# adriente/espm

Measured on AMD Instinct MI355X. Metric: MU iterations/sec, 2048ch x (512*512)px X, k=5 SmoothNMF, higher is better.
Workload: dtype f32; 1 GPU; 2048ch x (512x512)px, k=5, SmoothNMF simplex_H + Laplacian lambda=1, X stored ell, W/H fp32; n=2048, k=5, simplex_H=True, parallelism=single GPU, autotune=True, engine_policy=autotune='auto', as SmoothNMF(max_iter=10000).fit builds it, launch_plan=fused, units handed out dynamically

## Files before the change

espm_amd/_lib.py:

```python
from __future__ import annotations

import ctypes as C
import os

import torch

_HERE = os.path.dirname(os.path.abspath(__file__))
LIB_PATH = os.environ.get("ESPM_MU_LIB", os.path.join(_HERE, "lib", "libespm_mu.so"))

from . import _abi

_HEADER_TEXT = _abi.header_text()
_D = _abi.parse_defines(_HEADER_TEXT)
OK, EINVAL, ENOSOLUTION, EHIP, EUNSUPPORTED = 0, -1, -2, -3, -4
X_F32, X_BF16, X_U8, X_ELL = 0, 1, 2, 3
F64_X_U8, F64_X_BF16, F64_X_F32, F64_X_F64 = (_D["ESPM_F64_X_" + n] for n in ("U8", "BF16", "F32", "F64"))
F64_MAX_K, F64_MAXIT = _D["ESPM_F64_MAX_K"], _D["ESPM_F64_MAXIT"]
F64S_MAX_COUNT, F64S_MAX_N, F64S_WBLOCK = _D["ESPM_F64S_MAX_COUNT"], _D["ESPM_F64S_MAX_N"], _D["ESPM_F64S_WBLOCK"]
DIAG_X_U8, DIAG_X_U16, DIAG_X_F32, DIAG_X_F64 = (_D["ESPM_DIAG_X_" + n] for n in ("U8", "U16", "F32", "F64"))
DIAG_MAX_K, DIAG_BLOCK, DIAG_CHUNK = _D["ESPM_DIAG_MAX_K"], _D["ESPM_DIAG_BLOCK"], _D["ESPM_DIAG_CHUNK"]
CDIAG_BLOCK, CDIAG_PCHUNK = _D["ESPM_CDIAG_BLOCK"], _D["ESPM_CDIAG_PCHUNK"]
BIN_BLOCK, BIN_PARTS = _D["ESPM_BIN_BLOCK"], _D["ESPM_BIN_PARTS"]
SPLIT_BLOCK, SPLIT_HEAVY, SPLIT_MAX_K = _D["ESPM_SPLIT_BLOCK"], _D["ESPM_SPLIT_HEAVY"], _D["ESPM_SPLIT_MAX_K"]
SRC_F32, SRC_F64 = 0, 1
LAYOUT_CM, LAYOUT_PM = 0, 1
ABI_VERSION = _D["ESPM_MU_ABI_VERSION"]
XCHG_HANDLE_BYTES = _D["ESPM_XCHG_HANDLE_BYTES"]
ELL_TILE, ELL_PB, ELL_PBITS, ELL_LDS_MAX = _D["ESPM_ELL_TILE"], _D["ESPM_ELL_PB"], _D["ESPM_ELL_PBITS"], _D["ESPM_ELL_LDS_MAX"]
ELL_STREAM_BYTES = _D["ESPM_ELL_STREAM_BYTES"]
ELL_BUCKETS = _D["ESPM_ELL_BUCKETS"]
ELL_HEAVY_MIN, ELL_HEAVY_MAX = _D["ESPM_ELL_HEAVY_MIN"], _D["ESPM_ELL_HEAVY_MAX"]
ELL_UNIT_ROWS, ELL_UNIT_MAX_N, ELL_PAIR_MAX_K = _D["ESPM_ELL_UNIT_ROWS"], _D["ESPM_ELL_UNIT_MAX_N"], _D["ESPM_ELL_PAIR_MAX_K"]
KP, PPAD, NPAD = _D["ESPM_KP"], _D["ESPM_PPAD"], _D["ESPM_NPAD"]
MAX_K = KP
HP_STRIDE, HS_STRIDE, HI_STRIDE = 8 + 2 * KP, 2 * KP, _D["ESPM_HI_STRIDE"]
HS_ROWSUM, HS_MAX = 0, KP
WIDE_MAX_K = 16
WIDEST_MAX_K = 32
TAIL_DEFER, TAIL_RIDE = _D["ESPM_TAIL_DEFER"], _D["ESPM_TAIL_RIDE"]
HI_KLX, HI_REG, HI_LAP, HI_SUMY, HI_BAD, HI_REL_W, HI_REL_H = (_D["ESPM_HI_" + n] for n in ("KLX", "REG", "LAP", "SUMY", "BAD", "REL_W", "REL_H"))

_vp, _i32, _i64, _f32 = C.c_void_p, C.c_int32, C.c_int64, C.c_float


class MUState(C.Structure):
    _fields_ = _abi.parse_struct(_HEADER_TEXT)

    def __init__(self, *args, **kw):
        super().__init__(*args, **kw)
        self.struct_size = C.sizeof(type(self))
        self.abi_version = ABI_VERSION


_SP = C.POINTER(MUState)
SYMBOLS = {
    "espm_mu_version": (C.c_char_p, []),
    "espm_mu_last_error": (C.c_char_p, []),
    "espm_mu_state_size": (C.c_size_t, []),
    "espm_mu_abi_version": (C.c_int, []),
    "espm_mu_state_layout": (C.c_char_p, []),
    "espm_mu_query": (C.c_int, [_SP]),
    "espm_mu_w_update_is_local": (C.c_int, [_SP]),
    "espm_mu_w_update_tail": (C.c_int, [_SP, C.c_int, C.c_int, _vp]),
    "espm_mu_pack_x": (C.c_int, [_vp, C.c_int, C.c_int, _i64, C.c_int, C.c_int, _vp, _vp, C.c_int, C.c_int, C.c_int, C.c_int, C.c_int, _vp]),
    "espm_mu_ell_count": (C.c_int, [_SP, _vp, _vp, _vp, _vp, _vp]),
    "espm_mu_ell_count_hist": (C.c_int, [_SP, _vp, _vp, _vp, _vp, _vp, _vp, _vp]),
    "espm_mu_ell_fill_hist": (C.c_int, [_SP, _vp, _vp, _vp, _vp, _vp, _vp, _vp, _vp, _vp, _vp]),
    "espm_mu_ell_plan": (C.c_int, [_SP, _vp, _vp, _vp, _vp, _vp, _vp, _vp, _vp]),
    "espm_mu_ell_fill": (C.c_int, [_SP, _vp, _vp, _vp, _vp, _vp, _vp, _vp, _vp]),
    "espm_mu_ell_heavy_count": (C.c_int, [_SP, _vp, C.c_int, C.c_int, _i64, _vp, _vp, _vp, _vp]),
    "espm_mu_ell_heavy_fill": (C.c_int, [_SP, _vp, C.c_int, C.c_int, _i64, _vp, _vp, _vp]),
    "espm_mu_hstat": (C.c_int, [_SP, C.c_int, _vp]),
    "espm_mu_build_gw": (C.c_int, [_SP, C.c_int, _vp]),
    "espm_mu_step_h": (C.c_int, [_SP, C.c_int, C.c_int, _vp]),
    "espm_mu_h_finalize": (C.c_int, [_SP, C.c_int, C.c_int, _vp]),
    "espm_mu_loss_only": (C.c_int, [_SP, C.c_int, C.c_int, _vp]),
    "espm_mu_w_accum": (C.c_int, [_SP, _vp]),
    "espm_mu_step_hw": (C.c_int, [_SP, C.c_int, _vp]),
    "espm_mu_fused_applies": (C.c_int, [_SP]),
    "espm_mu_w_reduce": (C.c_int, [_SP, _vp]),
    "espm_mu_w_reduce_finalize": (C.c_int, [_SP, C.c_int, C.c_int, _vp]),
    "espm_mu_w_finish": (C.c_int, [_SP, C.c_int, C.c_int, C.c_int, _vp]),
    "espm_mu_iterate_timed": (C.c_int, [_SP, C.c_int, _vp, _vp, _vp]),
    "espm_mu_iterate": (C.c_int, [_SP, C.c_int, C.c_int, _vp]),
    "espm_mu_iterate_h": (C.c_int, [_SP, C.c_int, C.c_int, _vp]),
    "espm_mu_h_chain_applies": (C.c_int, [_SP]),
    "espm_mu_shard_record_bytes": (C.c_size_t, [_SP]),
    "espm_mu_shard_pack": (C.c_int, [_SP, C.c_int, _vp, _vp]),
    "espm_mu_shard_combine": (C.c_int, [_SP, _vp, C.c_int, C.c_int, _vp]),
    "espm_mu_shard_combine_finish": (C.c_int, [_SP, _vp, C.c_int, C.c_int, C.c_int, _vp]),
    "espm_mu_w_reduce_finish": (C.c_int, [_SP, C.c_int, C.c_int, C.c_int, _vp]),
    "espm_mu_w_reduce_pack": (C.c_int, [_SP, C.c_int, C.c_int, _vp, _vp]),
    "espm_xchg_create": (C.c_int, [C.c_int, C.c_int, C.c_size_t, C.POINTER(_vp)]),
    "espm_xchg_handle": (C.c_int, [_vp, _vp]),
    "espm_xchg_connect": (C.c_int, [_vp, _vp]),
    "espm_xchg_staging": (_vp, [_vp]),
    "espm_xchg_records": (_vp, [_vp, C.c_int]),
    "espm_xchg_post": (C.c_int, [_vp, C.c_uint32, _vp]),
    "espm_xchg_wait": (C.c_int, [_vp, C.c_uint32, _vp]),
    "espm_xchg_timeouts": (C.c_int, [_vp, C.POINTER(C.c_uint32)]),
    "espm_xchg_set_order": (C.c_int, [_vp, C.c_int]),
    "espm_xchg_order": (C.c_int, [_vp]),
    "espm_xchg_destroy": (C.c_int, [_vp]),
    "espm_mu_shard_exchange_finish": (C.c_int, [_SP, _vp, C.c_uint32, C.c_int, C.c_int, _vp]),
    "espm_mu_iterate_sharded": (C.c_int, [_SP, _vp, C.POINTER(C.c_uint32), C.c_int, C.c_int, _vp]),
    "espm_mu_linesearch_terms": (C.c_int, [_SP, C.c_int, C.c_int, _vp, _vp]),
    "espm_mu_linesearch_terms_sharded": (C.c_int, [_SP, C.c_int, C.c_int, _vp, _vp, _vp, _vp]),
    "espm_surrogate_terms": (C.c_int, [_vp, _vp, C.c_int, C.c_int, C.c_int64, C.c_int, C.c_int, C.c_int, _vp, C.c_int, _vp, _vp]),
    "espm_dichotomy_simplex_acc": (C.c_int, [C.c_double, _vp, _vp, C.c_int, C.c_int, C.c_int, C.c_double, C.c_double, C.c_int, _vp, _vp, _vp]),
    "espm_dichotomy_simplex_pg": (C.c_int, [_vp, C.c_int, C.c_int, C.c_double, C.c_double, C.c_int, _vp, _vp]),
    "espm_mu_l2_step_h": (C.c_int, [_SP, C.c_int, _vp, _vp, C.c_int, _vp]),
    "espm_mu_l2_step_w": (C.c_int, [_SP, C.c_int, _vp, _vp, _vp, C.c_int, _vp]),
    "espm_mu_l2_w_partials": (C.c_int, [_SP, _vp, _vp, C.c_int, _vp]),
    "espm_mu_l2_w_finish": (C.c_int, [_SP, C.c_int, _vp, _vp, _vp]),
    "espm_simplex_root_f32": (C.c_int, [_vp, _vp, C.c_int, C.c_int, C.c_float, C.c_float, C.c_int, C.c_int, _vp, _vp, _vp, _vp]),
    "espm_dichotomy_simplex": (C.c_int, [_vp, _vp, C.c_int, C.c_int, C.c_int, C.c_double, C.c_double, C.c_int, _vp, _vp, _vp]),
    "espm_mu_laplacian": (C.c_int, [_vp, C.c_int, C.c_int, C.c_int, _i64, _vp, _vp]),
    "espm_lu_pl_scratch_bytes": (C.c_size_t, [C.c_int, C.c_int, C.c_int]),
    "espm_lu_pl": (C.c_int, [_vp, C.c_int, C.c_int, C.c_int, _i64, _vp, _vp, C.c_size_t, _vp]),
    "espm_f64_scratch_doubles": (_i64, [C.c_int, C.c_int, C.c_int, _i64]),
    "espm_f64_gw": (C.c_int, [_vp, _vp, C.c_int, C.c_int, C.c_int, C.c_double, _vp, _vp, _vp, _vp]),
    "espm_f64_hstat": (C.c_int, [_vp, C.c_int, C.c_int, C.c_double, _vp, _vp, _vp]),
    "espm_f64_h_pass": (C.c_int, [_vp, C.c_int, C.c_int, C.c_int, C.c_double, _vp, _vp, _vp, _vp, C.c_int, _vp, _vp, C.c_double,
                                  C.c_double, C.c_double, C.c_int, C.c_int, C.c_double, C.c_int, _vp, _vp, _vp, _vp, _vp, _vp, _vp]),
    "espm_f64_bisect": (C.c_int, [_vp, _vp, C.c_int, C.c_int, C.c_double, C.c_double, C.c_int, _vp, _vp, _vp, _vp, _vp]),
    "espm_f64_rel": (C.c_int, [_vp, _vp, _i64, C.c_double, _vp, _vp, _vp]),
    "espm_f64_w_accum": (C.c_int, [_vp, C.c_int, C.c_int, C.c_int, C.c_double, _vp, _vp, C.c_int, C.c_double, _vp, _vp, _vp]),
    "espm_f64_w_finish": (C.c_int, [_vp, _vp, _vp, C.c_int, C.c_int, C.c_int, _vp, _vp, C.c_int, _vp, C.c_int, C.c_double, C.c_double,
                                    C.c_int, _vp, _vp, _vp, _vp]),
    "espm_f64_sparse_scratch_doubles": (_i64, [C.c_int, C.c_int, C.c_int]),
    "espm_f64_sparse_h_pass": (C.c_int, [_vp, _vp, _vp, C.c_int, _vp, C.c_int, C.c_int, C.c_double, _vp, _vp, _vp, _vp, C.c_int, _vp, _vp,
                                         C.c_double, C.c_double, C.c_double, C.c_int, C.c_int, C.c_double, C.c_int, _vp, _vp, _vp, _vp,
                                         _vp, _vp, _vp]),
    "espm_f64_sparse_w_accum": (C.c_int, [_vp, _vp, _vp, _vp, _vp, C.c_int, C.c_int, C.c_double, _vp, _vp, C.c_int, C.c_double, _vp, _vp,
                                          _vp]),
    "espm_pixel_diagnostics": (C.c_int, [_vp, C.c_int, C.c_int, _i64, C.c_int, C.c_int, _vp, _vp, C.c_int, C.c_double, C.c_int, _vp, _vp,
                                         _vp, _vp]),
    "espm_channel_diagnostics": (C.c_int, [_vp, C.c_int, C.c_int, _i64, C.c_int, C.c_int, _vp, _vp, C.c_int, C.c_double, _vp, _vp, _vp, _vp,
                                           _vp, C.c_size_t, _vp]),
    "espm_channel_diagnostics_scratch": (C.c_size_t, [C.c_int, C.c_int, C.c_int]),
    "espm_rebin_pixels": (C.c_int, [_vp, C.c_int, C.c_int, _i64, C.c_int, C.c_int, C.c_int, C.c_int, C.c_int, _vp, C.c_int, _i64, _vp]),
    "espm_binning_sums": (C.c_int, [_vp, C.c_int, C.c_int, _i64, C.c_int, C.c_int, C.c_int, _vp, C.c_int, _vp, _vp, C.c_size_t, _vp]),
    "espm_binning_sums_scratch": (C.c_size_t, [C.c_int, C.c_int, C.c_int, C.c_int]),
    "espm_thin_counts": (C.c_int, [_vp, C.c_int, C.c_int, _i64, C.c_int, C.c_int, _i64, _i64, _i64, C.c_uint64, _vp, _vp, _i64, _vp]),
    "espm_split_deviance": (C.c_int, [_vp, C.c_int, C.c_int, _i64, C.c_int, C.c_int, _i64, _i64, _i64, C.c_uint64, _vp, _vp, C.c_int, C.c_double,
                                      _vp, _vp, _vp, _vp]),
}

# ... 77 lines not shown
```

espm_amd/csrc/mu_api.hip:

```cpp
#include <vector>
#include <stdarg.h>
#include <stdio.h>

#include "mu_common.hpp"
#include "mu_xchg.hpp"

namespace espm {

static thread_local char g_err[512] = "";

int set_error(int code, const char* fmt, ...) {
  va_list ap;
  va_start(ap, fmt);
  vsnprintf(g_err, sizeof(g_err), fmt, ap);
  va_end(ap);
  return code;
}

int check_hip(hipError_t e, const char* what) {
  if (e == hipSuccess) return ESPM_OK;
  return set_error(ESPM_EHIP, "%s: %s", what, hipGetErrorString(e));
}

static int roundup(int v, int m) { return (v + m - 1) / m * m; }

#define ESPM_MU_STATE_FIELDS(F) \
  F(struct_size) F(abi_version) F(n) F(m) F(k) F(p) F(nx) F(ny) F(n_pad) F(p_pad) F(x_dtype) F(tile_px) F(nblk_w) \
  F(x_tile) F(n_cm) F(h_variant) F(p_total) F(simplex_h) F(simplex_w) F(grid_mode) F(compute_loss) F(lambda_l) \
  F(sigma_l) F(eps_reg) F(log_shift) F(dicotomy_tol) F(rel_tol) F(xscale) F(gw_floor) F(x_cm) F(x_pm) F(g) \
  F(colsum_g) F(w) F(gw_s) F(colsum_gw) F(gw_a) F(gw_p) F(h) F(h_t) F(mu) F(fixed_h) F(fixed_w) F(simplex_rows) \
  F(halo_top) F(halo_bot) F(hpart) F(hstat) F(a_slab) F(a) F(w_scratch) F(hist) F(hist_len) F(cur) F(it) F(ell_h) \
  F(ell_h_off) F(ell_klc) F(ell_w) F(ell_w_off) F(chan_perm) F(ell_cbits) F(n_cg) F(pix_perm) F(g_t) F(breg_sr_px) \
  F(breg_sr_ch) F(h_rule) F(pg_gamma_w) F(pg_q) F(ell_fill_px) F(ell_fill_num) F(ell_fill_n) F(tail_mode) F(no_fused) \
  F(ell_pb) F(ell_stream) F(ell_hv_n) F(ell_hv_npx) F(ell_hv_ngrp) F(ell_hv_px) F(ell_hv_px_off) F(ell_hv_pm) F(ell_hv_klc) F(ell_hv_kl) \
  F(ell_hv_grp) F(ell_hv_grp_off) F(ell_hv_wm) F(hpart_alt)

static int check_abi(const espm_mu_state* st) {
  ESPM_REQUIRE(st != nullptr, "state is NULL");
  ESPM_REQUIRE(st->struct_size == (uint32_t)sizeof(espm_mu_state) && st->abi_version == (uint32_t)ESPM_MU_ABI_VERSION,
               "espm_mu_state of %u bytes, ABI %u handed to a library built for %zu bytes, ABI %d: the binding's copy of the layout has drifted",
               st->struct_size, st->abi_version, sizeof(espm_mu_state), ESPM_MU_ABI_VERSION);
  return ESPM_OK;
}

static int check_state(const espm_mu_state* st) {
  if (int rc = check_abi(st)) return rc;
  ESPM_REQUIRE(st->n >= 1 && st->p >= 1, "n=%d, p=%d must be >= 1", st->n, st->p);
  if (st->k < ESPM_MIN_K || st->k > ESPM_MAX_K)
    return set_error(ESPM_EUNSUPPORTED, "k=%d: this build supports %d..%d components", st->k, ESPM_MIN_K, ESPM_MAX_K);
  ESPM_REQUIRE(st->n_pad == roundup(st->n, ESPM_NPAD) && st->p_pad == roundup(st->p, ESPM_PPAD),
               "n_pad/p_pad (%d, %d) do not match n, p (%d, %d); call espm_mu_query", st->n_pad, st->p_pad, st->n,
               st->p);
  ESPM_REQUIRE(st->x_dtype >= ESPM_X_F32 && st->x_dtype <= ESPM_X_ELL, "bad x_dtype %d", st->x_dtype);
  if (st->x_dtype == ESPM_X_ELL) {
    ESPM_REQUIRE(st->ell_h && st->ell_h_off && st->ell_klc && st->ell_w && st->ell_w_off && st->chan_perm && st->pix_perm,
                 "the sparse count store needs ell_h, ell_h_off, ell_klc, ell_w, ell_w_off, chan_perm and pix_perm");
    ESPM_REQUIRE((st->tile_px == 64 || st->tile_px == 128 || st->tile_px == 256 || st->tile_px == ESPM_ELL_TILE) &&
                     st->ell_pb == 2 * st->tile_px && st->nblk_w == (st->p + st->ell_pb - 1) / st->ell_pb &&
                     st->n_cg == (st->n + 63) / 64 && st->h_variant == 0,
                 "sparse count store: tile_px must be 64..%d, ell_pb 2 tile_px, nblk_w ceil(p / ell_pb), n_cg ceil(n / 64); call espm_mu_query",
                 ESPM_ELL_TILE);
  }
  ESPM_REQUIRE(st->ell_stream == 0 || (st->ell_stream == 1 && st->x_dtype == ESPM_X_ELL), "ell_stream=%d: 0, or 1 with the sparse store", st->ell_stream);
  ESPM_REQUIRE(st->ell_fill_n >= 0 && (st->ell_fill_n == 0 || (st->x_dtype == ESPM_X_ELL && st->ell_fill_px && st->ell_fill_num)),
               "ell_fill_n=%d needs the sparse store, ell_fill_px and ell_fill_num", st->ell_fill_n);
  ESPM_REQUIRE(st->ell_hv_n >= 0 && (st->ell_hv_n == 0 || (st->x_dtype == ESPM_X_ELL && st->h_rule == 0 && !st->breg_sr_px && st->ell_hv_npx >= 1 &&
                                                          st->ell_hv_npx <= st->ell_hv_n && st->ell_hv_ngrp >= 1 && st->ell_hv_ngrp <= st->ell_hv_n &&
                                                          st->ell_hv_px && st->ell_hv_px_off && st->ell_hv_pm && st->ell_hv_klc && st->ell_hv_kl &&
                                                          st->ell_hv_grp && st->ell_hv_grp_off && st->ell_hv_wm && st->ell_fill_num)),
               "ell_hv_n=%d needs the sparse store with the default H rule, 1 <= ell_hv_npx, ell_hv_ngrp <= ell_hv_n, every ell_hv_* array and "
               "ell_fill_num", st->ell_hv_n);
  ESPM_REQUIRE(st->grid_mode == 0 || (st->nx >= 1 && st->ny >= 1 && st->nx * st->ny == st->p),
               "grid %d x %d does not match p=%d", st->nx, st->ny, st->p);
  ESPM_REQUIRE(st->xscale > 0.f, "xscale must be positive");
  ESPM_REQUIRE(st->n_cm == roundup(st->n, ESPM_NCM), "n_cm must be roundup(n, %d)", ESPM_NCM);
  ESPM_REQUIRE((st->breg_sr_px == nullptr) == (st->breg_sr_ch == nullptr), "breg_sr_px and breg_sr_ch come together");
  ESPM_REQUIRE(!st->breg_sr_px || (st->m == 0 && !st->simplex_w && st->n <= 4096),
               "the Bregman variant is built for G = identity without simplex_W (and n <= 4096)");
  ESPM_REQUIRE(st->h_rule == 0 || ((st->h_rule == 1 || st->h_rule == 2) && !st->breg_sr_px), "h_rule must be 0, 1 or 2 (1, 2 not with the Bregman variant)");
  ESPM_REQUIRE(!(st->pg_gamma_w > 0.f) || (!st->simplex_w && !st->breg_sr_px && (st->m == 0 || (long)st->m * st->k <= 8192)),
               "the projected-gradient W step has no simplex over W (updates.py:368-369), no Bregman variant, and needs M k <= 8192 with a dictionary");
  ESPM_REQUIRE(st->h_variant == 0, "h_variant %d is not built (the matrix-core H-step was retired, DESIGN.md)", st->h_variant);
  ESPM_REQUIRE(st->x_tile >= 64 && ESPM_PPAD % st->x_tile == 0 && st->x_tile % st->tile_px == 0,
               "x_tile=%d must divide %d and be a multiple of tile_px=%d", st->x_tile, ESPM_PPAD, st->tile_px);
  ESPM_REQUIRE(st->m >= 0, "m must be >= 0");
  ESPM_REQUIRE(st->m == 0 || (st->g && st->colsum_g), "m=%d needs g and colsum_g", st->m);
  if (st->log_shift > 0.f && st->simplex_h && (double)st->k * (double)st->log_shift >= 1.0)
    return set_error(ESPM_ENOSOLUTION, "No solution exists! (k * log_shift >= 1)");
  return ESPM_OK;
}

static int nblk_h(const espm_mu_state* st) { return (st->p + st->tile_px - 1) / st->tile_px; }

static int ell_pre_h(const espm_mu_state* st, int src, hipStream_t s) {
  const int ld = st->ell_fill_n + (st->ell_hv_n > 0 ? st->ell_hv_npx : 0);
  if (st->ell_fill_n > 0)
    if (int rc = launch_ell_fill_num(st->gw_s, st->h[src], st->ell_fill_px, st->ell_fill_n, st->n, st->k, st->p_pad, st->log_shift,
                                     st->ell_fill_num, s, ld))
      return rc;
  return st->ell_hv_n > 0 ? launch_ell_hv_h(st, src, ld, s) : ESPM_OK;
}

static int ell_post(const espm_mu_state* st, int hnew, bool w, bool loss, hipStream_t s) {
  if (st->ell_hv_n <= 0) return ESPM_OK;
  if (hnew >= 0) return launch_ell_hv_post(st, st->h[hnew], (size_t)st->p_pad, 1, w, loss, s);
  return launch_ell_hv_post(st, st->h_t, 1, ESPM_KP, w, loss, s);
}

static bool fused_ok(const espm_mu_state* st) {
  return ESPM_MIN_K <= 8 && st->x_dtype == ESPM_X_ELL && st->h_rule == 0 && st->no_fused != 1 &&
         (st->ell_pb >= ESPM_FUSED_MIN_PB || st->nblk_w >= ESPM_FUSED_MIN_BLOCKS || st->no_fused == 3) &&
         fused_ell_lds_bytes(st->n_pad, st->k, st->ell_pb) <= ESPM_ELL_LDS_MAX;
}
static HStepArgs fused_h_args(const espm_mu_state* st, int src) {
  HStepArgs a = make_h_args(st, src, 1);
  a.rec_nb = nblk_h(st);
  return a;
}
// ... 730 lines not shown
```

espm_amd/csrc/mu_common.hpp:

```cpp
#pragma once
#include <hip/hip_runtime.h>
#include <stdint.h>

#include "espm_mu.h"

namespace espm {

constexpr int KP = ESPM_KP;
static_assert(KP == 8 || KP == 16 || KP == 32, "ESPM_KP: 8, 16 or 32");
static_assert(ESPM_MIN_K >= 1 && ESPM_MAX_K <= KP && ESPM_MIN_K <= ESPM_MAX_K, "ESPM_MIN_K .. ESPM_MAX_K must fit the stride");

#if ESPM_MIN_K <= 8
#define ESPM_K_CASES(X) X(1) X(2) X(3) X(4) X(5) X(6) X(7) X(8)
#elif ESPM_MIN_K <= 16
#define ESPM_K_CASES(X) X(9) X(10) X(11) X(12) X(13) X(14) X(15) X(16)
#else
#define ESPM_K_CASES(X) X(17) X(18) X(19) X(20) X(21) X(22) X(23) X(24) X(25) X(26) X(27) X(28) X(29) X(30) X(31) X(32)
#endif

__device__ __forceinline__ void store_row_kp(float* dst, const float (&row)[KP]) {
#pragma unroll
  for (int q = 0; q < KP / 4; ++q)
    reinterpret_cast<float4*>(dst)[q] = make_float4(row[4 * q], row[4 * q + 1], row[4 * q + 2], row[4 * q + 3]);
}
// ... 494 lines not shown
  float x = fminf(fmaxf(0.f, lo), hi), dxold = hi - lo;
  for (int it = 0; it < maxit; ++it) {
    float f = -target, fp = 0.f;
#pragma unroll
    for (int i = 0; i < K; ++i) {
      const float s = b[i] + x, q = 4.f * a * c[i];
      const float r = __builtin_amdgcn_sqrtf(fmaf(s, s, q));
      const float g = s >= 0.f ? q * __builtin_amdgcn_rcpf(r + s) : r - s;
      if (g > floor_g) {
        f += g;
        fp -= g * __builtin_amdgcn_rcpf(r);
      } else {
        f += floor_g;
      }
    }
    if (fabsf(f) <= 4e-7f * target) break;
    if (f > 0.f) lo = x; else hi = x;
    float dx = fp < 0.f ? -f * __builtin_amdgcn_rcpf(fp) : 0.f;
    float xn = x + dx;
    if (!(fp < 0.f) || !(xn > lo && xn < hi) || fabsf(dx) > 0.5f * fabsf(dxold)) {
      dx = (hi - lo) * 0.5f;
      xn = lo + dx;
    }
    dxold = dx;
    if (xn == x) break;
    x = xn;
  }
  nu = x;
  return true;
}

__device__ __forceinline__ float stencil_hl(const float* hrow, const float* halo_top, const float* halo_bot,
                                            int q, int nx, int ny, float hc) {
  const int i = q / ny, j = q - i * ny;
  float acc = 0.f;
  int deg = 0;
  if (j > 0) { acc += hrow[q - 1]; ++deg; }
  if (j < ny - 1) { acc += hrow[q + 1]; ++deg; }
  if (i > 0) { acc += hrow[q - ny]; ++deg; }
  else if (halo_top) { acc += halo_top[j]; ++deg; }
  if (i < nx - 1) { acc += hrow[q + ny]; ++deg; }
  else if (halo_bot) { acc += halo_bot[j]; ++deg; }
  return (float)deg * hc - acc;
}

struct HFinalizeArgs {
  const double* hpart;
  const double* colsum_gw;
  const double* hstat_in;
  double* hstat_out;
  double* hist_slot;
  int nblk, k, compute_loss, have_prev;
  float xscale;
  double* pg_q;
};
struct HStepArgs {
  const void* x_cm;
  const void* x_pm;
  int mfma;
  const float* gw_s;
  const double* colsum_gw;
  const float* h_in;
  float* h_out;
  float* h_t;
  const float* mu;
  const float* fixed_h;
  const float* halo_top;
  const float* halo_bot;
  const double* hstat_in;
  double* hpart;
  int n, k, p, nx, ny, p_pad;
  int x_tile;
  int n_cm;
  const void* gw_a;
  const float* gw_p;
  int simplex_h, grid_mode, compute_loss, write_h;
  int have_prev;
  float lambda_l, sigma_l, eps_reg, log_shift, tol, xscale, rel_tol;
  double inv_count;
  const uint32_t* ell;
  const int32_t* ell_off;
  const float* ell_klc;
  const int32_t* ell_pix;
  int ell_bits, n_pad;
  int ell_tp;
  const float* l2_m;
  const float* breg_sr;
  int h_rule;
  const float* fill_num;
  int fill_n;
  const double* cs_parts;
  int cs_nbk, cs_lds_off, tail_on;
  WTailArgs tail;
  int rec_nb;
  const double* chain_prev;
  int chain_nb, chain_lds_off, chain_fin_on;
  HFinalizeArgs chain_fin;
};
__host__ __device__ inline int ell_pbits(int pb) {
  int b = 6;
  while ((1 << b) < pb) ++b;
  return b;
}
struct WAccumArgs {
  const void* x_pm;
  const void* x_cm;
  int x_tile, n_cm, p_pad, mfma;
  const float* gw_s;
  const float* h_t;
  float* a_slab;
  int n_pad, p, ppb;
  const uint32_t* ell;
  const int32_t* ell_off;
  const int32_t* chan_perm;
  int n_cg;
  int pb, pbits;
  int l2;
};
struct WFinishArgs {
  const float* g;
  const float* g_t;
  const float* colsum_g;
  const float* w_old;
  float* w_new;
  const float* a;
  const double* hstat;
  const float* fixed_w;
  const int32_t* simplex_rows;
  float* scratch;
  const float* breg_sr;
  float pg_gamma_w;
  double* pg_q;
  float* gw_s;
  double* colsum_gw;
  void* gw_a;
  float* gw_p;
  double* hist_slot;
  int n, m, k, n_pad, n_cm, simplex_w, update_w;
  float log_shift, tol, rel_tol, xscale, gw_floor;
};


__device__ __forceinline__ void h_finalize_body(const HFinalizeArgs& a, double* scratch) {
  constexpr int NV = ESPM_HP_NSCALAR + 2 * KP + 1;
  constexpr int V_RELH = 4 + KP, V_MAX = 5 + KP, V_RELW = 5 + 2 * KP;
  double v[NV];
#pragma unroll
  for (int i = 0; i < NV; ++i) v[i] = 0.0;
  v[V_RELW] = -1.0;
  const size_t nb = a.nblk;
  constexpr int U = KP > 8 ? 1 : 4;
  for (int b0 = threadIdx.x; b0 < a.nblk; b0 += U * 256) {
    double t[U][ESPM_HP_RELH + 1], tw[U];
#pragma unroll
    for (int u = 0; u < U; ++u) {
      const int b = b0 + u * 256;
#pragma unroll
      for (int i = 0; i <= ESPM_HP_RELH; ++i) t[u][i] = b < a.nblk ? a.hpart[i * nb + b] : 0.0;
      tw[u] = b < a.nblk ? a.hpart[(size_t)ESPM_HP_RELW * nb + b] : -1.0;
    }
#pragma unroll
    for (int u = 0; u < U; ++u) {
#pragma unroll
      for (int i = 0; i < 4 + KP; ++i) v[i] += t[u][i];
      v[V_RELH] = fmax(v[V_RELH], t[u][ESPM_HP_RELH]);
      v[V_RELW] = fmax(v[V_RELW], tw[u]);
// ... 44 lines not shown
    if (a.pg_q) {
      double q1[1] = {0.0};
      for (int b = threadIdx.x; b < a.nblk; b += 256) q1[0] += a.hpart[(size_t)ESPM_HP_PGQ * nb + b];
      block_reduce<1, 1>(q1, scratch);
      if (threadIdx.x == 0) *a.pg_q = q1[0];
    }
    return;
  }
  const bool is_sum = job < 4 + KP;
  const int field = is_sum ? job : (job == V_RELH ? ESPM_HP_RELH : (job == V_RELW ? ESPM_HP_RELW : ESPM_HP_MAX + (job - V_MAX)));
  double v[1] = {job == V_RELW ? -1.0 : 0.0};
  for (int b = threadIdx.x; b < a.nblk; b += 256) {
    const double t = a.hpart[(size_t)field * nb + b];
    v[0] = is_sum ? v[0] + t : fmax(v[0], t);
  }
  if (is_sum)
    block_reduce<1, 1>(v, scratch);
  else
    block_reduce<1, 0>(v, scratch);
  if (threadIdx.x != 0) return;
  if (job == ESPM_HP_KL) {
    if (a.compute_loss) a.hist_slot[ESPM_HI_KLX] = (double)a.xscale * 0.6931471805599453 * v[0];
  } else if (job == ESPM_HP_REG) {
    a.hist_slot[ESPM_HI_REG] = v[0];
  } else if (job == ESPM_HP_LAP) {
    a.hist_slot[ESPM_HI_LAP] = v[0];
  } else if (job == ESPM_HP_BAD) {
    a.hist_slot[ESPM_HI_BAD] = v[0];
  } else if (is_sum) {
    if (a.hstat_out) a.hstat_out[ESPM_HS_ROWSUM + (job - ESPM_HP_ROWSUM)] = v[0];
  } else if (job == V_RELH) {
    if (a.have_prev) a.hist_slot[ESPM_HI_REL_H] = v[0];
  } else if (job == V_RELW) {
    if (v[0] >= 0.0) a.hist_slot[ESPM_HI_REL_W] = v[0];
  } else {
    if (a.hstat_out) a.hstat_out[ESPM_HS_MAX + (job - V_MAX)] = v[0];
  }
}


inline HStepArgs make_h_args(const espm_mu_state* st, int src, int write_h) {
  HStepArgs a;
  a.x_cm = st->x_cm;
  a.x_pm = st->x_pm;
  a.mfma = st->no_fused == 0;
  a.gw_s = st->gw_s;
  a.colsum_gw = st->colsum_gw;
  a.h_in = st->h[src];
  a.h_out = st->h[1 - src];
  a.h_t = st->h_t;
  a.mu = st->mu;
  a.fixed_h = st->fixed_h;
  a.halo_top = st->grid_mode ? st->halo_top : nullptr;
  a.halo_bot = st->grid_mode ? st->halo_bot : nullptr;
  a.hstat_in = st->hstat[src];
  a.hpart = st->hpart;
  a.n = st->n;
  a.k = st->k;
  a.p = st->p;
  a.nx = st->nx;
  a.ny = st->ny;
  a.p_pad = st->p_pad;
  a.x_tile = st->x_tile;
  a.n_cm = st->n_cm;
  a.gw_a = st->gw_a;
  a.gw_p = st->gw_p;
  a.simplex_h = st->simplex_h;
  a.grid_mode = st->grid_mode;
  a.compute_loss = st->compute_loss;
  a.write_h = write_h;
  a.have_prev = st->it > 0;
  a.rel_tol = st->rel_tol;
  a.inv_count = 1.0 / ((double)st->k * (double)(st->p_total > 0 ? st->p_total : st->p));
  a.lambda_l = st->lambda_l;
  a.sigma_l = st->sigma_l;
  a.eps_reg = st->eps_reg;
  a.log_shift = st->log_shift;
  a.tol = st->dicotomy_tol;
  a.xscale = st->xscale;
  a.ell = st->ell_h;
  a.ell_off = st->ell_h_off;
  a.ell_klc = st->ell_klc;
  a.ell_pix = st->pix_perm;
  a.ell_bits = st->ell_cbits;
  a.ell_tp = st->tile_px;
  a.l2_m = nullptr;
  a.breg_sr = st->breg_sr_px;
  a.h_rule = st->h_rule;
  a.fill_n = st->ell_fill_n + (st->ell_hv_n > 0 ? st->ell_hv_npx : 0);
  a.fill_num = (st->x_dtype == ESPM_X_ELL && a.fill_n > 0) ? st->ell_fill_num : nullptr;
  a.cs_parts = nullptr;
  a.cs_nbk = a.cs_lds_off = a.tail_on = 0;
  a.rec_nb = 0;
  a.chain_prev = nullptr;
  a.chain_nb = a.chain_lds_off = a.chain_fin_on = 0;
  a.chain_fin = HFinalizeArgs{};
  a.n_pad = st->n_pad;
  return a;
}

inline WAccumArgs make_w_args(const espm_mu_state* st) {
  WAccumArgs a;
  a.x_pm = st->x_pm;
  a.x_cm = st->x_cm;
  a.x_tile = st->x_tile;
  a.n_cm = st->n_cm;
  a.p_pad = st->p_pad;
  a.mfma = st->no_fused == 0;
  a.gw_s = st->gw_s;
  a.h_t = st->h_t;
  a.a_slab = st->a_slab;
  a.n_pad = st->n_pad;
  a.p = st->p;
  a.ppb = (st->p + st->nblk_w - 1) / st->nblk_w;
  a.ell = st->ell_w;
  a.ell_off = st->ell_w_off;
  a.chan_perm = st->chan_perm;
  a.n_cg = st->n_cg;
  a.pb = st->ell_pb > 0 ? st->ell_pb : ESPM_ELL_PB;
  a.pbits = ell_pbits(a.pb);
  a.l2 = 0;
  return a;
}

int dispatch_h_step(const HStepArgs& args, int x_dtype, int tile_px, int nblk, hipStream_t stream);
bool h_chain_built(const espm_mu_state* st);
int launch_h_chain(const HStepArgs& args, int x_dtype, int tile_px, int nblk, hipStream_t stream);
int launch_h_finalize(const HFinalizeArgs& args, hipStream_t stream);
int launch_h_ell(const HStepArgs& args, int nblk, hipStream_t stream);
int launch_fused_ell(const HStepArgs& h, const WAccumArgs& w, int nblk, hipStream_t stream, int static_units = 0, int stream_lists = 0);
size_t fused_ell_lds_bytes(int n_pad, int k, int pb);
int launch_ell_count(const uint8_t* x_pm, int n, int n_pad, int p, int p_pad, int cbits, int n_cg, int nblk, int pb,
                     int32_t* cnt_px, int32_t* cnt_bc, float* klc, hipStream_t stream, uint8_t* bkt_px = nullptr, uint8_t* bkt_bc = nullptr);
int launch_ell_plan(const int32_t* cnt_px, const int32_t* cnt_bc, int n, int n_cg, int nblk, int p_pad, int win,
                    int32_t* chan_perm, int32_t* pix_perm, int32_t* h_off, int32_t* w_off, long long* rows, hipStream_t stream);
int launch_ell_fill(const uint8_t* x_pm, int n, int n_pad, int p, int p_pad, int cbits, int n_cg, int nblk, int win, int pb,
                    const int32_t* chan_perm, const int32_t* pix_perm, const int32_t* h_off, const int32_t* w_off,
                    uint32_t* ell_h, uint32_t* ell_w, hipStream_t stream, const uint8_t* x_cm = nullptr, int n_cm = 0, const uint8_t* bkt_px = nullptr,
                    const uint8_t* bkt_bc = nullptr);
int launch_w_ell(const WAccumArgs& args, int k, int nblk, hipStream_t stream);
int launch_ell_fill_num(const float* gw_s, const float* h_in, const int32_t* fill_px, int fill_n, int n, int k, int p_pad, float fill,
                        float* fill_num, hipStream_t stream, int ld = 0);
int launch_ell_hv_count(const void* x, int src_dtype, int layout, int64_t ld, int n, int p, int n_pad, int n_cm, uint8_t* x8, uint8_t* x8c,
                        int32_t* cnt_px, hipStream_t stream);
int launch_ell_hv_fill(const void* x, int src_dtype, int layout, int64_t ld, int n, int p, const int32_t* px_off, int32_t* hv_pm,
                       hipStream_t stream);
int launch_ell_hv_h(const espm_mu_state* st, int src, int ld, hipStream_t stream);
int launch_ell_hv_post(const espm_mu_state* st, const float* h, size_t hs_k, size_t hs_p, bool w, bool loss, hipStream_t stream);
int dispatch_w_accum(const WAccumArgs& args, int k, int x_dtype, int nblk, hipStream_t stream);
int launch_w_reduce(const float* slab, float* out, int nblk, int total, const HFinalizeArgs* fused_finalize,
                    hipStream_t stream, const float* bw_old = nullptr, double* bparts = nullptr, int n = 0, int k = 0, int n_pad = 0);
int launch_w_simplex_update(const WFinishArgs& f, float* a_inout, const double* bparts, double tol, hipStream_t stream, WTailArgs* defer_tail);
int launch_w_reduce_pack(const float* slab, int nblk, int k, int n_pad, const HFinalizeArgs& fin_to_record,
                         const float* h_new, int nx, int ny, int p_pad, int with_halo, void* rec, hipStream_t stream);
int launch_w_finish(const WFinishArgs& args, hipStream_t stream);
int launch_gram(const float* m, int rows, int k, double* part, int part_cap, float* out, hipStream_t stream);
int launch_w_finish_l2(const float* a, int n, int n_pad, int m, int k, const float* g, const float* gtg, const float* hh, const float* w_old,
                       float* w_new, const float* fixed_w, float log_shift, hipStream_t stream);
int launch_w_reduce_update(const WFinishArgs& f, const void* src, size_t src_stride, int nsrc, float* a_out,
                           const double* hpart, int nblk_h, const double* hstat_rs, size_t rec_hstat_off, double* hstat_out,
                           const HFinalizeArgs* fused_finalize, hipStream_t stream, WTailArgs* defer_tail = nullptr);
int launch_w_update_tail(const WTailArgs& t, hipStream_t stream);
int launch_w_exchange_update(const WFinishArgs& f, const void* slabs, size_t slab_stride, int nslab, float* a_out, double* hstat_out,
                             const HFinalizeArgs& fin, const struct ::espm_xchg* xc, unsigned int seq, const float* h_new, int nx, int ny,
                             int p_pad, int with_halo, hipStream_t stream, WTailArgs* defer_tail, double* simplex_bparts = nullptr);
bool w_gsplit_applies(const WFinishArgs& args);
// ... 24 lines not shown
```

espm_amd/csrc/mu_ell_build.hip:

```cpp
#include <mutex>

#include "mu_common.hpp"

namespace espm {

__device__ __forceinline__ int ell_reps(int x, int xmax) { return (x + xmax - 1) / xmax; }

template <typename F>
__device__ __forceinline__ void ell_block_for_each_count(const uint8_t* __restrict__ x_pm, int n, int n_pad, int q_mine,
                                                         uint32_t* tile, int* s_q, F f) {
  static_assert(ESPM_NPAD % 8 == 0, "8-byte row reads");
  const int t = threadIdx.x;
  s_q[t] = q_mine;
  __syncthreads();
  for (int c0 = 0; c0 < n; c0 += 128) {
#pragma unroll
    for (int i = 0; i < 16; ++i) {
      const int id = i * 256 + t, r = id >> 4, c8 = id & 15;
      const int q = s_q[r], c = c0 + 8 * c8;
      uint2 v = make_uint2(0u, 0u);
      if (q >= 0 && c < n_pad) v = *reinterpret_cast<const uint2*>(x_pm + (size_t)q * n_pad + c);
      tile[r * 33 + 2 * c8] = v.x;
      tile[r * 33 + 2 * c8 + 1] = v.y;
    }
// ... 320 lines not shown
      for (int u = 0; u < 16; ++u)
        if (x[u] != 0) f(qb + u - q0, x[u]);
    }
  };
  if (units) {
    bk.clear();
    if (bkt) {
      for (int i = 0; i < EllBuckets::B; ++i) bk.c(i) = bkt[((size_t)b * n_cg * 64 + c) * EllBuckets::B + i];
    } else {
      for_each_count([&](int i, int x) {
        if (x == 1) bk.count(i);
      });
    }
    holes = bk.plan(lane, units);
  }
  int j = 0, overflow = 0;
  for_each_count([&](int i, int x) {
    if (x == 1 && units) {
      const int pos = bk.place(i, lane, units, holes, overflow);
      if (pos >= 0) {
        ell_put(base16, row0, pos, lane, (uint32_t)i << 4);
        return;
      }
    }
    while (x > 0) {
      const int v = x > xmax ? xmax : x;
      ell_put(base16, row1, j++, lane, ((uint32_t)v << pbits) | (uint32_t)i);
      x -= v;
    }
  });
}

struct SideStream {
  hipStream_t stream = nullptr;
  hipEvent_t fork = nullptr, join = nullptr;
};
static hipStream_t side_stream_of_device() {
  static const bool enabled = [] { const char* e = getenv("ESPM_ELL_BUILD_SIDE"); return !(e && e[0] == '0'); }();
  if (!enabled) return nullptr;
  static std::mutex mu;
  static hipStream_t per_device[64] = {};
  int dev = 0;
  if (hipGetDevice(&dev) != hipSuccess || dev < 0 || dev >= 64) return nullptr;
  std::lock_guard<std::mutex> lock(mu);
  if (!per_device[dev] && hipStreamCreateWithFlags(&per_device[dev], hipStreamNonBlocking) != hipSuccess) per_device[dev] = nullptr;
  return per_device[dev];
}
static hipStream_t side_fork(SideStream& s, hipStream_t stream) {
  s.stream = side_stream_of_device();
  if (!s.stream) return stream;
  if (hipEventCreateWithFlags(&s.fork, hipEventDisableTiming) != hipSuccess || hipEventCreateWithFlags(&s.join, hipEventDisableTiming) != hipSuccess ||
      hipEventRecord(s.fork, stream) != hipSuccess || hipStreamWaitEvent(s.stream, s.fork, 0) != hipSuccess) {
    (void)hipGetLastError();
    s.stream = nullptr;
    return stream;
  }
  return s.stream;
}
static int side_join(SideStream& s, hipStream_t stream) {
  int rc = ESPM_OK;
  if (s.stream) {
    rc = check_hip(hipEventRecord(s.join, s.stream), "ell build: side stream");
    if (!rc) rc = check_hip(hipStreamWaitEvent(stream, s.join, 0), "ell build: side stream");
  }
  if (s.fork) (void)hipEventDestroy(s.fork);
  if (s.join) (void)hipEventDestroy(s.join);
  return rc;
}

int launch_ell_count(const uint8_t* x_pm, int n, int n_pad, int p, int p_pad, int cbits, int n_cg, int nblk, int pb,
                     int32_t* cnt_px, int32_t* cnt_bc, float* klc, hipStream_t stream, uint8_t* bkt_px, uint8_t* bkt_bc) {
  const int xmax_h = (1 << (16 - cbits)) - 1, xmax_w = (1 << (16 - ell_pbits(pb))) - 1;
  SideStream side;
  const hipStream_t s2 = side_fork(side, stream);
  hipLaunchKernelGGL(ell_count_h_kernel, dim3((p_pad + 255) / 256), dim3(256), 0, stream, x_pm, n, n_pad, p, p_pad, xmax_h,
                     n <= ESPM_ELL_UNIT_MAX_N ? 1 : 0, cnt_px, klc, bkt_px);
  hipLaunchKernelGGL(ell_count_w_kernel, dim3(nblk, (n_cg * 64 + 255) / 256), dim3(256), 0, s2, x_pm, n, n_pad, p,
                     n_cg * 64, xmax_w, pb, cnt_bc, bkt_bc);
  const int rc = check_hip(hipGetLastError(), "ell_count launch");
  const int rc2 = side_join(side, stream);
  return rc ? rc : rc2;
}

int launch_ell_plan(const int32_t* cnt_px, const int32_t* cnt_bc, int n, int n_cg, int nblk, int p_pad, int win,
                    int32_t* chan_perm, int32_t* pix_perm, int32_t* h_off, int32_t* w_off, long long* rows, hipStream_t stream) {
  const size_t lds = (size_t)(n > win ? n : win) * sizeof(int32_t);
  if (lds > 64 * 1024) {
    if (int rc = check_hip(hipFuncSetAttribute(reinterpret_cast<const void*>(ell_order_kernel),
                                               hipFuncAttributeMaxDynamicSharedMemorySize, (int)lds), "ell_plan"))
      return rc;
  }
  hipLaunchKernelGGL(ell_order_kernel, dim3(nblk + p_pad / win), dim3(1024), lds, stream, cnt_px, cnt_bc, n, n_cg, nblk, win,
                     chan_perm, pix_perm);
  const long long groups = (long long)(p_pad / 64) + (long long)nblk * n_cg;
  hipLaunchKernelGGL(ell_group_extent_kernel, dim3((unsigned)((groups + 3) / 4)), dim3(256), 0, stream, cnt_px, cnt_bc, n_cg, nblk,
                     p_pad / 64, win, chan_perm, pix_perm, h_off, w_off);
  hipLaunchKernelGGL(ell_offsets_kernel, dim3(1), dim3(1024), 0, stream, n_cg, nblk, p_pad / 64, h_off, w_off, rows);
  return check_hip(hipGetLastError(), "ell_plan launch");
}

int launch_ell_fill(const uint8_t* x_pm, int n, int n_pad, int p, int p_pad, int cbits, int n_cg, int nblk, int win, int pb,
                    const int32_t* chan_perm, const int32_t* pix_perm, const int32_t* h_off, const int32_t* w_off,
                    uint32_t* ell_h, uint32_t* ell_w, hipStream_t stream, const uint8_t* x_cm, int n_cm, const uint8_t* bkt_px,
                    const uint8_t* bkt_bc) {
  SideStream side;
  const hipStream_t s2 = side_fork(side, stream);
  hipLaunchKernelGGL(ell_fill_h_kernel, dim3((p_pad + 255) / 256), dim3(256), 0, stream, x_pm, n, n_pad, p, p_pad, cbits, win,
                     pix_perm, h_off, ell_h, bkt_px);
  hipLaunchKernelGGL(ell_fill_w_kernel, dim3(nblk, (n_cg + ESPM_ELL_FILLW_WAVES - 1) / ESPM_ELL_FILLW_WAVES), dim3(64 * ESPM_ELL_FILLW_WAVES), 0, s2, x_pm, x_cm, n_cm, n_pad, p, n_cg, pb, ell_pbits(pb), chan_perm, w_off, ell_w, bkt_bc);
  const int rc = check_hip(hipGetLastError(), "ell_fill launch");
  const int rc2 = side_join(side, stream);
  return rc ? rc : rc2;
}

}
```

espm_amd/csrc/mu_ell_kernel.hpp:

```cpp
#pragma once
#include "mu_h_kernel.hpp"


namespace espm {

typedef float lds_v4f __attribute__((ext_vector_type(4)));
typedef float lds_v2f __attribute__((ext_vector_type(2)));
#define ESPM_LDS(T) __attribute__((address_space(3))) const T*
__device__ __forceinline__ uint32_t lds_address(const float* ptr) {
  return (uint32_t)(uintptr_t)(__attribute__((address_space(3))) const float*)ptr;
}
__device__ __forceinline__ void ell_table_at_lds_zero(const float* tab) {
  if (lds_address(tab) != 0u) __builtin_trap();
}
template <int K>
struct EllTab {
  static constexpr int WB = LdsTabGeom<K>::WB;
  static constexpr int FLOATS = 4 + WB;
  static constexpr int WQ = WB / 4;
  static __device__ __forceinline__ const float* quad(const float* tab, int rows) { return tab + (size_t)WB * rows; }
  static __device__ __forceinline__ void put(float* tab, int rows, int r, const float* src) {
    float row[(K + 3) / 4 * 4];
#pragma unroll
    for (int i = 0; i < (K + 3) / 4 * 4; i += 4) {
// ... 3 lines not shown
    lds_table_put_row<K>(tab, rows, r, row);
  }
  static __device__ __forceinline__ void get(const float* tab, int rows, uint32_t r, float (&g)[K]) {
#ifdef ESPM_EXPERIMENT_GENERAL_NOCONFLICT
    r = (threadIdx.x & 15) + 16 * ((r >> 4) & 7);
#endif
    const float4 lo = reinterpret_cast<const float4*>(quad(tab, rows))[r];
    const float l[4] = {lo.x, lo.y, lo.z, lo.w};
#pragma unroll
    for (int i = 0; i < (K < 4 ? K : 4); ++i) g[i] = l[i];
    if constexpr (WB == 1) g[4] = tab[r];
    if constexpr (WB == 2) {
      const float2 v = reinterpret_cast<const float2*>(tab)[r];
      g[4] = v.x;
      g[5] = v.y;
    }
    if constexpr (WB >= 4) {
#pragma unroll
      for (int q = 0; q < WQ; ++q) {
        const float4 v = reinterpret_cast<const float4*>(tab)[(size_t)r * WQ + q];
        const float h[4] = {v.x, v.y, v.z, v.w};
#pragma unroll
        for (int i = 0; i < 4; ++i)
          if (4 + 4 * q + i < K) g[4 + 4 * q + i] = h[i];
      }
    }
  }
  static __device__ __forceinline__ void get_unit(uint32_t lds_q, uint32_t off, float (&g)[K]) {
    const lds_v4f lo = *(ESPM_LDS(lds_v4f))(uintptr_t)(lds_q + off);
#pragma unroll
    for (int i = 0; i < (K < 4 ? K : 4); ++i) g[i] = lo[i];
    if constexpr (WB == 1) g[4] = *(ESPM_LDS(float))(uintptr_t)(off >> 2);
    if constexpr (WB == 2) {
      const lds_v2f v = *(ESPM_LDS(lds_v2f))(uintptr_t)(off >> 1);
      g[4] = v[0];
      g[5] = v[1];
    }
    if constexpr (WB >= 4) {
      const uint32_t base = off * WQ;
#pragma unroll
      for (int q = 0; q < WQ; ++q) {
        const lds_v4f v = *(ESPM_LDS(lds_v4f))(uintptr_t)(base + 16 * q);
#pragma unroll
        for (int i = 0; i < 4; ++i)
          if (4 + 4 * q + i < K) g[4 + 4 * q + i] = v[i];
      }
    }
  }
};

#ifndef ESPM_ELL_DOT_PLAIN
#define ESPM_ELL_DOT_PLAIN 0
#endif
#ifndef ESPM_ELL_DOT_PLAIN_K
#define ESPM_ELL_DOT_PLAIN_K 5
#endif
template <int K>
__device__ __forceinline__ float ell_dot(const float (&g)[K], const float (&h)[K]) {
  if constexpr (ESPM_ELL_DOT_PLAIN || K == ESPM_ELL_DOT_PLAIN_K) {
    float y = g[0] * h[0];
#pragma unroll
    for (int i = 1; i < K; ++i) y = fmaf(g[i], h[i], y);
    return y;
  } else if constexpr (K == 1) {
    return g[0] * h[0];
  } else {
    f2 s = f2{g[0], g[1]} * f2{h[0], h[1]};
#pragma unroll
    for (int q = 1; q < K / 2; ++q) s = f2{g[2 * q], g[2 * q + 1]} * f2{h[2 * q], h[2 * q + 1]} + s;
    float y = s.x + s.y;
    if constexpr (K & 1) y = fmaf(g[K - 1], h[K - 1], y);
    return y;
  }
}
template <int K>
__device__ __forceinline__ void ell_axpy(float (&acc)[K], const float (&g)[K], float r) {
#pragma unroll
  for (int q = 0; q < K / 2; ++q) {
    const f2 t = f2{g[2 * q], g[2 * q + 1]} * r + f2{acc[2 * q], acc[2 * q + 1]};
    acc[2 * q] = t.x;
    acc[2 * q + 1] = t.y;
  }
  if constexpr (K & 1) acc[K - 1] = fmaf(g[K - 1], r, acc[K - 1]);
}

struct EllNoFlush {
  template <typename Redo>
  __device__ __forceinline__ void operator()(Redo) const {}
};
template <int PRIO>
__device__ __forceinline__ void ell_walk_prio(int left) {
  if constexpr (PRIO > 0) {
    if (left > 3 * PRIO) __builtin_amdgcn_s_setprio(3);
    else if (left > 2 * PRIO) __builtin_amdgcn_s_setprio(2);
    else if (left > PRIO) __builtin_amdgcn_s_setprio(1);
    else __builtin_amdgcn_s_setprio(0);
  }
}
template <bool STREAM>
__device__ __forceinline__ uint32_t ell_list_load(const uint32_t* p) {
  if constexpr (STREAM) return __builtin_nontemporal_load(p);
  else return *p;
}
template <int UNR, int PF, bool STREAM>
__device__ __forceinline__ bool ell_walk_request(const uint32_t* row, int len, uint32_t (&pre)[PF][UNR]) {
  if (len < UNR) return false;
#pragma unroll
  for (int d = 0; d < PF; ++d) {
    const int jd = min(d * UNR, len - UNR);
#pragma unroll
    for (int u = 0; u < UNR; ++u) pre[d][u] = ell_list_load<STREAM>(row + (size_t)(jd + u) * 64);
  }
  return true;
}
#ifndef ESPM_ELL_WALK_PP_MAX_K
#define ESPM_ELL_WALK_PP_MAX_K 5
#endif
#ifndef ESPM_ELL_BATCH_HALVES_K
#define ESPM_ELL_BATCH_HALVES_K 7
#endif
template <int K, int UNR, int PF = 1, int PRIO = 0, bool STREAM = false, bool PP = false, typename Get, typename Body, typename Flush = EllNoFlush>
__device__ __forceinline__ void ell_walk_pre(const uint32_t* row, int len, Get get, Body body, Flush flush, bool use_pre, const uint32_t (&pre)[PF][UNR]) {
  auto batch = [&](const uint32_t (&e)[UNR]) {
    constexpr int HALVES = (K >= ESPM_ELL_BATCH_HALVES_K && K <= 8 && UNR % 2 == 0) ? 2 : 1;
    constexpr int UH = UNR / HALVES;
#pragma unroll
    for (int hh = 0; hh < HALVES; ++hh) {
      float g[2 * UH][K], x[2 * UH];
#pragma unroll
      for (int u = 0; u < UH; ++u) {
        x[2 * u] = get(e[hh * UH + u], 0, g[2 * u]);
        x[2 * u + 1] = get(e[hh * UH + u], 1, g[2 * u + 1]);
      }
#pragma unroll
      for (int u = 0; u < 2 * UH; ++u) body(x[u], g[u]);
      if constexpr (HALVES > 1) __builtin_amdgcn_sched_barrier(0);
    }
    flush([&](auto alt) {
#pragma unroll
      for (int u = 0; u < UNR; ++u) {
        float g0[K], g1[K];
        const float x0 = get(e[u], 0, g0), x1 = get(e[u], 1, g1);
        alt(x0, g0);
        alt(x1, g1);
      }
    });
  };
  int j = 0;
  if constexpr (PF == 1 && PP) {
    if (len >= UNR) {
      uint32_t qa[UNR], qb[UNR];
      if (use_pre) {
#pragma unroll
        for (int u = 0; u < UNR; ++u) qa[u] = pre[0][u];
      } else {
#pragma unroll
        for (int u = 0; u < UNR; ++u) qa[u] = ell_list_load<STREAM>(row + (size_t)u * 64);
      }
      for (; j + 2 * UNR <= len; j += 2 * UNR) {
        ell_walk_prio<PRIO>(len - j);
        const int jb = min(j + UNR, len - UNR);
#pragma unroll
        for (int u = 0; u < UNR; ++u) qb[u] = ell_list_load<STREAM>(row + (size_t)(jb + u) * 64);
        batch(qa);
        ell_walk_prio<PRIO>(len - j - UNR);
        const int ja = min(j + 2 * UNR, len - UNR);
#pragma unroll
        for (int u = 0; u < UNR; ++u) qa[u] = ell_list_load<STREAM>(row + (size_t)(ja + u) * 64);
        batch(qb);
      }
      if (j + UNR <= len) {
        ell_walk_prio<PRIO>(len - j);
        batch(qa);
        j += UNR;
      }
    }
  } else if (len >= UNR) {
    uint32_t q[PF][UNR];
    if (use_pre) {
#pragma unroll
      for (int d = 0; d < PF; ++d)
#pragma unroll
        for (int u = 0; u < UNR; ++u) q[d][u] = pre[d][u];
    } else {
#pragma unroll
      for (int d = 0; d < PF; ++d) {
        const int jd = min(d * UNR, len - UNR);
#pragma unroll
        for (int u = 0; u < UNR; ++u) q[d][u] = ell_list_load<STREAM>(row + (size_t)(jd + u) * 64);
      }
    }
    for (; j + UNR <= len; j += UNR) {
      ell_walk_prio<PRIO>(len - j);
      uint32_t e[UNR];
#pragma unroll
      for (int u = 0; u < UNR; ++u) e[u] = q[0][u];
#pragma unroll
      for (int d = 0; d + 1 < PF; ++d)
#pragma unroll
        for (int u = 0; u < UNR; ++u) q[d][u] = q[d + 1][u];
      const int jn = min(j + PF * UNR, len - UNR);
#pragma unroll
      for (int u = 0; u < UNR; ++u) q[PF - 1][u] = ell_list_load<STREAM>(row + (size_t)(jn + u) * 64);
      batch(e);
    }
  }
  for (; j < len; ++j) {
    const uint32_t v = ell_list_load<STREAM>(row + (size_t)j * 64);
    float g0[K], g1[K];
    const float x0 = get(v, 0, g0), x1 = get(v, 1, g1);
    body(x0, g0);
    body(x1, g1);
    flush([&](auto alt) {
      float a0[K], a1[K];
      const float y0 = get(v, 0, a0), y1 = get(v, 1, a1);
      alt(y0, a0);
      alt(y1, a1);
    });
  }
}
template <int K, int UNR, int PF = 1, int PRIO = 0, bool STREAM = false, bool PP = false, typename Get, typename Body, typename Flush = EllNoFlush>
__device__ __forceinline__ void ell_walk(const uint32_t* row, int len, Get get, Body body, Flush flush = Flush()) {
  uint32_t none[PF][UNR];
  ell_walk_pre<K, UNR, PF, PRIO, STREAM, PP>(row, len, get, body, flush, false, none);
}
template <int K>
struct EllGet {
  const float* tab;
  int rows, idx_bits;
  uint32_t mask;
  __device__ __forceinline__ EllGet(const float* t, int r, int bits) : tab(t), rows(r), idx_bits(bits), mask((1u << bits) - 1u) {}
  __device__ __forceinline__ float operator()(uint32_t e, int half, float (&g)[K]) const {
    const uint32_t v = half ? e >> 16 : e & 0xffffu;
    EllTab<K>::get(tab, rows, v & mask, g);
    return (float)(v >> idx_bits);
  }
};
template <int K>
struct EllGetUnit {
  uint32_t lds_q;
  __device__ __forceinline__ EllGetUnit(int rows) : lds_q((uint32_t)(EllTab<K>::WB * rows) * 4u) {}
  __device__ __forceinline__ float operator()(uint32_t e, int half, float (&g)[K]) const {
    EllTab<K>::get_unit(lds_q, half ? e >> 16 : e & 0xffffu, g);
    return 1.f;
  }
};

template <int K>
struct EllGetUnitFix {
  static constexpr bool FIXED = FixTab<K>::TWO && FixTab<K>::FIXED;
  uint32_t lds_q;
  __device__ __forceinline__ EllGetUnitFix(int rows = 0) : lds_q((uint32_t)(EllTab<K>::WB * rows) * 4u) {}
  static __device__ __forceinline__ void row(uint32_t off, float (&g)[K]) {
    const lds_v4f lo = *(ESPM_LDS(lds_v4f))(uintptr_t)off;
#pragma unroll
    for (int i = 0; i < (K < 4 ? K : 4); ++i) g[i] = lo[i];
    if constexpr (K == 5) g[4] = *(ESPM_LDS(float))(uintptr_t)(off + ESPM_TAB2_BASE);
    if constexpr (K == 6) {
      const lds_v2f v = *(ESPM_LDS(lds_v2f))(uintptr_t)(off + ESPM_TAB2_BASE);
      g[4] = v[0];
      g[5] = v[1];
    }
    if constexpr (K >= 7) {
      const lds_v4f v = *(ESPM_LDS(lds_v4f))(uintptr_t)(off + ESPM_TAB2_BASE);
#pragma unroll
      for (int i = 0; i < 4; ++i)
        if (4 + i < K) g[4 + i] = v[i];
    }
  }
  __device__ __forceinline__ float operator()(uint32_t e, int half, float (&g)[K]) const {
    if constexpr (FIXED || K <= 4) row(half ? e >> 16 : e & 0xffffu, g);
    else EllTab<K>::get_unit(lds_q, half ? e >> 16 : e & 0xffffu, g);
    return 1.f;
  }
};
template <int K>
struct EllGetFix {
  const float* tab;
  int rows, idx_bits;
  uint32_t mask;
  __device__ __forceinline__ EllGetFix(const float* t, int r, int bits) : tab(t), rows(r), idx_bits(bits), mask((1u << bits) - 1u) {}
  __device__ __forceinline__ float operator()(uint32_t e, int half, float (&g)[K]) const {
    const uint32_t v = half ? e >> 16 : e & 0xffffu;
    if constexpr (EllGetUnitFix<K>::FIXED || K <= 4) EllGetUnitFix<K>::row((v & mask) << 4, g);
    else EllTab<K>::get(tab, rows, v & mask, g);
    return (float)(v >> idx_bits);
  }
};
template <int K, bool FIX>
struct EllGetters {
  typedef EllGetUnit<K> Unit;
  typedef EllGet<K> General;
};
template <int K>
struct EllGetters<K, true> {
  typedef EllGetUnitFix<K> Unit;
  typedef EllGetFix<K> General;
};

#ifndef ESPM_ELL_KLPROD
#define ESPM_ELL_KLPROD 1
#endif
template <int K, bool LOSS, int UNR, int PF, int PRIO = 0, bool STREAM = false, bool FIX = false, bool PP = false>
__device__ __forceinline__ void ell_h_rows(const uint32_t* lrow, int x0, int x1, int mid, const float* tab, int n_pad, int ell_bits,
                                           const float (&hk)[K], float (&acc)[K], float& kl) {
  if (x0 < mid) {
    if constexpr (LOSS && ESPM_ELL_KLPROD) {
      float prod = 1.f;
      ell_walk<K, UNR, PF, PRIO, STREAM, PP>(lrow + (size_t)x0 * 64, min(x1, mid) - x0, typename EllGetters<K, FIX>::Unit(n_pad),
        [&](float, const float (&g)[K]) {
          const float r = __builtin_amdgcn_rcpf(ell_dot<K>(g, hk));
          ell_axpy<K>(acc, g, r);
          prod *= r;
        },
        [&](auto redo) {
          const bool ok = __builtin_amdgcn_classf(prod, 0x100);
          if (__builtin_expect(__builtin_amdgcn_ballot_w64(!ok) != 0, 0)) {
            redo([&](float, const float (&g)[K]) { kl += __builtin_amdgcn_logf(__builtin_amdgcn_rcpf(ell_dot<K>(g, hk))); });
          } else {
            kl += __builtin_amdgcn_logf(prod);
          }
          prod = 1.f;
        });
    } else {
      ell_walk<K, UNR, PF, PRIO, STREAM, PP>(lrow + (size_t)x0 * 64, min(x1, mid) - x0, typename EllGetters<K, FIX>::Unit(n_pad), [&](float, const float (&g)[K]) {
        const float r = __builtin_amdgcn_rcpf(ell_dot<K>(g, hk));
        ell_axpy<K>(acc, g, r);
        if constexpr (LOSS) kl += __builtin_amdgcn_logf(r);
      });
    }
  }
  if (x1 > mid) {
    const int g0 = max(x0, mid);
    ell_walk<K, UNR, PF, PRIO, STREAM, PP>(lrow + (size_t)g0 * 64, x1 - g0, typename EllGetters<K, FIX>::General(tab, n_pad, ell_bits), [&](float x, const float (&g)[K]) {
      const float y = ell_dot<K>(g, hk);
      const float r = LOSS ? fmaf(x, __builtin_amdgcn_rcpf(y), 1e-37f) : x * __builtin_amdgcn_rcpf(y);
      ell_axpy<K>(acc, g, r);
      if constexpr (LOSS) kl = fmaf(x, __builtin_amdgcn_logf(r), kl);
    });
  }
}

template <int K, bool LOSS, int UNR, int RULE = 0, bool CHAIN = false>
__global__ __launch_bounds__(ESPM_ELL_TILE, (K > 8 ? 2 : 4)) void h_step_ell_kernel(const HStepArgs a) {
  constexpr int NT = ESPM_ELL_TILE;
  constexpr bool PAIRS_OK = K <= ESPM_ELL_PAIR_MAX_K;
  extern __shared__ __attribute__((aligned(16))) float smem[];
  float* tab = smem;
  ell_table_at_lds_zero(tab);
  float* part = smem + (size_t)a.n_pad * EllTab<K>::FLOATS;
  const int TP = a.ell_tp;
  const int gpw = TP >> 6;
  const bool pairs = PAIRS_OK && gpw == NT / 64;
  double* chain_scr = nullptr;
  if constexpr (CHAIN) {
    if (a.chain_fin_on && blockIdx.x == gridDim.x - 1) {
      chain_finalize_wg(a.chain_fin, reinterpret_cast<double*>(smem));
      return;
    }
    chain_scr = reinterpret_cast<double*>(reinterpret_cast<unsigned char*>(smem) + a.chain_lds_off);
    if (a.chain_prev) chain_stats_wave_stage<K>(a.chain_prev, a.chain_nb, chain_scr);
  } else if (a.tail_on && blockIdx.x == gridDim.x - 1) {
    w_tail_body<20>(a.tail, reinterpret_cast<double*>(smem));
    return;
  }
  double* cs_lds = a.cs_parts ? reinterpret_cast<double*>(reinterpret_cast<unsigned char*>(smem) + a.cs_lds_off) : nullptr;
  const bool cs_late = cs_lds && a.cs_lds_off == 0;
  auto form_cs = [&]() {
    for (int kk = threadIdx.x >> 6; kk < K; kk += NT / 64) {
      double v = 0.0;
      for (int j = threadIdx.x & 63; j < a.cs_nbk; j += 64) v += a.cs_parts[(size_t)kk * a.cs_nbk + j];
      v = wave_sum(v);
      if ((threadIdx.x & 63) == 0) cs_lds[kk] = v;
    }
  };
  if (cs_lds && !cs_late) form_cs();
  for (int r = threadIdx.x; r < a.n_pad; r += NT) EllTab<K>::put(tab, a.n_pad, r, a.gw_s + (size_t)r * KP);
  if (pairs) {
#pragma unroll
    for (int kk = 0; kk < K; ++kk) part[((size_t)K + kk) * TP + threadIdx.x] = 0.f;
  }
  __syncthreads();
  const int lane = threadIdx.x & 63;
  const int wave = __builtin_amdgcn_readfirstlane(threadIdx.x >> 6);
  const int tile0 = blockIdx.x * TP;
  float kl = 0.f;

  auto walk_rows = [&](int gi, int x0, int x1, int slot) {
    const int grp = tile0 / 64 + gi;
    const int lp = a.ell_pix[tile0 + gi * 64 + lane];
    const int px = tile0 + lp;
    float hk[K], acc[K];
#pragma unroll
    for (int kk = 0; kk < K; ++kk) {
      hk[kk] = a.h_in[(size_t)kk * a.p_pad + px];
      acc[kk] = 0.f;
    }
    const int beg = a.ell_off[2 * grp], mid = a.ell_off[2 * grp + 1] - beg;
    const uint32_t* lrow = a.ell + (size_t)beg * 64 + lane;
    ell_h_rows<K, LOSS, UNR, 1>(lrow, x0, x1, mid, tab, a.n_pad, a.ell_bits, hk, acc, kl);
#pragma unroll
    for (int kk = 0; kk < K; ++kk) part[((size_t)slot * K + kk) * TP + lp] = acc[kk];
    if (LOSS && slot == 0) kl += fmaxf(a.ell_klc[px], 0.f);
  };
  auto group_rows = [&](int gi) { return a.ell_off[2 * (tile0 / 64 + gi) + 2] - a.ell_off[2 * (tile0 / 64 + gi)]; };

  int nparts;
  if (pairs) {
    const int gl = wave < 4 ? wave : 7 - wave;
    const int len_l = group_rows(gl), len_s = group_rows(7 - gl);
    const int half = min(len_l, (len_l + len_s + 1) / 2);
    if (wave < 4) {
      walk_rows(gl, 0, half, 0);
    } else {
      walk_rows(wave, 0, len_s, 0);
      if (half < len_l) walk_rows(gl, half, len_l, 1);
    }
    nparts = 2;
  } else {
    const int nsplit = (NT / 64) / gpw;
// ... 63 lines not shown
```

espm_amd/csrc/mu_fused.hip:

```cpp
#include <stdlib.h>

#include "mu_fused_kernel.hpp"

#ifndef ESPM_ELL_UNR_H
#define ESPM_ELL_UNR_H 4
#endif
#ifndef ESPM_FUSED_SMALL_UNR_H
#define ESPM_FUSED_SMALL_UNR_H ESPM_ELL_UNR_H
#endif
#ifndef ESPM_FUSED_SMALL_UNR_W
#define ESPM_FUSED_SMALL_UNR_W ESPM_ELL_UNR_W
#endif
#ifndef ESPM_ELL_UNR_W
#define ESPM_ELL_UNR_W 4
#endif

#ifndef ESPM_FUSED_FULL_PERM_LDS
#define ESPM_FUSED_FULL_PERM_LDS 0
#endif
#define ESPM_FUSED_LDS_LIMIT (160 * 1024)
#ifndef ESPM_FUSED_SMALL_SEGS_DEFAULT
#define ESPM_FUSED_SMALL_SEGS_DEFAULT 0
#endif

// ... 41 lines not shown
    if (red > part) part = red;
    if (tail_scratch > part) part = tail_scratch;
    return part;
  };
  size_t bytes = 0;
  auto layout = [&](size_t part, bool red_in_table) {
    const size_t tab_bytes = FixTab<K>::bytes(tab_rows);
    bytes = tab_bytes + part;
    args.cnt_lds_off = (int)bytes;
    bytes += 16 + ESPM_FUSED_MAX_UNITS * sizeof(float);
    args.meta_lds_off = (int)bytes;
    bytes += (size_t)(3 * (pb / 64) + 2 * args.w.n_cg + 1 + 3) / 4 * 16;
    args.perm_lds_off = (int)bytes;
    const size_t perm_bytes = (size_t)(pb + 64 * args.w.n_cg) * sizeof(int);
    args.perm_lds = pb != ESPM_ELL_PB || (ESPM_FUSED_FULL_PERM_LDS && bytes + perm_bytes + KP * sizeof(double) <= ESPM_FUSED_LDS_LIMIT);
    if (args.perm_lds) bytes += perm_bytes;
    args.red_lds_off = -1;
    const size_t hp_tab = FixTab<K>::bytes(pb);
    if (ESPM_FUSED_RED_ONE_BARRIER && red_in_table && hp_tab + red_own <= tab_bytes) {
      args.red_lds_off = (int)hp_tab;
    } else if (ESPM_FUSED_RED_ONE_BARRIER && bytes + red_own + 2 * KP * sizeof(double) <= ESPM_FUSED_LDS_LIMIT) {
      bytes = (bytes + 7) / 8 * 8;
      args.red_lds_off = (int)bytes;
      bytes += red_own;
    }
    if (args.h.cs_parts) {
      bytes = (bytes + 7) / 8 * 8;
      args.h.cs_lds_off = (int)bytes;
      bytes += 2 * KP * sizeof(double);
    }
  };
  args.h_segs = full ? FusedGeom<K>::S : ESPM_ELL_PB / pb;
  size_t part0 = part_of(args.h_segs);
  bool red_in_table = false;
  if (full) {
    for (int segs = FusedGeom<K>::S_MAX; segs > FusedGeom<K>::S; --segs) {
      bool ok = false;
      for (int rit = 0; rit < 2 && !ok; ++rit) {
        layout(part_of(segs), rit != 0);
        ok = bytes <= ESPM_FUSED_LDS_LIMIT && args.red_lds_off >= 0;
        if (ok) red_in_table = rit != 0;
      }
      if (ok) {
        args.h_segs = segs;
        part0 = part_of(segs);
        break;
      }
    }
  }
  const size_t slab = (size_t)K * args.w.n_pad * sizeof(float);
  args.slab_lds = 0;
  layout(part0, red_in_table);
  args.w_split = 0;
  if (ESPM_FUSED_SLAB_LDS && args.w.n_pad % 4 == 0) {
    if (slab > part0) {
      layout(slab, false);
      if (bytes > ESPM_FUSED_LDS_LIMIT || args.red_lds_off < 0) {
        layout(part0, red_in_table);
      } else {
        args.slab_lds = 1;
        const int want = fused_env_small_segs();
        const int fit = (int)(slab / ((size_t)FusedGeom<K>::PROWS * pb * sizeof(float)));
        int segs = want > 0 ? want : args.h_segs;
        if (segs > fit) segs = fit;
        if (segs > ESPM_FUSED_MAX_SEGS) segs = ESPM_FUSED_MAX_SEGS;
        if (segs > args.h_segs) args.h_segs = segs;
      }
    } else {
      args.slab_lds = args.red_lds_off >= 0;
      args.w_split = ESPM_FUSED_W_SPLIT && args.slab_lds && pb == ESPM_ELL_PB && 2 * slab <= part0;
    }
  }
  if (args.h.tail_on && !args.h.tail.pg_q) args.h.tail_on = 2;
  if (bytes > ((args.perm_lds && pb == ESPM_ELL_PB) || args.red_lds_off >= 0 ? ESPM_FUSED_LDS_LIMIT : ESPM_ELL_LDS_MAX))
    return set_error(ESPM_EUNSUPPORTED, "fused half-steps: %zu bytes of LDS exceed %d", bytes, ESPM_ELL_LDS_MAX);
  {
    const int NT = ESPM_ELL_WTHREADS;
    const int n_perm = args.perm_lds ? pb + 64 * args.w.n_cg : 0, n_woff = 2 * args.w.n_cg + 1;
    const bool staged_ok = args.h.n_pad <= 4 * NT && n_perm <= 4 * NT && n_woff <= NT && args.h.cs_nbk <= 64 && 2 * K <= NT / 64;
    const bool plain = ESPM_FUSED_PLAIN && fused_env_plain() && !args.h.fixed_h && !args.h.fill_num && !args.h.breg_sr && !args.h.l2_m &&
                       args.h.simplex_h && args.h.lambda_l != 0.f && args.h.grid_mode && args.h.have_prev && args.h.write_h && args.h.h_rule == 0 &&
                       args.h.tail_on != 1 && !args.static_units && args.slab_lds && !args.w_split && args.red_lds_off >= 0 && staged_ok &&
                       (args.perm_lds != 0) == (pb != ESPM_ELL_PB) && ESPM_FUSED_SMALL_THREADS == ESPM_ELL_WTHREADS;
    if (plain && args.stream_lists && pb == ESPM_ELL_PB) return launch_fused_plain_stream(args, K, args.h.compute_loss != 0, true, nblk, bytes, stream);
    if (plain) return launch_fused_plain(args, K, args.h.compute_loss != 0, pb == ESPM_ELL_PB, nblk, bytes, stream);
  }
  auto go = [&](auto kern, int threads) -> int {
    if (bytes > 64 * 1024)
      if (int rc = check_hip(hipFuncSetAttribute(reinterpret_cast<const void*>(kern), hipFuncAttributeMaxDynamicSharedMemorySize, (int)bytes),
                             "fused half-steps"))
        return rc;
    hipLaunchKernelGGL(kern, dim3(nblk + (args.h.tail_on == 1 ? 1 : 0)), dim3(threads), bytes, stream, args);
    return check_hip(hipGetLastError(), "fused half-steps launch");
  };
  if (pb == ESPM_ELL_PB)
    return args.h.compute_loss ? go(mu_fused_ell_kernel<K, true, ESPM_ELL_UNR_H, ESPM_ELL_UNR_W, ESPM_ELL_WTHREADS, true>, ESPM_ELL_WTHREADS)
                               : go(mu_fused_ell_kernel<K, false, ESPM_ELL_UNR_H, ESPM_ELL_UNR_W, ESPM_ELL_WTHREADS, true>, ESPM_ELL_WTHREADS);
  return args.h.compute_loss ? go(mu_fused_ell_kernel<K, true, ESPM_FUSED_SMALL_UNR_H, ESPM_FUSED_SMALL_UNR_W, ESPM_FUSED_SMALL_THREADS, false>, ESPM_FUSED_SMALL_THREADS)
                             : go(mu_fused_ell_kernel<K, false, ESPM_FUSED_SMALL_UNR_H, ESPM_FUSED_SMALL_UNR_W, ESPM_FUSED_SMALL_THREADS, false>, ESPM_FUSED_SMALL_THREADS);
}
#endif

size_t fused_ell_lds_bytes(int n_pad, int k, int pb) {
  if (pb < 128 || pb > ESPM_ELL_PB || (pb & (pb - 1))) return (size_t)-1;
  const int tab_rows = n_pad > pb ? n_pad : pb;
  const bool fixed = k > 4 && k >= ESPM_FIXTAB_MIN_K;
  if (fixed && tab_rows > ESPM_TAB2_BASE / 16) return (size_t)-1;
  const int wb = k <= 4 ? 0 : (k == 5 ? 1 : (k == 6 ? 2 : 4));
  const size_t tab_bytes = fixed ? (size_t)ESPM_TAB2_BASE + (size_t)16 * tab_rows : (size_t)(4 + wb) * 4 * tab_rows;
  const int seg = pb == ESPM_ELL_PB ? (k <= 4 ? 4 : (k <= 6 ? 3 : 2)) : ESPM_ELL_PB / pb;
  const int n_cg = (n_pad + 63) / 64;
  size_t part = (size_t)seg * k * pb * 4;
  const size_t red = (size_t)(ESPM_ELL_WTHREADS / 64 + 1) * (ESPM_HP_NSCALAR + 2 * k + 1) * sizeof(double);
  const size_t tail_scratch = (size_t)((ESPM_ELL_WTHREADS / 64 + 1) * (KP + 1) + 1) * sizeof(double);
  if (red > part) part = red;
  if (tail_scratch > part) part = tail_scratch;
  return tab_bytes + part + 16 + ESPM_FUSED_MAX_UNITS * sizeof(float) + (size_t)(3 * (pb / 64) + 2 * n_cg + 4) / 4 * 16 + 2 * KP * sizeof(double) + 8 +
         (pb != ESPM_ELL_PB ? (size_t)(pb + 64 * n_cg) * sizeof(int) : 0);
}

int launch_fused_ell(const HStepArgs& h, const WAccumArgs& w, int nblk, hipStream_t stream, int static_units, int stream_lists) {
  ESPM_REQUIRE(h.ell && h.ell_off && h.ell_klc && h.ell_pix && w.ell && w.ell_off && w.chan_perm, "fused half-steps: the sparse store's lists are missing");
  ESPM_REQUIRE(w.pb >= 128 && w.pb <= ESPM_ELL_PB && (w.pb & (w.pb - 1)) == 0 && 2 * h.ell_tp == w.pb && h.h_rule == 0 && h.write_h && !h.l2_m,
               "fused half-steps: blocks of two H tiles (tile_px=%d, ell_pb=%d), the default H rule, write_h", h.ell_tp, w.pb);
  ESPM_REQUIRE(nblk == (h.p + w.pb - 1) / w.pb && w.n_cg >= 1, "fused half-steps: nblk_w=%d must be ceil(p / %d)", nblk, w.pb);
  FusedArgs fa;
  fa.h = h;
  fa.w = w;
  fa.static_units = static_units;
  fa.stream_lists = stream_lists;
  switch (h.k) {
#if ESPM_MIN_K <= 8
#define ESPM_X(KK) case KK: return launch_fused_k<KK>(fa, nblk, stream);
    ESPM_K_CASES(ESPM_X)
#undef ESPM_X
#endif
  }
  return set_error(ESPM_EUNSUPPORTED, "fused half-steps: k=%d not built", h.k);
}

}

#ifdef ESPM_PHASE_CLOCK
extern "C" int espm_debug_phase_buffer(void* dev_ptr) {
  unsigned long long* p = static_cast<unsigned long long*>(dev_ptr);
  if (int rc = espm::phase_buffer_plain(p)) return rc;
  if (int rc = espm::phase_buffer_plain_stream(p)) return rc;
  return espm::check_hip(hipMemcpyToSymbol(HIP_SYMBOL(espm::espm_phase_buf), &p, sizeof(p)), "phase buffer");
}
#endif
```

espm_amd/csrc/mu_fused_kernel.hpp:

```cpp
#pragma once
#include "mu_ell_kernel.hpp"

#ifndef ESPM_FUSED_SMALL_THREADS
#define ESPM_FUSED_SMALL_THREADS 1024
#endif
#ifndef ESPM_FUSED_SMALL_PREFETCH
#define ESPM_FUSED_SMALL_PREFETCH 1
#endif
#ifndef ESPM_FUSED_CUT2
#define ESPM_FUSED_CUT2 60
#endif
#ifndef ESPM_FUSED_FIRST_PREFETCH
#define ESPM_FUSED_FIRST_PREFETCH 1
#endif
#ifndef ESPM_FUSED_FULL_PREFETCH
#define ESPM_FUSED_FULL_PREFETCH 1
#endif
#ifndef ESPM_FUSED_RED_ONE_BARRIER
#define ESPM_FUSED_RED_ONE_BARRIER 1
#endif
#ifndef ESPM_FUSED_SMALL_PRIO
#define ESPM_FUSED_SMALL_PRIO 4
#endif
#ifndef ESPM_FUSED_FULL_PRIO
// ... 6 lines not shown
#ifndef ESPM_FUSED_SUM_BATCHED
#define ESPM_FUSED_SUM_BATCHED 1
#endif
#ifndef ESPM_FUSED_SLAB_LDS
#define ESPM_FUSED_SLAB_LDS 1
#endif
#ifndef ESPM_FUSED_MAX_SEGS
#define ESPM_FUSED_MAX_SEGS 8
#endif
#ifndef ESPM_FUSED_SMALL_SKEW
#define ESPM_FUSED_SMALL_SKEW 0
#endif
#ifndef ESPM_FUSED_W_SPLIT
#define ESPM_FUSED_W_SPLIT 0
#endif
#ifndef ESPM_FUSED_SLAB_WT
#define ESPM_FUSED_SLAB_WT 1
#endif

namespace espm {

struct FusedArgs {
  HStepArgs h;
  WAccumArgs w;
  int cnt_lds_off;
  int meta_lds_off;
  int perm_lds_off;
  int static_units;
  int red_lds_off;
  int perm_lds;
  int h_segs;
  int w_split;
  int stream_lists;
  int slab_lds;
};

#ifndef ESPM_FUSED_CUT4_A
#define ESPM_FUSED_CUT4_A 45
#endif
#ifndef ESPM_FUSED_CUT4_B
#define ESPM_FUSED_CUT4_B 75
#endif
#ifndef ESPM_FUSED_CUT4_C
#define ESPM_FUSED_CUT4_C 92
#endif
#define ESPM_FUSED_MAX_UNITS 64
template <int K>
struct FusedGeom {
  static constexpr int S = K <= 4 ? 4 : (K <= 6 ? 3 : 2);
  static constexpr int S_MAX = K <= 6 ? 4 : 3;
  static constexpr int PROWS = K;
  static constexpr int MIN_SPLIT = 48;
  static __device__ __forceinline__ int seg_begin(int len, int s) {
    if (len < MIN_SPLIT) return s == 0 ? 0 : len;
    constexpr int cut4[5] = {0, ESPM_FUSED_CUT4_A, ESPM_FUSED_CUT4_B, ESPM_FUSED_CUT4_C, 100}, cut3[4] = {0, 45, 80, 100}, cut2[3] = {0, ESPM_FUSED_CUT2, 100};
    const int c = S == 4 ? cut4[s] : (S == 3 ? cut3[s] : cut2[s]);
    return (int)((long)len * c / 100);
  }
  static __device__ __forceinline__ int seg_begin_rt(int len, int s, int segs) {
    if (len < MIN_SPLIT) return s == 0 ? 0 : len;
    constexpr int cut4[5] = {0, ESPM_FUSED_CUT4_A, ESPM_FUSED_CUT4_B, ESPM_FUSED_CUT4_C, 100}, cut3[4] = {0, 45, 80, 100}, cut2[3] = {0, ESPM_FUSED_CUT2, 100};
    const int c = segs == 4 ? cut4[s] : (segs == 3 ? cut3[s] : cut2[s]);
    return (int)((long)len * c / 100);
  }
  static __device__ __forceinline__ int seg_begin_even(int len, int s, int segs) {
    if (len < MIN_SPLIT) return s == 0 ? 0 : len;
    if constexpr (ESPM_FUSED_SMALL_SKEW != 0) {
      if (segs > 1) return (int)(((long)len * s * (100L * segs + (long)ESPM_FUSED_SMALL_SKEW * (segs - s))) / (100L * segs * segs));
    }
    return (int)((long)len * s / segs);
  }
};

template <int K, bool LOSS, int UNR_H, int UNR_W, int NT, bool FULL, bool PLAIN = false, bool STREAM = false>
__global__ __launch_bounds__(NT) void mu_fused_ell_kernel(const FusedArgs fa) {
  static_assert(!FULL || NT == ESPM_ELL_WTHREADS, "full geometry: 1024 threads");
  static_assert(FULL || !STREAM, "streamed lists: the full geometry (an image below it fits the last-level cache)");
  static_assert(ESPM_ELL_PB == 2 * ESPM_ELL_TILE && ESPM_ELL_WTHREADS == ESPM_ELL_PB, "full geometry: a workgroup is two H tiles, one thread per pixel");
  const int PB = FULL ? ESPM_ELL_PB : fa.w.pb;
  const int PBITS = FULL ? ESPM_ELL_PBITS : fa.w.pbits;
  const int TP = PB / 2;
  const int GPT_SHIFT = PBITS - 7;
  constexpr int PROWS = FusedGeom<K>::PROWS;
  constexpr bool S_RT = FULL && FusedGeom<K>::S_MAX > FusedGeom<K>::S;
  const int S = (FULL && !S_RT) ? FusedGeom<K>::S : fa.h_segs;
  constexpr int PF = FULL ? ESPM_FUSED_FULL_PREFETCH : ESPM_FUSED_SMALL_PREFETCH;
  constexpr bool WALK_PP = FULL && K <= ESPM_ELL_WALK_PP_MAX_K;
  constexpr int PRIO = FULL ? (K >= 5 ? ESPM_FUSED_FULL_PRIO : 0) : ESPM_FUSED_SMALL_PRIO;
  const int NGRP = PB / 64;
  const HStepArgs& a = fa.h;
  extern __shared__ __attribute__((aligned(16))) float smem[];
  float* tab = smem;
  ell_table_at_lds_zero(tab);
  ESPM_PHASE_STAMP(0);
  ESPM_PHASE_WHERE();
  const int tab_rows = a.n_pad > PB ? a.n_pad : PB;
  float* part = smem + FixTab<K>::bytes(tab_rows) / sizeof(float);
  int* cnt = reinterpret_cast<int*>(reinterpret_cast<unsigned char*>(smem) + fa.cnt_lds_off);
  float* ukl = reinterpret_cast<float*>(cnt + 4);
  if (!PLAIN && a.tail_on == 1 && blockIdx.x == gridDim.x - 1) {
    w_tail_body<(10 * ESPM_ELL_WTHREADS) / NT>(a.tail, reinterpret_cast<double*>(smem));
    ESPM_PHASE_STAMP(7);
    return;
  }
  double* cs_lds = a.cs_parts ? reinterpret_cast<double*>(reinterpret_cast<unsigned char*>(smem) + a.cs_lds_off) : nullptr;
  int* meta = reinterpret_cast<int*>(reinterpret_cast<unsigned char*>(smem) + fa.meta_lds_off);
  int* lpix = reinterpret_cast<int*>(reinterpret_cast<unsigned char*>(smem) + fa.perm_lds_off);
  int* lchan = lpix + PB;
  const bool perm_lds = PLAIN ? !FULL : (!FULL || fa.perm_lds);
  const bool spread = a.tail_on == 2 && cs_lds;
  constexpr int RW = 2;
  const int rw_n = a.tail.n * a.tail.k, rw_per = (rw_n + (int)gridDim.x - 1) / (int)gridDim.x;
  const int rw_lo = min(rw_n, (int)blockIdx.x * rw_per), rw_hi = min(rw_n, rw_lo + rw_per);
  const bool rw_staged = rw_per <= RW * NT;
  float rwn[RW], rwo[RW];
#pragma unroll
  for (int u = 0; u < RW; ++u) rwn[u] = rwo[u] = 1.f;
  constexpr bool OWN_H = PLAIN && !FULL && ESPM_FUSED_SMALL_SKEW != 0;
  constexpr bool PREF_W = PLAIN && !FULL && K <= 6 && ESPM_FUSED_FIRST_PREFETCH != 0;
  const int wave_id = __builtin_amdgcn_readfirstlane((int)(threadIdx.x >> 6));
  bool staged = false;
  if constexpr (ESPM_FUSED_PROLOGUE_BATCH) {
    constexpr int TR = 4, PC = 4;
    const int n_perm = perm_lds ? PB + 64 * fa.w.n_cg : 0, n_woff = 2 * fa.w.n_cg + 1;
    staged = PLAIN || (a.n_pad <= TR * NT && n_perm <= PC * NT && n_woff <= NT && a.cs_nbk <= 64 && 2 * K <= NT / 64);
    if (staged) {
      float4 tlo[TR], thi[TR];
#pragma unroll
      for (int i = 0; i < TR; ++i) {
        const int r = threadIdx.x + i * NT;
        const float* src = a.gw_s + (size_t)min(r, a.n_pad - 1) * KP;
        tlo[i] = *reinterpret_cast<const float4*>(src);
        thi[i] = K > 4 ? *reinterpret_cast<const float4*>(src + 4) : make_float4(0.f, 0.f, 0.f, 0.f);
      }
      int pv[PC];
#pragma unroll
      for (int i = 0; i < PC; ++i) {
        const int j = threadIdx.x + i * NT;
        pv[i] = 0;
        if (j < n_perm) pv[i] = j < PB ? a.ell_pix[(size_t)blockIdx.x * PB + j] : fa.w.chan_perm[(size_t)blockIdx.x * fa.w.n_cg * 64 + (j - PB)];
      }
      int mh = 0, mw = 0;
      if ((int)threadIdx.x < 3 * NGRP) {
        const int gi = threadIdx.x / 3, j = threadIdx.x - 3 * gi;
        const bool tile_ok = blockIdx.x * PB + (gi >> GPT_SHIFT) * TP < a.p_pad;
        mh = tile_ok ? a.ell_off[2 * (blockIdx.x * NGRP + gi) + j] : 0;
      }
      if ((int)threadIdx.x < n_woff) mw = fa.w.ell_off[(size_t)2 * blockIdx.x * fa.w.n_cg + threadIdx.x];
      double csv = 0.0;
      const int cw = threadIdx.x >> 6;
      if (cs_lds && cw < K && (int)(threadIdx.x & 63) < a.cs_nbk) csv = a.cs_parts[(size_t)cw * a.cs_nbk + (threadIdx.x & 63)];
      if (spread && cw >= K && cw < 2 * K && (int)(threadIdx.x & 63) < a.cs_nbk)
        csv = a.cs_parts[(size_t)K * a.cs_nbk + (size_t)(cw - K) * a.cs_nbk + (threadIdx.x & 63)];
      if (spread && rw_staged) {
#pragma unroll
        for (int u = 0; u < RW; ++u) {
          const int i = rw_lo + (int)threadIdx.x + u * NT;
          rwn[u] = i < rw_hi ? a.tail.w_new[i] : 1.f;
          rwo[u] = i < rw_hi ? a.tail.w_old[i] : 1.f;
        }
      }
#pragma unroll
      for (int i = 0; i < TR; ++i) {
        const int r = threadIdx.x + i * NT;
        if (r < a.n_pad) FixTab<K>::put(tab, a.n_pad, r, tlo[i], thi[i]);
      }
#pragma unroll
      for (int i = 0; i < PC; ++i) {
        const int j = threadIdx.x + i * NT;
        if (j < n_perm) lpix[j] = pv[i];
      }
      if ((int)threadIdx.x < 3 * NGRP) meta[threadIdx.x] = mh;
      if ((int)threadIdx.x < n_woff) meta[3 * NGRP + threadIdx.x] = mw;
      if (cs_lds && cw < (spread ? 2 * K : K)) {
        csv = wave_sum(csv);
        if ((threadIdx.x & 63) == 0) (cw < K ? cs_lds : cs_lds + KP - K)[cw] = csv;
      }
      if (threadIdx.x == 0) {
        cnt[0] = OWN_H ? NT / 64 : 0;
        cnt[1] = PREF_W ? NT / 64 : 0;
      }
    }
  }
  if (!PLAIN && !staged) {
    if (cs_lds) {
      for (int kk = threadIdx.x >> 6; kk < (spread ? 2 * K : K); kk += NT / 64) {
        double v = 0.0;
        for (int j = threadIdx.x & 63; j < a.cs_nbk; j += 64) v += a.cs_parts[(size_t)kk * a.cs_nbk + j];
        v = wave_sum(v);
        if ((threadIdx.x & 63) == 0) (kk < K ? cs_lds : cs_lds + KP - K)[kk] = v;
      }
    }
    for (int r = threadIdx.x; r < a.n_pad; r += NT) FixTab<K>::put_row(tab, a.n_pad, r, a.gw_s + (size_t)r * KP);
    if (threadIdx.x == 0) cnt[0] = cnt[1] = 0;
    if ((int)threadIdx.x < 3 * NGRP) {
      const int gi = threadIdx.x / 3, j = threadIdx.x - 3 * gi;
      const bool tile_ok = blockIdx.x * PB + (gi >> GPT_SHIFT) * TP < a.p_pad;
      meta[threadIdx.x] = tile_ok ? a.ell_off[2 * (blockIdx.x * NGRP + gi) + j] : 0;
    }
    for (int i = threadIdx.x; i <= 2 * fa.w.n_cg; i += NT) meta[3 * NGRP + i] = fa.w.ell_off[(size_t)2 * blockIdx.x * fa.w.n_cg + i];
    if (perm_lds) {
      for (int i = threadIdx.x; i < PB; i += NT) lpix[i] = a.ell_pix[(size_t)blockIdx.x * PB + i];
      for (int i = threadIdx.x; i < 64 * fa.w.n_cg; i += NT) lchan[i] = fa.w.chan_perm[(size_t)blockIdx.x * fa.w.n_cg * 64 + i];
    }
  }
  __syncthreads();
  ESPM_PHASE_STAMP(1);
  float relw = -1.f;
  if (spread) {
    if (blockIdx.x == 0 && threadIdx.x < KP) a.tail.colsum_gw[threadIdx.x] = (int)threadIdx.x < K ? cs_lds[threadIdx.x] : 0.0;
    if (a.tail.hist_slot) {
      double sw = 0.0;
#pragma unroll
      for (int kk = 0; kk < K; ++kk) sw += cs_lds[KP + kk];
      const float shift = (float)((double)a.tail.rel_tol * (sw / (double)rw_n));
      relw = 0.f;
      if (rw_staged && (PLAIN || staged)) {
#pragma unroll
        for (int u = 0; u < RW; ++u)
          if (rw_lo + (int)threadIdx.x + u * NT < rw_hi) relw = fmaxf(relw, fabsf(rwn[u] - rwo[u]) / (rwn[u] + shift));
      } else {
        for (int i = rw_lo + (int)threadIdx.x; i < rw_hi; i += NT) {
          const float x = a.tail.w_new[i], y = a.tail.w_old[i];
          relw = fmaxf(relw, fabsf(x - y) / (x + shift));
        }
      }
    }
  }
  const int lane = threadIdx.x & 63;
  const int blk0 = blockIdx.x * PB;
  int own_next[2] = {(int)(threadIdx.x >> 6), (int)(threadIdx.x >> 6)};
  auto next_unit = [&](int which) {
    if (!PLAIN && fa.static_units) {
      const int u = own_next[which];
      own_next[which] += NT / 64;
      return __builtin_amdgcn_readfirstlane(u);
    }
    int u = 0;
    if (lane == 0) u = __hip_atomic_fetch_add(cnt + which, 1, __ATOMIC_RELAXED, __HIP_MEMORY_SCOPE_WORKGROUP);
    return __builtin_amdgcn_readfirstlane(u);
  };

  for (int u = OWN_H ? wave_id : next_unit(0); u < NGRP * S; u = next_unit(0)) {
    const int seg = u / NGRP, gi = u - seg * NGRP;
    const int grp = blk0 / 64 + gi;
    float acc[K];
#pragma unroll
    for (int kk = 0; kk < K; ++kk) acc[kk] = 0.f;
    float kl = 0.f;
    int lp = lane;
    if (blk0 + (gi >> GPT_SHIFT) * TP < a.p_pad) {
      lp = perm_lds ? lpix[gi * 64 + lane] : a.ell_pix[grp * 64 + lane];
      const int beg = meta[3 * gi], mid = meta[3 * gi + 1] - beg, len = meta[3 * gi + 2] - beg;
      const int x0 = FULL ? (S_RT ? FusedGeom<K>::seg_begin_rt(len, seg, S) : FusedGeom<K>::seg_begin(len, seg)) : FusedGeom<K>::seg_begin_even(len, seg, S);
      const int x1 = FULL ? (S_RT ? FusedGeom<K>::seg_begin_rt(len, seg + 1, S) : FusedGeom<K>::seg_begin(len, seg + 1)) : FusedGeom<K>::seg_begin_even(len, seg + 1, S);
      if (x0 < x1) {
        const int px = blk0 + (gi >> GPT_SHIFT) * TP + lp;
        float hk[K];
#pragma unroll
        for (int kk = 0; kk < K; ++kk) hk[kk] = a.h_in[(size_t)kk * a.p_pad + px];
        const uint32_t* lrow = a.ell + (size_t)beg * 64 + lane;
        ell_h_rows<K, LOSS, UNR_H, PF, PRIO, STREAM, true, WALK_PP>(lrow, x0, x1, mid, tab, a.n_pad, a.ell_bits, hk, acc, kl);
        if constexpr (PRIO > 0) __builtin_amdgcn_s_setprio(0);
      }
    }
    float* dst = part + (size_t)seg * PROWS * PB + (gi >> GPT_SHIFT) * TP + lp;
#pragma unroll
    for (int kk = 0; kk < K; ++kk) dst[(size_t)kk * PB] = acc[kk];
    if constexpr (LOSS) {
      const float klw = wave_sum(kl);
      if (lane == 0) ukl[u] = klw;
    } else if (lane == 0) {
      ukl[u] = 0.f;
    }
  }
  ESPM_PHASE_STAMP(2);
  ESPM_WAVE_STAMP(8);
  uint32_t fw_rows[PF][UNR_W];
  float fw_gw[K];
  int fw_c = -1, fw_kind = 0;
  auto request_w = [&]() {
    if constexpr (PREF_W) {
      if (wave_id < fa.w.n_cg) {
        const int cg = wave_id;
        fw_c = perm_lds ? lchan[cg * 64 + lane] : fa.w.chan_perm[((size_t)blockIdx.x * fa.w.n_cg + cg) * 64 + lane];
        const float* gsrc = fa.w.gw_s + (size_t)(fw_c < 0 ? 0 : fw_c) * KP;
#pragma unroll
        for (int kk = 0; kk < K; ++kk) fw_gw[kk] = gsrc[kk];
        const int* off = meta + 3 * NGRP + 2 * cg;
        const int beg = off[0], mid = off[1], end = off[2];
        const uint32_t* lrow = fa.w.ell + (size_t)beg * 64 + lane;
        if (ell_walk_request<UNR_W, PF, STREAM>(lrow, mid - beg, fw_rows)) fw_kind = 1;
        else if (mid == beg && ell_walk_request<UNR_W, PF, STREAM>(lrow, end - mid, fw_rows)) fw_kind = 2;
      }
    }
  };
  h_epilogue<K, true, 0, ESPM_FUSED_SUM_BATCHED ? (FULL ? FusedGeom<K>::S_MAX : ESPM_FUSED_MAX_SEGS) : 0, PLAIN>(
      a, part, S, PB, blk0, 0.f, cs_lds, tab, PB, false,
      (PLAIN || fa.red_lds_off >= 0) ? reinterpret_cast<double*>(reinterpret_cast<unsigned char*>(smem) + fa.red_lds_off) : nullptr, relw, request_w,
      ukl, NGRP * S);

  ESPM_PHASE_STAMP(5);
  const WAccumArgs& w = fa.w;
  const int b = blockIdx.x;
  const bool w_split = !PLAIN && ESPM_FUSED_W_SPLIT && fa.w_split;
  const bool slab_lds = PLAIN || (ESPM_FUSED_SLAB_LDS && fa.slab_lds);
  const int w_units = w_split ? 2 * w.n_cg : w.n_cg;
  bool first_w = PREF_W;
  for (int wu = PREF_W ? wave_id : next_unit(1); wu < w_units; wu = next_unit(1), first_w = false) {
    const int cg = w_split ? wu >> 1 : wu, whalf = w_split ? wu & 1 : 0;
    const int c = (PREF_W && first_w) ? fw_c : (perm_lds ? lchan[cg * 64 + lane] : w.chan_perm[((size_t)b * w.n_cg + cg) * 64 + lane]);
    const float* gsrc = w.gw_s + (size_t)(c < 0 ? 0 : c) * KP;
    float gw[K], acc[K];
    if (PREF_W && first_w) {
#pragma unroll
      for (int kk = 0; kk < K; ++kk) gw[kk] = fw_gw[kk];
    } else {
#pragma unroll
      for (int kk = 0; kk < K; ++kk) gw[kk] = gsrc[kk];
    }
#pragma unroll
    for (int kk = 0; kk < K; ++kk) acc[kk] = 0.f;
    const int wkind = (PREF_W && first_w) ? fw_kind : 0;
    const int* off = meta + 3 * NGRP + 2 * cg;
    const int beg = off[0], mid = off[1], end = off[2];
    int u0 = beg, u1 = mid, g0 = mid, g1 = end;
    if (w_split) {
      const int hu = beg + (mid - beg) / 2, hg = mid + (end - mid) / 2;
      if (whalf == 0) {
        u1 = hu;
        g1 = hg;
      } else {
        u0 = hu;
        g0 = hg;
      }
    }
    const uint32_t* lrow = w.ell + (size_t)beg * 64 + lane;
    ell_walk_pre<K, UNR_W, PF, PRIO, STREAM, WALK_PP>(lrow + (size_t)(u0 - beg) * 64, u1 - u0, EllGetUnitFix<K>(PB), [&](float, const float (&h)[K]) {
      ell_axpy<K>(acc, h, __builtin_amdgcn_rcpf(ell_dot<K>(h, gw)));
    }, EllNoFlush(), wkind == 1, fw_rows);
    ell_walk_pre<K, UNR_W, PF, PRIO, STREAM, WALK_PP>(lrow + (size_t)(g0 - beg) * 64, g1 - g0, EllGetFix<K>(tab, PB, PBITS), [&](float x, const float (&h)[K]) {
      const float r = x * __builtin_amdgcn_rcpf(ell_dot<K>(h, gw));
      ell_axpy<K>(acc, h, r);
    }, EllNoFlush(), wkind == 2, fw_rows);
    if constexpr (PRIO > 0) __builtin_amdgcn_s_setprio(0);
    if (c >= 0) {
      if (slab_lds) {
        float* copy = part + (size_t)whalf * K * w.n_pad;
#pragma unroll
        for (int kk = 0; kk < K; ++kk) copy[(size_t)kk * w.n_pad + c] = acc[kk];
      } else {
#pragma unroll
        for (int kk = 0; kk < K; ++kk) w.a_slab[((size_t)b * K + kk) * w.n_pad + c] = acc[kk];
      }
    }
  }
  ESPM_PHASE_STAMP(6);
  ESPM_WAVE_STAMP(24);
  if (slab_lds) {
    __syncthreads();
    float* dst = w.a_slab + (size_t)b * K * w.n_pad;
    typedef float xf4 __attribute__((ext_vector_type(4)));
    for (int i = threadIdx.x; i < (K * w.n_pad) / 4; i += NT) {
      xf4 v = reinterpret_cast<const xf4*>(part)[i];
      if (w_split) v += reinterpret_cast<const xf4*>(part + (size_t)K * w.n_pad)[i];
      const int c0 = (4 * i) % w.n_pad;
      if (c0 + 3 >= a.n) {
        if (c0 >= a.n) v[0] = 0.f;
        if (c0 + 1 >= a.n) v[1] = 0.f;
        if (c0 + 2 >= a.n) v[2] = 0.f;
        v[3] = 0.f;
      }
#if ESPM_FUSED_SLAB_WT
      asm volatile("global_store_dwordx4 %0, %1, off sc0 sc1\n\ts_nop 1" : : "v"(dst + 4 * i), "v"(v) : "memory");
#else
      *reinterpret_cast<xf4*>(dst + 4 * i) = v;
#endif
    }
  }
#ifdef ESPM_PHASE_CLOCK
  __syncthreads();
  ESPM_PHASE_STAMP(7);
#endif
}

}
```

espm_amd/csrc/mu_h_kernel.hpp:

```cpp
#pragma once
#ifndef ESPM_HOUT_WRITE_THROUGH
#define ESPM_HOUT_WRITE_THROUGH 1
#endif
#ifndef ESPM_FUSED_RED_PACKED
#define ESPM_FUSED_RED_PACKED 1
#endif
#include "mu_common.hpp"
#include "mu_h_chain.hpp"

namespace espm {

template <int K>
struct LdsTabGeom {
  static constexpr int WB = K <= 4 ? 0 : (K == 5 ? 1 : (K == 6 ? 2 : (K <= 8 ? 4 : (K <= 12 ? 8 : 12))));
};
template <int K>
__device__ __forceinline__ void lds_table_put_row(float* tab, int rows, int r, const float* src) {
  constexpr int WB = LdsTabGeom<K>::WB;
  reinterpret_cast<float4*>(tab + (size_t)WB * rows)[r] = make_float4(src[0], K > 1 ? src[1] : 0.f, K > 2 ? src[2] : 0.f, K > 3 ? src[3] : 0.f);
  if constexpr (WB == 1) tab[r] = src[4];
  if constexpr (WB == 2) reinterpret_cast<float2*>(tab)[r] = make_float2(src[4], src[5]);
  if constexpr (WB >= 4) {
#pragma unroll
    for (int q = 0; q < WB / 4; ++q)
      reinterpret_cast<float4*>(tab)[(size_t)r * (WB / 4) + q] =
          make_float4(4 + 4 * q < K ? src[4 + 4 * q] : 0.f, 5 + 4 * q < K ? src[5 + 4 * q] : 0.f, 6 + 4 * q < K ? src[6 + 4 * q] : 0.f, 7 + 4 * q < K ? src[7 + 4 * q] : 0.f);
  }
}
template <int K>
__device__ __forceinline__ void lds_table_put(float* tab, int rows, int r, const float4 lo, const float4 hi) {
  static_assert(K >= 1, "");
  if constexpr (K <= 8) {
    const float src[8] = {lo.x, lo.y, lo.z, lo.w, hi.x, hi.y, hi.z, hi.w};
    lds_table_put_row<K>(tab, rows, r, src);
  }
}

#define ESPM_TAB2_BASE 32768
#ifndef ESPM_FIXTAB_MIN_K
#define ESPM_FIXTAB_MIN_K 6
#endif
template <int K>
struct FixTab {
  static constexpr bool TWO = K > 4;
  static constexpr bool FIXED = K >= ESPM_FIXTAB_MIN_K;
  static constexpr int MAX_ROWS = (TWO && FIXED) ? ESPM_TAB2_BASE / 16 : (1 << 30);
  __host__ __device__ static constexpr size_t bytes(int rows) {
    return (TWO && FIXED) ? (size_t)ESPM_TAB2_BASE + 16u * (size_t)rows : (size_t)(4 + LdsTabGeom<K>::WB) * 4u * (size_t)rows;
  }
  static __device__ __forceinline__ void put(float* tab, int rows, int r, const float4 lo, const float4 hi) {
    if constexpr (!(TWO && FIXED)) {
      lds_table_put<K>(tab, rows, r, lo, hi);
    } else {
      reinterpret_cast<float4*>(tab)[r] = lo;
      float* p2 = tab + ESPM_TAB2_BASE / 4 + 4 * (size_t)r;
      if constexpr (K == 5) p2[0] = hi.x;
      else if constexpr (K == 6) *reinterpret_cast<float2*>(p2) = make_float2(hi.x, hi.y);
      else *reinterpret_cast<float4*>(p2) = hi;
    }
  }
  static __device__ __forceinline__ void put_row(float* tab, int rows, int r, const float* src) {
    const float4 lo = *reinterpret_cast<const float4*>(src);
    float4 hi = make_float4(0.f, 0.f, 0.f, 0.f);
    if constexpr (TWO && KP > 4) hi = *reinterpret_cast<const float4*>(src + 4);
    put(tab, rows, r, lo, hi);
  }
};

template <int K>
struct HEpiIn {
  float hin[K], hprev[K];
  float l[K], r[K], u[K], d[K];
  float wl, wr, wu, wd;
};
template <int K, bool PLAIN = false>
__device__ __forceinline__ void h_epilogue_load(const HStepArgs& a, int q, bool stencil, HEpiIn<K>& v) {
#pragma unroll
  for (int kk = 0; kk < K; ++kk) {
    v.hin[kk] = a.h_in[(size_t)kk * a.p_pad + q];
    v.hprev[kk] = (PLAIN || a.have_prev) ? a.h_out[(size_t)kk * a.p_pad + q] : 0.f;
    v.l[kk] = v.r[kk] = v.u[kk] = v.d[kk] = 0.f;
  }
  v.wl = v.wr = v.wu = v.wd = 0.f;
  if (stencil) {
    const int i = q / a.ny, j = q - i * a.ny;
    v.wl = j > 0 ? 1.f : 0.f;
    v.wr = j < a.ny - 1 ? 1.f : 0.f;
    const bool up_in = i > 0, dn_in = i < a.nx - 1;
    v.wu = (up_in || a.halo_top) ? 1.f : 0.f;
    v.wd = (dn_in || a.halo_bot) ? 1.f : 0.f;
    const int ql = j > 0 ? q - 1 : q, qr = j < a.ny - 1 ? q + 1 : q;
#pragma unroll
    for (int kk = 0; kk < K; ++kk) {
      const float* hrow = a.h_in + (size_t)kk * a.p_pad;
      const float* pu = up_in ? hrow + (q - a.ny) : (a.halo_top ? a.halo_top + (size_t)kk * a.ny + j : hrow + q);
      const float* pd = dn_in ? hrow + (q + a.ny) : (a.halo_bot ? a.halo_bot + (size_t)kk * a.ny + j : hrow + q);
      v.l[kk] = hrow[ql];
      v.r[kk] = hrow[qr];
      v.u[kk] = *pu;
      v.d[kk] = *pd;
    }
  }
}

#ifndef ESPM_SIMPLEX_FAST_EXIT
#define ESPM_SIMPLEX_FAST_EXIT 1
#endif
#ifndef ESPM_SUM_ROW_FENCE
#define ESPM_SUM_ROW_FENCE 1
#endif
#ifndef ESPM_SUM_SWITCH
#define ESPM_SUM_SWITCH 1
#endif
struct HEpiNoHook {
  __device__ __forceinline__ void operator()() const {}
};
template <int K, bool EARLY = true, int RULE = 0, int MAXP = 0, bool PLAIN = false, typename Hook = HEpiNoHook, bool CHAIN = false>
__device__ __forceinline__ void h_epilogue(const HStepArgs& a, float* smem, int nparts, int TP, int tile0, float kl_lane,
                                           const double* colsum = nullptr,
                                           float* lds_tab = nullptr, int lds_rows = 0, bool kl_rows = false,
                                           double* red_scratch = nullptr,
                                           float relw_lane = -1.f, Hook after_pixels = Hook(),
                                           const float* unit_kl = nullptr, int n_unit_kl = 0, const ChainStats<K>* chain = nullptr, const double* chain_scr = nullptr) {
  constexpr int NRED = ESPM_HP_NSCALAR + 2 * K + 1;
  float red[NRED];
#pragma unroll
  for (int i = 0; i < NRED; ++i) red[i] = 0.f;
  constexpr int R_ROWSUM = 4, R_RELH = 4 + K, R_MAX = 5 + K, R_RELW = 5 + 2 * K;
  red[ESPM_HP_KL] = kl_lane;
  red[R_RELW] = relw_lane;
  double pg_q = 0.0;
  static_assert(!PLAIN || RULE == 0, "the plain instance: the default H rule");
  const bool f_fill = PLAIN ? false : a.fill_num != nullptr, f_breg = PLAIN ? false : a.breg_sr != nullptr, f_l2 = PLAIN ? false : a.l2_m != nullptr;
  const bool f_mu = a.mu != nullptr, f_fixed = PLAIN ? false : a.fixed_h != nullptr;
  const bool f_prev = PLAIN ? true : a.have_prev != 0, f_lap = PLAIN ? true : a.lambda_l != 0.f, f_grid = PLAIN ? true : a.grid_mode != 0;
  const bool f_write = PLAIN ? true : a.write_h != 0, f_simplex = PLAIN ? true : a.simplex_h != 0;
  const bool stencil = f_lap && f_grid;
  HEpiIn<K> in;
  bool loaded = false;
  if (EARLY && K <= 6 && (int)threadIdx.x < TP && tile0 + (int)threadIdx.x < a.p) {
    h_epilogue_load<K, PLAIN>(a, tile0 + (int)threadIdx.x, stencil, in);
    loaded = true;
  }
  const bool want_klc = kl_rows || f_fill || unit_kl != nullptr;
  float klc_first = 0.f;
  bool klc_loaded = false;
  if (want_klc && (int)threadIdx.x < TP && tile0 + (int)threadIdx.x < a.p) {
    klc_first = a.ell_klc[tile0 + (int)threadIdx.x];
    klc_loaded = true;
  }
  bool chained = false;
  if constexpr (CHAIN) chained = a.chain_prev != nullptr;
  float rel_shift = 0.f;
  if (f_prev && !chained) {
    double tot = 0.0;
#pragma unroll
    for (int kk = 0; kk < K; ++kk) tot += a.hstat_in[ESPM_HS_ROWSUM + kk];
    rel_shift = (float)((double)a.rel_tol * tot * a.inv_count);
  }
  float mhv[K];
#pragma unroll
  for (int kk = 0; kk < K; ++kk) mhv[kk] = (RULE == 0 && f_lap && !chained) ? (float)a.hstat_in[ESPM_HS_MAX + kk] : 0.f;
  if constexpr (CHAIN) {
    if (chained && !chain_scr) {
      if (f_prev) rel_shift = chain->rel_shift;
      if (RULE == 0 && f_lap) {
#pragma unroll
        for (int kk = 0; kk < K; ++kk) mhv[kk] = chain->mhv[kk];
      }
    }
  }
  __syncthreads();
  ESPM_PHASE_STAMP(3);
  if constexpr (CHAIN) {
    if (chained && chain_scr) {
      const ChainStats<K> late = chain_stats_combine<K>(a, chain_scr);
      if (f_prev) rel_shift = late.rel_shift;
      if (RULE == 0 && f_lap) {
#pragma unroll
        for (int kk = 0; kk < K; ++kk) mhv[kk] = late.mhv[kk];
      }
    }
  }

  auto emit_ht = [&](int q, int jj, const float (&ht)[KP]) {
    if (lds_tab) {
      float4 hi = make_float4(0.f, 0.f, 0.f, 0.f);
      if constexpr (KP > 4 && K > 4) hi = make_float4(ht[4], ht[5], ht[6], ht[7]);
      FixTab<K>::put(lds_tab, lds_rows, jj, make_float4(ht[0], ht[1], ht[2], ht[3]), hi);
    } else {
      store_row_kp(a.h_t + (size_t)q * KP, ht);
    }
  };
  const float ls = a.lambda_l * a.sigma_l;
  for (int jj = threadIdx.x; jj < TP; jj += (int)blockDim.x) {
    const int q = tile0 + jj;
    if (q >= a.p) {
      if (lds_tab) FixTab<K>::put(lds_tab, lds_rows, jj, make_float4(1.f, 1.f, 1.f, 1.f), make_float4(1.f, 1.f, 1.f, 1.f));
      continue;
    }
    if (!loaded) h_epilogue_load<K, PLAIN>(a, q, stencil, in);
    loaded = false;
    const float klc = klc_loaded ? klc_first : (want_klc ? a.ell_klc[q] : 0.f);
    klc_loaded = false;
    float hin[K], nv[K], dv[K];
    const int prows = kl_rows ? K + 1 : K;
    if constexpr (MAXP > 0) {
      auto row_sum_n = [&](auto nslots, int kk, float s) {
        constexpr int NS = decltype(nslots)::value;
        float pv[NS];
#pragma unroll
        for (int w = 0; w < NS; ++w) pv[w] = smem[((size_t)(w < nparts ? w : 0) * prows + kk) * TP + jj];
#pragma unroll
        for (int w = 0; w < NS; ++w) s += w < nparts ? pv[w] : 0.f;
#if ESPM_SUM_ROW_FENCE
        __builtin_amdgcn_sched_barrier(0);
#endif
        return s;
      };
      auto sum_rows = [&](auto nslots) {
        if (kl_rows) red[ESPM_HP_KL] += row_sum_n(nslots, K, fmaxf(klc, 0.f));
        else if (unit_kl) red[ESPM_HP_KL] += fmaxf(klc, 0.f);
#pragma unroll
        for (int kk = 0; kk < K; ++kk) nv[kk] = row_sum_n(nslots, kk, 0.f) * a.xscale;
      };
      if (ESPM_SUM_SWITCH && MAXP > 2 && nparts <= 2) sum_rows(std::integral_constant<int, 2>());
      else if (ESPM_SUM_SWITCH && MAXP > 4 && nparts <= 4) sum_rows(std::integral_constant<int, 4>());
      else sum_rows(std::integral_constant<int, MAXP>());
#pragma unroll
      for (int kk = 0; kk < K; ++kk) {
        hin[kk] = in.hin[kk];
        dv[kk] = (float)(colsum ? colsum[kk] : a.colsum_gw[kk]);
      }
    } else {
      if (kl_rows) {
        float s = fmaxf(klc, 0.f);
        for (int w = 0; w < nparts; ++w) s += smem[((size_t)w * prows + K) * TP + jj];
        red[ESPM_HP_KL] += s;
      } else if (unit_kl) {
        red[ESPM_HP_KL] += fmaxf(klc, 0.f);
      }
#pragma unroll
      for (int kk = 0; kk < K; ++kk) {
        float s = 0.f;
        for (int w = 0; w < nparts; ++w) s += smem[((size_t)w * prows + kk) * TP + jj];
        hin[kk] = in.hin[kk];
        nv[kk] = s * a.xscale;
        dv[kk] = (float)(colsum ? colsum[kk] : a.colsum_gw[kk]);
      }
    }
    ESPM_PHASE_STAMP(40);
    if (f_fill) {
      const float mark = klc;
      if (mark < 0.f) {
        const int idx = (int)(-mark) - 1;
#pragma unroll
        for (int kk = 0; kk < K; ++kk) nv[kk] += a.fill_num[(size_t)kk * a.fill_n + idx] * a.xscale;
      }
    }
    if (f_breg) {
      const float sr = a.xscale * a.breg_sr[q];
#pragma unroll
      for (int kk = 0; kk < K; ++kk) {
        const float t = sr * __builtin_amdgcn_rcpf(hin[kk]);
        dv[kk] = (dv[kk] - nv[kk]) + t;
        nv[kk] = t;
      }
    }
    if (f_l2) {
#pragma unroll
      for (int kk = 0; kk < K; ++kk) {
        float d = 0.f;
#pragma unroll
        for (int l = 0; l < K; ++l) d = fmaf(a.l2_m[kk * KP + l], hin[l], d);
        dv[kk] = d;
      }
    }
    if (f_prev) {
      float worst = 0.f;
#pragma unroll
      for (int kk = 0; kk < K; ++kk) worst = fmaxf(worst, fabsf(hin[kk] - in.hprev[kk]) * __builtin_amdgcn_rcpf(hin[kk] + rel_shift));
      red[R_RELH] = fmaxf(red[R_RELH], worst);
    }
    constexpr bool quad = RULE == 1;
    constexpr bool pgrad = RULE == 2;
    if (f_mu) {
#pragma unroll
      for (int kk = 0; kk < K; ++kk) {
        const float m = a.mu[kk];
        if (!quad) dv[kk] += m * __builtin_amdgcn_rcpf(hin[kk] + a.eps_reg);
        red[ESPM_HP_REG] += m * logf(hin[kk] + a.eps_reg);
      }
    }
    float hlv[K];
#pragma unroll
    for (int kk = 0; kk < K; ++kk) hlv[kk] = 0.f;
    if (f_lap) {
#pragma unroll
      for (int kk = 0; kk < K; ++kk) {
        const float hl = f_grid ? ((in.wl + in.wr) + (in.wu + in.wd)) * hin[kk] -
                                           (((in.wl * in.l[kk] + in.wr * in.r[kk]) + in.wu * in.u[kk]) + in.wd * in.d[kk])
                                     : hin[kk];
        hlv[kk] = hl;
        red[ESPM_HP_LAP] += hin[kk] * hl;
        if constexpr (RULE == 0) {
          const float mh = mhv[kk];
          nv[kk] += ls * mh;
          dv[kk] += ls * mh + a.lambda_l * hl;
        }
        if constexpr (pgrad) dv[kk] += a.lambda_l * hl;
      }
    }
    if (!f_write) continue;
    if constexpr (pgrad) {
      const float inv_gamma = __builtin_amdgcn_rcpf(a.sigma_l);
      float hg[K];
      float hmin = INFINITY;
#pragma unroll
      for (int kk = 0; kk < K; ++kk) {
        hg[kk] = hin[kk] - (dv[kk] - nv[kk]) * inv_gamma;
        hmin = fminf(hmin, hg[kk]);
      }
      float nu = 0.f;
      if (f_simplex) {
        nu = 1.f / (float)K - hmin;
        for (int it = 0; it < K + 2; ++it) {
          float f = -1.f, cnt = 0.f;
#pragma unroll
          for (int kk = 0; kk < K; ++kk) {
            const float t = hg[kk] + nu;
            if (t > a.log_shift) { f += t; cnt += 1.f; } else { f += a.log_shift; }
          }
// ... 279 lines not shown
```

espm_amd/ell.py:

```python
from __future__ import annotations

import torch

from . import _lib


def _split_counts(x, xmax):
    return (x + (xmax - 1)) // xmax


def _expand(idx_major, idx_minor, x, reps, xmax):
    if int(reps.max()) <= 1:
        return idx_major, idx_minor, x
    total = torch.repeat_interleave(reps)
    first = torch.cumsum(reps, 0) - reps
    pos = torch.arange(total.numel(), device=x.device) - first[total]
    r_e, x_e = reps[total], x[total]
    val = torch.where(pos < r_e - 1, torch.full_like(x_e, xmax), x_e - (r_e - 1) * xmax)
    return idx_major[total], idx_minor[total], val


def _store16(ell16, dword, half, value):
    v = value.to(torch.int32)
    v = torch.where(v >= 32768, v - 65536, v).to(torch.int16)
# ... 99 lines not shown
    if n > _lib.ELL_UNIT_MAX_N:
        ones_px = torch.zeros_like(ones_px)

    ngrp = p_pad // 64
    cnt_pad = torch.zeros(p_pad, dtype=torch.int64, device=dev)
    cnt_pad[:p] = per_px
    ones_pad = torch.zeros(p_pad, dtype=torch.int64, device=dev)
    ones_pad[:p] = ones_px
    pix_perm = torch.argsort(cnt_pad.view(-1, tile_px), dim=1, descending=True, stable=True)
    win0 = (torch.arange(p_pad, device=dev) // tile_px) * tile_px
    slot_pixel = win0 + pix_perm.reshape(-1)
    slot_of = torch.empty(p_pad, dtype=torch.int64, device=dev)
    slot_of[slot_pixel] = torch.arange(p_pad, device=dev)
    glen = cnt_pad[slot_pixel].view(ngrp, 64).max(dim=1).values
    gones = ones_pad[slot_pixel].view(ngrp, 64).min(dim=1).values
    gunit, ggen = _group_rows(glen, gones)
    h_off = _offsets(gunit, ggen)
    rows_h = int(h_off[-1])
    if rows_h * 64 >= 2 ** 31:
        raise ValueError("sparse count store: H lists exceed 2^31 dwords")
    ell_h = torch.zeros(max(rows_h, 1) * 64, **i32)
    ell_h16 = ell_h.view(torch.int16)
    klc = torch.zeros(p_pad, dtype=torch.float32, device=dev)
    xm = float(xmax_h)
    grp_of_px = slot_of >> 6
    for q0 in range(0, p, chunk):
        blk = Xpm[q0:q0 + chunk]
        xi = blk.to(torch.int64)
        xd = blk.to(torch.float64)
        nfull = torch.ceil(xd / xm).clamp_min(1.0) - 1.0
        rest = xd - nfull * xm
        klc[q0:q0 + blk.shape[0]] = (xd * torch.log2(xd.clamp_min(1.0)) - nfull * xm * float(torch.log2(torch.tensor(xm)))
                                     - rest * torch.log2(rest.clamp_min(1.0))).sum(dim=1).to(torch.float32)
        nz = xi.nonzero(as_tuple=False)
        if nz.numel() == 0:
            continue
        q, c = nz[:, 0], nz[:, 1]
        g = grp_of_px[q0:q0 + blk.shape[0]]
        _scatter_lists(ell_h16, q, c, xi[q, c], blk.shape[0], 2 * gunit[g], h_off[2 * g], h_off[2 * g + 1],
                       slot_of[q0:q0 + blk.shape[0]] & 63, xmax_h, cbits)

    cnt_bc = torch.zeros((nblk_w, n), dtype=torch.int64, device=dev)
    ones_bc = torch.zeros((nblk_w, n), dtype=torch.int64, device=dev)
    for b in range(nblk_w):
        xi = Xpm[b * PB:(b + 1) * PB].to(torch.int32)
        cnt_bc[b] = _split_counts(xi, xmax_w).sum(dim=0).to(torch.int64)
        ones_bc[b] = (xi == 1).sum(dim=0)
    order = torch.argsort(cnt_bc, dim=1, descending=True, stable=True)
    chan_perm = torch.full((nblk_w, n_cg * 64), -1, dtype=torch.int64, device=dev)
    chan_perm[:, :n] = order
    cnt_slot = torch.zeros((nblk_w, n_cg * 64), dtype=torch.int64, device=dev)
    cnt_slot[:, :n] = torch.gather(cnt_bc, 1, order)
    ones_slot = torch.zeros((nblk_w, n_cg * 64), dtype=torch.int64, device=dev)
    ones_slot[:, :n] = torch.gather(ones_bc, 1, order)
    wunit, wgen = _group_rows(cnt_slot.view(nblk_w, n_cg, 64).max(dim=2).values, ones_slot.view(nblk_w, n_cg, 64).min(dim=2).values)
    w_off = _offsets(wunit.reshape(-1), wgen.reshape(-1))
    rows_w = int(w_off[-1])
    if rows_w * 64 >= 2 ** 31:
        raise ValueError("sparse count store: W lists exceed 2^31 dwords")
    ell_w = torch.zeros(max(rows_w, 1) * 64, **i32)
    ell_w16 = ell_w.view(torch.int16)
    for b in range(nblk_w):
        xt = Xpm[b * PB:(b + 1) * PB].to(torch.int64).t().contiguous()
        nz = xt.nonzero(as_tuple=False)
        if nz.numel() == 0:
            continue
        c, pl = nz[:, 0], nz[:, 1]
        slot_of_c = torch.empty(n, dtype=torch.int64, device=dev)
        slot_of_c[order[b]] = torch.arange(n, device=dev)
        g = b * n_cg + (slot_of_c >> 6)
        _scatter_lists(ell_w16, c, pl, xt[c, pl], n, 2 * wunit.reshape(-1)[g], w_off[2 * g], w_off[2 * g + 1], slot_of_c & 63,
                       xmax_w, PBITS)

    out = dict(ell_h=ell_h, ell_h_off=h_off.to(torch.int32), klc=klc, pix_perm=pix_perm.reshape(-1).to(torch.int32), ell_w=ell_w, ell_w_off=w_off.to(torch.int32),
               chan_perm=chan_perm.to(torch.int32), n_cg=n_cg, nblk_w=nblk_w, nnz=nnz,
               entries_h=int(per_px.sum()), entries_w=int(per_ch.sum()), rows_h=rows_h, rows_w=rows_w,
               unit_rows_h=int(gunit.sum()), unit_rows_w=int(wunit.sum()))
    if hv is not None:
        out["hv"] = hv
        out["nnz"] += hv["n"]
    return out


def lds_bytes_h(n_pad, k):
    wb = 0 if k <= 4 else (1 if k == 5 else (2 if k == 6 else (4 if k <= 8 else (8 if k <= 12 else 12))))
    sets = 2 if k <= _lib.ELL_PAIR_MAX_K else 1
    kp = 8 if k <= 8 else 16
    return n_pad * (4 + wb) * 4 + max(sets * k * _lib.ELL_TILE * 4, 9 * (5 + 2 * k) * 8, (9 * (kp + 1) + 1) * 8)
```

espm_amd/engine.py:

```python
from __future__ import annotations

import contextlib
import ctypes as C
import os
import sys
import time

import numpy as np
import torch

from . import _lib
from ._lib import MUState
from .store import CODES, StoreFacts, choose_store

AUTOTUNE_MIN_ITERS = 5000


def _ptr(t):
    return C.c_void_p(t.data_ptr()) if t is not None else C.c_void_p(None)


def _stream():
    return C.c_void_p(torch.cuda.current_stream().cuda_stream)

# ... 173 lines not shown
            breg_px = Xd.sum(dim=ch_axis, dtype=torch.float64).to(torch.float32)
        return Xd, empty_ch, empty_px, x_facts, breg_px

    def _select_store(self, Xd, layout, x_store, x_facts, empty_ch, empty_px, log_shift, h_rule, pg_gamma_w, masks_given):
        group = self.group
        note, n_heavy, nnz, refill = None, 0, None, False
        if x_store in ("auto", "ell"):
            unfilled = (not self.bregman and ((empty_ch is not None and bool(empty_ch.any()))
                                              or (empty_px is not None and bool(empty_px.any()))))
            if unfilled:
                _set_lines(Xd, layout, empty_px, empty_ch, 0)
            heavy_on = os.environ.get("ESPM_ELL_HEAVY", "1") != "0"
            facts = _scan_x(Xd, None if unfilled else x_facts, heavy_on)
            n_heavy, nnz = facts.n_heavy, facts.nnz
            code, dense_code, note, warn = choose_store(self.n, self.p, self.k, x_store, facts, h_rule=h_rule, bregman=self.bregman,
                                                        pg_gamma_w=pg_gamma_w, heavy_on=heavy_on)
            if warn:
                import warnings
                warnings.warn("espm_amd: " + note, RuntimeWarning, stacklevel=4)
            flag = torch.tensor([code, dense_code], device=self.device, dtype=torch.int32)
            self._tick("storage type (integer counts, bf16-exact, density)")
            if group is not None:
                torch.distributed.all_reduce(flag, op=torch.distributed.ReduceOp.MIN, group=group)
            flag = flag[:1] if int(flag[0]) == 3 else flag.min().reshape(1)
            if unfilled and int(flag.item()) != 3:
                _set_lines(Xd, layout, empty_px, empty_ch, log_shift)
                flag.fill_(0)
            if x_store == "ell" and int(flag.item()) != 3:
                raise ValueError("x_store='ell' needs integer counts <= 2^24 (above 255: the default H rule, no Bregman variant, no "
                                 "projected-gradient W step), n <= 16384 and a GW table that fits in LDS (12- or 16-float rows from 9 components on)")
            refill = unfilled and int(flag.item()) == 3 and masks_given
            x_store = CODES[int(flag.item())]
        if int(h_rule) != 0 and x_store in ("u8", "bf16"):
            x_store = "f32"
        if x_store not in CODES:
            raise ValueError("x_store must be 'auto', 'ell', 'u8', 'bf16' or 'f32'")
        return x_store, note, n_heavy, nnz, refill

    def _geometry(self, shape_2d, tile_px, x_tile):
        p, x_store = self.p, self.x_store
        st = MUState()
        st.n, st.p, st.k = self.n, p, self.k
        st.x_dtype = {"u8": _lib.X_U8, "bf16": _lib.X_BF16, "f32": _lib.X_F32, "ell": _lib.X_ELL}[x_store]
        if shape_2d is not None:
            nx, ny = int(shape_2d[0]), int(shape_2d[1])
            if nx * ny != p:
                raise ValueError(f"shape_2d {shape_2d} does not match the {p} pixels of X")
            st.nx, st.ny, st.grid_mode = nx, ny, 1
        else:
            st.nx, st.ny, st.grid_mode = 0, 0, 0
        self._check(self.lib.espm_mu_query(C.byref(st)))
        force_tile = tile_px if tile_px is not None else (int(os.environ["ESPM_FORCE_ELL_TILE"]) if os.environ.get("ESPM_FORCE_ELL_TILE") else None)
        if x_store == "ell" and force_tile in (64, 128, 256, 512):
            st.tile_px = st.x_tile = int(force_tile)
            st.ell_pb = 2 * st.tile_px
            st.nblk_w = (p + st.ell_pb - 1) // st.ell_pb
        if x_store != "ell":
            if tile_px is not None:
                st.tile_px = int(tile_px)
                st.x_tile = int(tile_px)
            if x_tile is not None:
                st.x_tile = int(x_tile)
        p_total = torch.tensor([p], dtype=torch.int64, device=self.device)
        if self.group is not None:
            torch.distributed.all_reduce(p_total, group=self.group)
        st.p_total = int(p_total.item())
        self.p_total = st.p_total
        return st

    def _build_store(self, Xd, layout, n_heavy, nnz, empty_px):
        st, dev, k = self.st, self.device, self.k
        self.ell = None
        self.fill_px = self.fill_num = None
        torch_builder = self.x_store == "ell" and os.environ.get("ESPM_ELL_BUILDER", "hip") == "torch"
        if not torch_builder:
            Xc = Xd.contiguous()
            src = (_ptr(Xc), _lib.SRC_F64 if Xc.dtype == torch.float64 else _lib.SRC_F32, _lib.LAYOUT_PM if layout == "pm" else _lib.LAYOUT_CM,
                   Xc.shape[1])
        if self.x_store == "ell":
            from . import ell as _ell
            self.x_cm = self.x_pm = None
            if torch_builder:
                self.ell = _ell.build(Xd if layout == "pm" else Xd.t(), st.p_pad, st.ell_cbits, st.tile_px)
            else:
                self.ell = self._build_ell(src, n_heavy, nnz)
                self._tick("sparse store build")
            assert self.ell["n_cg"] == st.n_cg and self.ell["nblk_w"] == st.nblk_w
            fill_n = 0
            if empty_px is not None and bool(empty_px.any()):
                idx = torch.nonzero(empty_px).flatten()
                if idx.numel() >= 1 << 24:
                    raise NotImplementedError("more than 2^24 pixels without counts")
                fill_n = idx.numel()
                self.fill_px = idx.to(torch.int32).contiguous()
                self.ell["klc"][idx] = -(torch.arange(idx.numel(), device=dev, dtype=torch.float32) + 1.0)
            hv = self.ell.get("hv")
            npx = hv["npx"] if hv is not None else 0
            if hv is not None:
                if fill_n + npx >= 1 << 24:
                    raise NotImplementedError("more than 2^24 pixels without counts or with counts above 255")
                hpx = hv["px"].long()
                self.hv_klc = self.ell["klc"][hpx].clone()
                self.hv_kl = torch.zeros(npx, dtype=torch.float64, device=dev)
                self.ell["klc"][hpx] = -(torch.arange(npx, device=dev, dtype=torch.float32) + float(fill_n + 1))
            if fill_n + npx > 0:
                self.fill_num = torch.zeros((k, fill_n + npx), dtype=torch.float32, device=dev)
            self.x_bytes = 4 * (self.ell["ell_h"].numel() + self.ell["ell_w"].numel()) + (16 * hv["n"] if hv is not None else 0)
        else:
            xt = {"u8": torch.uint8, "bf16": torch.bfloat16, "f32": torch.float32}[self.x_store]
            self.x_cm = torch.empty((st.p_pad // st.x_tile, st.n_cm, st.x_tile), dtype=xt, device=dev)
            self.x_pm = torch.empty((self.p, st.n_pad), dtype=xt, device=dev)
            self._check(self.lib.espm_mu_pack_x(*src, self.n, self.p, _ptr(self.x_cm), _ptr(self.x_pm), st.x_dtype, st.n_pad, st.p_pad,
                                                st.x_tile, st.n_cm, _stream()))
            self.x_bytes = self.x_cm.numel() * self.x_cm.element_size() + self.x_pm.numel() * self.x_pm.element_size()

    def _ingest_G(self, G):
        st, dev = self.st, self.device
        if G is not None:
            Gh = np.ascontiguousarray(np.asarray(G, dtype=np.float32))
            if Gh.ndim != 2 or Gh.shape[0] != self.n:
                raise ValueError(f"G must be (n={self.n}, m), got {Gh.shape}")
            self.m = Gh.shape[1]
            self.g = torch.from_numpy(Gh).to(dev)
            self.g_t = torch.zeros((self.m, st.n_pad), dtype=torch.float32, device=dev)
            self.g_t[:, :self.n] = self.g.t()
            self.colsum_g = torch.from_numpy(np.asarray(G, dtype=np.float64).sum(axis=0).astype(np.float32)).to(dev)
            st.m = self.m
        else:
            self.m, self.g, self.colsum_g, self.g_t = 0, None, None, None
            st.m = 0
        self.M = self.m if self.m > 0 else self.n

    def _set_hyper_parameters(self, *, simplex_H, simplex_W, compute_loss, lambda_L, sigmaL, h_rule, pg_gamma_w, epsilon_reg, log_shift,
                              dicotomy_tol, tol, xscale, gw_floor, mu):
        st = self.st
        st.simplex_h, st.simplex_w = int(bool(simplex_H)), int(bool(simplex_W))
        st.compute_loss = int(bool(compute_loss))
        st.lambda_l, st.sigma_l = float(lambda_L), float(sigmaL)
        st.h_rule = int(h_rule)
        st.pg_gamma_w = float(pg_gamma_w)
        st.eps_reg, st.log_shift = float(epsilon_reg), float(log_shift)
        st.dicotomy_tol, st.rel_tol = float(dicotomy_tol), float(tol)
        self.rel_tol = float(tol)
        st.xscale, st.gw_floor = float(xscale), float(gw_floor)
        self.lambda_L, self.xscale = float(lambda_L), float(xscale)
        mu_arr = np.asarray(mu, dtype=np.float64)
        if mu_arr.ndim == 0 and float(mu_arr) == 0.0:
            self.mu = None
        else:
            self.mu = torch.from_numpy(np.broadcast_to(mu_arr, (self.k,)).astype(np.float32).copy()).to(self.device)

    def _allocate(self, max_iter, fixed_H, fixed_W, simplex_rows, simplex_W, log_shift, breg_px, with_pg_q):
        st, dev, k = self.st, self.device, self.k
        f32 = dict(dtype=torch.float32, device=dev)
        f64 = dict(dtype=torch.float64, device=dev)
        self.w = [torch.zeros((self.M, k), **f32) for _ in range(2)]
        self.h = [torch.ones((k, st.p_pad), **f32) for _ in range(2)]
        self.h_t = torch.zeros((self.p, self.V.KP), **f32)
        self.gw_s = torch.zeros((st.n_pad, self.V.KP), **f32)
        self.colsum_gw = torch.zeros(self.V.KP, **f64)
        nblk_h = (self.p + st.tile_px - 1) // st.tile_px
        self.hpart = torch.zeros((nblk_h, self.V.HP_STRIDE), **f64)
        self.hpart_alt = torch.zeros_like(self.hpart)
        self.hstat = [torch.zeros(self.V.HS_STRIDE, **f64) for _ in range(2)]
        self._tick("rest up to the state buffers")
        self.a_slab = torch.zeros((st.nblk_w, k, st.n_pad), **f32)
        self.a = torch.zeros((k, st.n_pad), **f32)
        self.w_scratch = torch.zeros((2, self.M, k), **f32)
        self.hist_len = int(max_iter) + 3
        self.hist = torch.zeros((self.hist_len, _lib.HI_STRIDE), **f64)
        self.frob = torch.zeros(self.hist_len, **f64) if self.frobenius else None
        self.fixed_h = self._pad_h(fixed_H) if fixed_H is not None else None
        self.fixed_w = (torch.from_numpy(np.ascontiguousarray(np.asarray(fixed_W, dtype=np.float32))).to(dev)
                        if fixed_W is not None else None)
        if simplex_rows is not None:
            mask = np.zeros(self.M, dtype=np.int32)
            mask[np.asarray(simplex_rows)] = 1
            self.simplex_rows = torch.from_numpy(mask).to(dev)
            if log_shift > 0 and simplex_W and mask.sum() * log_shift >= 1:
                raise ValueError("No solution exists!")
        else:
            self.simplex_rows = None
        if self.bregman:
            self.breg_px = torch.zeros(st.p_pad, **f32)
            self.breg_px[:self.p] = breg_px
        self.pg_q = torch.zeros((self.hist_len, 2), **f64) if with_pg_q else None

    def _bind(self):
        st = self.st
        if self.ell is None:
            st.x_cm, st.x_pm = self.x_cm.data_ptr(), self.x_pm.data_ptr()
        else:
            st.x_cm = st.x_pm = None
            st.ell_h, st.ell_h_off, st.ell_klc = (self.ell[key].data_ptr() for key in ("ell_h", "ell_h_off", "klc"))
            if self.fill_px is not None:
                st.ell_fill_px, st.ell_fill_n = self.fill_px.data_ptr(), int(self.fill_px.numel())
            if self.fill_num is not None:
                st.ell_fill_num = self.fill_num.data_ptr()
            hv = self.ell.get("hv")
            if hv is not None:
                st.ell_hv_n, st.ell_hv_npx, st.ell_hv_ngrp = hv["n"], hv["npx"], hv["ngrp"]
                st.ell_hv_px, st.ell_hv_px_off, st.ell_hv_pm = (hv[key].data_ptr() for key in ("px", "px_off", "pm"))
                st.ell_hv_grp, st.ell_hv_grp_off, st.ell_hv_wm = (hv[key].data_ptr() for key in ("grp", "grp_off", "wm"))
                st.ell_hv_klc, st.ell_hv_kl = self.hv_klc.data_ptr(), self.hv_kl.data_ptr()
            st.ell_w, st.ell_w_off, st.chan_perm = (self.ell[key].data_ptr() for key in ("ell_w", "ell_w_off", "chan_perm"))
            st.pix_perm = self.ell["pix_perm"].data_ptr()
        st.g = self.g.data_ptr() if self.g is not None else None
        st.g_t = self.g_t.data_ptr() if self.g_t is not None else None
        st.colsum_g = self.colsum_g.data_ptr() if self.colsum_g is not None else None
        st.w[0], st.w[1] = self.w[0].data_ptr(), self.w[1].data_ptr()
        st.h[0], st.h[1] = self.h[0].data_ptr(), self.h[1].data_ptr()
        st.gw_s, st.colsum_gw, st.h_t = self.gw_s.data_ptr(), self.colsum_gw.data_ptr(), self.h_t.data_ptr()
        st.gw_a, st.gw_p = None, None
        st.mu = self.mu.data_ptr() if self.mu is not None else None
        st.fixed_h = self.fixed_h.data_ptr() if self.fixed_h is not None else None
        st.fixed_w = self.fixed_w.data_ptr() if self.fixed_w is not None else None
        st.simplex_rows = self.simplex_rows.data_ptr() if self.simplex_rows is not None else None
        st.halo_top = st.halo_bot = None
        if self.bregman:
            st.breg_sr_px, st.breg_sr_ch = self.breg_px.data_ptr(), self._breg_ch.data_ptr()
        else:
            st.breg_sr_px = st.breg_sr_ch = None
        st.hpart = self.hpart.data_ptr()
        st.hpart_alt = self.hpart_alt.data_ptr() if os.environ.get("ESPM_H_CHAIN", "0") == "1" else None
        st.hstat[0], st.hstat[1] = self.hstat[0].data_ptr(), self.hstat[1].data_ptr()
        st.a_slab, st.a, st.w_scratch = self.a_slab.data_ptr(), self.a.data_ptr(), self.w_scratch.data_ptr()
        st.hist, st.hist_len = self.hist.data_ptr(), self.hist_len
        st.pg_q = self.pg_q.data_ptr() if self.pg_q is not None else None
        st.cur, st.it = 0, 0
        self._pending_finalize = None
        self._pending_tail = False
        self._accum_done = False

    def _launch_policy(self, fused, autotune, max_iter):
        st = self.st
        if os.environ.get("ESPM_FUSED"):
            fused = {"0": False, "1": True}.get(os.environ["ESPM_FUSED"], os.environ["ESPM_FUSED"])
        st.no_fused = {"static": 2, "always": 3}.get(fused, 0 if fused else 1)
        limit = float(os.environ["ESPM_ELL_STREAM_MB"]) * 2 ** 20 if os.environ.get("ESPM_ELL_STREAM_MB") else _lib.ELL_STREAM_BYTES
        st.ell_stream = int(self.x_store == "ell" and self.x_bytes > limit)
        self._autotune = (int(max_iter) >= AUTOTUNE_MIN_ITERS) if autotune == "auto" else bool(autotune)
        self.plan_timings = None

    def _build_ell(self, src, n_heavy, nnz):
        st, dev = self.st, self.device
        i32 = dict(dtype=torch.int32, device=dev)
        x8 = torch.empty((self.p, st.n_pad), dtype=torch.uint8, device=dev)
        x8c = torch.empty((st.p_pad // _lib.PPAD, st.n_cm, _lib.PPAD), dtype=torch.uint8, device=dev) if os.environ.get("ESPM_ELL_BUILD_CM") != "0" else None
        self._check(self.lib.espm_mu_pack_x(*src, self.n, self.p, _ptr(x8c) if x8c is not None else None, _ptr(x8), _lib.X_U8, st.n_pad,
                                            st.p_pad, _lib.PPAD, st.n_cm, _stream()))
        hv = None
        if n_heavy:
            hv_cnt = torch.empty(self.p, **i32)
            self._check(self.lib.espm_mu_ell_heavy_count(C.byref(st), *src, _ptr(x8), _ptr(x8c) if x8c is not None else None, _ptr(hv_cnt),
                                                         _stream()))
            hv_off = torch.zeros(self.p + 1, **i32)
            hv_off[1:] = torch.cumsum(hv_cnt, 0)
            n_hv = int(hv_off[-1])
            if n_hv:
                pm = torch.empty((n_hv, 2), **i32)
                self._check(self.lib.espm_mu_ell_heavy_fill(C.byref(st), *src, _ptr(hv_off), _ptr(pm), _stream()))
                q = torch.repeat_interleave(torch.arange(self.p, device=dev), hv_cnt.long())
                from . import ell as _ell
                hv = _ell.heavy_orders(q, pm[:, 0].long(), pm[:, 1].long(), self.n, st.ell_pb)
        cnt_px = torch.empty((2, st.p_pad), **i32)
        cnt_bc = torch.empty((2, st.nblk_w, st.n_cg * 64), **i32)
        klc = torch.empty(st.p_pad, dtype=torch.float32, device=dev)
        hist = os.environ.get("ESPM_ELL_BUILD_HIST") != "0"
        bkt_px = torch.empty((st.p_pad, _lib.ELL_BUCKETS), dtype=torch.uint8, device=dev) if hist else None
        bkt_bc = torch.empty((st.nblk_w, st.n_cg * 64, _lib.ELL_BUCKETS), dtype=torch.uint8, device=dev) if hist else None
        self._check(self.lib.espm_mu_ell_count_hist(C.byref(st), _ptr(x8), _ptr(cnt_px), _ptr(cnt_bc), _ptr(klc),
                                                    _ptr(bkt_px) if hist else None, _ptr(bkt_bc) if hist else None, _stream()))
        chan_perm = torch.empty((st.nblk_w, st.n_cg * 64), **i32)
        pix_perm = torch.empty(st.p_pad, **i32)
        h_off = torch.empty(2 * (st.p_pad // 64) + 1, **i32)
        w_off = torch.empty(2 * st.nblk_w * st.n_cg + 1, **i32)
        rows = torch.zeros(2, dtype=torch.int64, device=dev)
        self._check(self.lib.espm_mu_ell_plan(C.byref(st), _ptr(cnt_px), _ptr(cnt_bc), _ptr(chan_perm), _ptr(pix_perm), _ptr(h_off),
                                   _ptr(w_off), _ptr(rows), _stream()))
        rows_h, rows_w = (int(v) for v in rows.cpu())
        if max(rows_h, rows_w) * 64 >= 2 ** 31:
            raise ValueError("sparse count store: the lists exceed 2^31 dwords")
        ell_h = torch.zeros(max(rows_h, 1) * 64, **i32)
        ell_w = torch.zeros(max(rows_w, 1) * 64, **i32)
        st.x_cm = x8c.data_ptr() if x8c is not None else None
        try:
            self._check(self.lib.espm_mu_ell_fill_hist(C.byref(st), _ptr(x8), _ptr(chan_perm), _ptr(pix_perm), _ptr(h_off), _ptr(w_off),
                                                       _ptr(ell_h), _ptr(ell_w), _ptr(bkt_px) if hist else None, _ptr(bkt_bc) if hist else None, _stream()))
        finally:
            st.x_cm = None
        torch.cuda.current_stream().synchronize()
        out = dict(ell_h=ell_h, ell_h_off=h_off, klc=klc, pix_perm=pix_perm, ell_w=ell_w, ell_w_off=w_off, chan_perm=chan_perm, n_cg=st.n_cg,
                   nblk_w=st.nblk_w, nnz=nnz, entries_h=int(cnt_px[0].sum()), entries_w=int(cnt_bc[0].sum()), rows_h=rows_h,
                   rows_w=rows_w, unit_rows_h=int((h_off[1::2] - h_off[0:-1:2]).sum()),
                   unit_rows_w=int((w_off[1::2] - w_off[0:-1:2]).sum()))
        if hv is not None:
            out["hv"] = hv
        return out

    def _pad_h(self, H):
        Hh = np.asarray(H, dtype=np.float32)
        if Hh.shape != (self.k, self.p):
            raise ValueError(f"expected an array of shape {(self.k, self.p)}, got {Hh.shape}")
        out = torch.full((self.k, self.st.p_pad), -1.0, dtype=torch.float32, device=self.device)
        out[:, :self.p] = torch.from_numpy(np.ascontiguousarray(Hh)).to(self.device)
        return out

    def load_state(self, W, H):
        st = self.st

        def as_f32(a, shape, name):
            if isinstance(a, torch.Tensor):
                t = a.to(device=self.device, dtype=torch.float32)
            else:
                t = torch.from_numpy(np.ascontiguousarray(np.asarray(a, dtype=np.float32)))
            if tuple(t.shape) != shape:
                raise ValueError(f"{name} must be {shape}, got {tuple(t.shape)}")
            return t
        Wt = as_f32(W, (self.M, self.k), "W")
        Ht = as_f32(H, (self.k, self.p), "H")
        st.cur, st.it = 0, 0
        self._pending_finalize = None
        self._pending_tail = False
        self._accum_done = False
        self.hist.zero_()
        self.w[0].copy_(Wt)
        self.h[0][:, :self.p].copy_(Ht)
        self._check(self.lib.espm_mu_build_gw(C.byref(st), 0, _stream()))
        self._check(self.lib.espm_mu_hstat(C.byref(st), 0, _stream()))
        if self.sharded:
            self._globalize_hstat(0)
            self._exchange_halo_only(0)
        if self._autotune:
            self._autotune = False
            self.autotune_plan()

    PLANS = {0: "fused, units handed out dynamically", 2: "fused, fixed unit assignment", 1: "H-step and W accumulation as two launches"}

    def autotune_plan(self, iters=48, warm=4):
        st = self.st
        if self.sharded or self.frobenius or self.ell is None:
            return None
        keep = st.no_fused
        st.no_fused = 0
        if not bool(self.lib.espm_mu_fused_applies(C.byref(st))):
            st.no_fused = keep
            return None
        iters = int(os.environ.get("ESPM_AUTOTUNE_ITERS", iters))
        iters = min(iters, self.hist_len - st.it - 2 - warm)
        if iters < 4:
            st.no_fused = keep
            return None
        tensors = [self.w[0], self.w[1], self.h[0], self.h[1], self.gw_s, self.colsum_gw, self.hstat[0], self.hstat[1], self.hist,
                   self.w_scratch, self.hpart]
        saved = [t.clone() for t in tensors]
        state = (st.cur, st.it)

        def restore():
            for t, sv in zip(tensors, saved):
                t.copy_(sv)
            st.cur, st.it = state
        rounds = 3
        per = max(iters // rounds, 2)
        st.no_fused = 0
        self._check(self.lib.espm_mu_iterate(C.byref(st), min(2 * iters, self.hist_len - st.it - 2), 0, _stream()))
        restore()
        total = {plan: 0.0 for plan in self.PLANS}
        for _ in range(rounds):
            for plan in self.PLANS:
                st.no_fused = plan
                self._check(self.lib.espm_mu_iterate(C.byref(st), min(warm, 2), 0, _stream()))
                e0, e1 = torch.cuda.Event(enable_timing=True), torch.cuda.Event(enable_timing=True)
                e0.record()
                self._check(self.lib.espm_mu_iterate(C.byref(st), per, 0, _stream()))
                e1.record()
# ... 429 lines not shown
```

include/espm_mu.h:

```cpp
#ifndef ESPM_MU_H
#define ESPM_MU_H

#include <stddef.h>
#include <stdint.h>

#ifdef __cplusplus
extern "C" {
#endif

typedef void* espm_stream_t;

typedef enum espm_status {
  ESPM_OK = 0,
  ESPM_EINVAL = -1,
  ESPM_ENOSOLUTION = -2,
  ESPM_EHIP = -3,
  ESPM_EUNSUPPORTED = -4
} espm_status;

enum { ESPM_X_F32 = 0, ESPM_X_BF16 = 1, ESPM_X_U8 = 2 ,
       ESPM_X_ELL = 3  };
enum { ESPM_SRC_F32 = 0, ESPM_SRC_F64 = 1 };
enum { ESPM_LAYOUT_CM = 0 , ESPM_LAYOUT_PM = 1  };

#ifndef ESPM_KP
#define ESPM_KP 8
#endif
#ifndef ESPM_MAX_K
#define ESPM_MAX_K ESPM_KP
#endif
#ifndef ESPM_MIN_K
#define ESPM_MIN_K 1
#endif
#define ESPM_PPAD 512
#define ESPM_NPAD 8
#define ESPM_ELL_TILE 512
#define ESPM_ELL_PB 1024
#define ESPM_ELL_PBITS 10
#define ESPM_ELL_UNIT_ROWS 8
#define ESPM_ELL_UNIT_MAX_N 4080
#define ESPM_ELL_PAIR_MAX_K 6
#define ESPM_ELL_STREAM_BYTES (256 << 20)
#define ESPM_FUSED_MIN_PB 512
#define ESPM_FUSED_MIN_BLOCKS 192
#define ESPM_ELL_HEAVY_MIN 256
#define ESPM_ELL_HEAVY_MAX (1 << 24)
#define ESPM_ELL_WTHREADS 1024
#ifndef ESPM_ELL_BUCKETS
#define ESPM_ELL_BUCKETS 16
#endif
#define ESPM_ELL_LDS_MAX (160 * 1024)
#define ESPM_NCM 16
#define ESPM_W_DICOTOMY_TOL 1e-5f
#define ESPM_TAIL_DEFER 1
#define ESPM_TAIL_RIDE 2

#define ESPM_HP_KL 0
#define ESPM_HP_REG 1
#define ESPM_HP_LAP 2
#define ESPM_HP_BAD 3
#define ESPM_HP_ROWSUM 4
#define ESPM_HP_MAX (4 + ESPM_KP)
#define ESPM_HP_RELH (4 + 2 * ESPM_KP)
#define ESPM_HP_PGQ (5 + 2 * ESPM_KP)
#define ESPM_HP_RELW (6 + 2 * ESPM_KP)
#define ESPM_HP_NSCALAR 5
#define ESPM_HP_STRIDE (8 + 2 * ESPM_KP)

#define ESPM_HS_ROWSUM 0
#define ESPM_HS_MAX ESPM_KP
#define ESPM_HS_STRIDE (2 * ESPM_KP)

#define ESPM_HI_KLX 0
#define ESPM_HI_REG 1
#define ESPM_HI_LAP 2
#define ESPM_HI_SUMY 3
#define ESPM_HI_BAD 4
#define ESPM_HI_REL_W 5
#define ESPM_HI_REL_H 6
#define ESPM_HI_STRIDE 8

#define ESPM_MU_ABI_VERSION 6

typedef struct espm_mu_state {
  uint32_t struct_size;
  uint32_t abi_version;
  int32_t n;
  int32_t m;
  int32_t k;
  int32_t p;
  int32_t nx, ny;
  int32_t n_pad;
  int32_t p_pad;
  int32_t x_dtype;
  int32_t tile_px;
  int32_t nblk_w;
  int32_t x_tile;
  int32_t n_cm;
  int32_t h_variant;
  int64_t p_total;
  int32_t simplex_h, simplex_w;
  int32_t grid_mode;
  int32_t compute_loss;
  float lambda_l, sigma_l, eps_reg, log_shift, dicotomy_tol, rel_tol;
  float xscale;
  float gw_floor;
  const void* x_cm;
  const void* x_pm;
  const float* g;
  const float* colsum_g;
  float* w[2];
  float* gw_s;
  double* colsum_gw;
  void* gw_a;
  float* gw_p;
  float* h[2];
  float* h_t;
  const float* mu;
  const float* fixed_h;
  const float* fixed_w;
  const int32_t* simplex_rows;
  const float* halo_top;
  const float* halo_bot;
  double* hpart;
  double* hstat[2];
  float* a_slab;
  float* a;
  float* w_scratch;
  double* hist;
  int32_t hist_len;
  int32_t cur;
  int32_t it;
  const uint32_t* ell_h;
  const int32_t* ell_h_off;
  const float* ell_klc;
  const uint32_t* ell_w;
  const int32_t* ell_w_off;
  const int32_t* chan_perm;
  int32_t ell_cbits;
  int32_t n_cg;
  const int32_t* pix_perm;
  const float* g_t;
  const float* breg_sr_px;
  const float* breg_sr_ch;
  int32_t h_rule;
  float pg_gamma_w;
  double* pg_q;
  const int32_t* ell_fill_px;
  float* ell_fill_num;
  int32_t ell_fill_n;
  int32_t tail_mode;
  int32_t no_fused;
  int32_t ell_pb;
  int32_t ell_stream;
  int32_t ell_hv_n;
  int32_t ell_hv_npx;
  int32_t ell_hv_ngrp;
  const int32_t* ell_hv_px;
  const int32_t* ell_hv_px_off;
  const int32_t* ell_hv_pm;
  const float* ell_hv_klc;
  double* ell_hv_kl;
  const int32_t* ell_hv_grp;
  const int32_t* ell_hv_grp_off;
  const int32_t* ell_hv_wm;
  double* hpart_alt;
} espm_mu_state;

const char* espm_mu_version(void);
const char* espm_mu_last_error(void);
size_t espm_mu_state_size(void);
int espm_mu_abi_version(void);
const char* espm_mu_state_layout(void);

int espm_mu_query(espm_mu_state* st);

int espm_mu_pack_x(const void* src, int src_dtype, int src_layout, int64_t ld, int n, int p,
                   void* x_cm, void* x_pm, int x_dtype, int n_pad, int p_pad, int x_tile, int n_cm,
                   espm_stream_t stream);

int espm_mu_ell_count(const espm_mu_state* st, const void* x_pm_u8, int32_t* cnt_px, int32_t* cnt_bc, float* ell_klc,
                      espm_stream_t stream);
int espm_mu_ell_count_hist(const espm_mu_state* st, const void* x_pm_u8, int32_t* cnt_px, int32_t* cnt_bc, float* ell_klc, uint8_t* bkt_px,
                           uint8_t* bkt_bc, espm_stream_t stream);
int espm_mu_ell_fill_hist(const espm_mu_state* st, const void* x_pm_u8, const int32_t* chan_perm, const int32_t* pix_perm,
                          const int32_t* ell_h_off, const int32_t* ell_w_off, uint32_t* ell_h, uint32_t* ell_w, const uint8_t* bkt_px,
                          const uint8_t* bkt_bc, espm_stream_t stream);
int espm_mu_ell_plan(const espm_mu_state* st, const int32_t* cnt_px, const int32_t* cnt_bc, int32_t* chan_perm,
                     int32_t* pix_perm, int32_t* ell_h_off, int32_t* ell_w_off, int64_t* rows, espm_stream_t stream);
int espm_mu_ell_fill(const espm_mu_state* st, const void* x_pm_u8, const int32_t* chan_perm, const int32_t* pix_perm,
                     const int32_t* ell_h_off, const int32_t* ell_w_off, uint32_t* ell_h, uint32_t* ell_w,
                     espm_stream_t stream);
int espm_mu_ell_heavy_count(const espm_mu_state* st, const void* x, int src_dtype, int src_layout, int64_t ld, uint8_t* x_pm_u8,
                            uint8_t* x_cm_u8, int32_t* cnt_px, espm_stream_t stream);
int espm_mu_ell_heavy_fill(const espm_mu_state* st, const void* x, int src_dtype, int src_layout, int64_t ld, const int32_t* px_off,
                           int32_t* hv_pm, espm_stream_t stream);

int espm_mu_hstat(const espm_mu_state* st, int which, espm_stream_t stream);

int espm_mu_build_gw(const espm_mu_state* st, int which, espm_stream_t stream);

int espm_mu_step_h(const espm_mu_state* st, int src, int write_h, espm_stream_t stream);

int espm_mu_h_finalize(const espm_mu_state* st, int src, int slot, espm_stream_t stream);

int espm_mu_loss_only(const espm_mu_state* st, int src, int slot, espm_stream_t stream);

int espm_mu_w_accum(const espm_mu_state* st, espm_stream_t stream);
int espm_mu_step_hw(const espm_mu_state* st, int src, espm_stream_t stream);
int espm_mu_fused_applies(const espm_mu_state* st);
int espm_mu_w_reduce(const espm_mu_state* st, espm_stream_t stream);
int espm_mu_w_reduce_finalize(const espm_mu_state* st, int src, int slot, espm_stream_t stream);
int espm_mu_w_finish(const espm_mu_state* st, int src, int hsrc, int slot, espm_stream_t stream);

int espm_mu_w_reduce_finish(const espm_mu_state* st, int src, int slot, int with_finalize, espm_stream_t stream);

int espm_mu_iterate(espm_mu_state* st, int n_iter, int final_loss, espm_stream_t stream);
int espm_mu_iterate_h(espm_mu_state* st, int n_iter, int final_loss, espm_stream_t stream);
int espm_mu_h_chain_applies(const espm_mu_state* st);
int espm_mu_w_update_is_local(const espm_mu_state* st);
int espm_mu_w_update_tail(const espm_mu_state* st, int src, int slot, espm_stream_t stream);

size_t espm_mu_shard_record_bytes(const espm_mu_state* st);
int espm_mu_shard_pack(const espm_mu_state* st, int hnew, void* record, espm_stream_t stream);
int espm_mu_w_reduce_pack(const espm_mu_state* st, int src, int slot, void* record, espm_stream_t stream);
int espm_mu_shard_combine(const espm_mu_state* st, const void* records, int world, int hnew,
                          espm_stream_t stream);
int espm_mu_shard_combine_finish(const espm_mu_state* st, const void* records, int world, int src, int slot,
                                 espm_stream_t stream);

typedef struct espm_xchg espm_xchg;
#define ESPM_XCHG_HANDLE_BYTES 64
int espm_xchg_create(int world, int rank, size_t record_bytes, espm_xchg** out);
int espm_xchg_handle(const espm_xchg* x, void* handle_out );
int espm_xchg_connect(espm_xchg* x, const void* handles );
void* espm_xchg_staging(const espm_xchg* x);
const void* espm_xchg_records(const espm_xchg* x, int parity);
int espm_xchg_post(espm_xchg* x, uint32_t seq, espm_stream_t stream);
int espm_xchg_wait(espm_xchg* x, uint32_t seq, espm_stream_t stream);
int espm_xchg_timeouts(const espm_xchg* x, uint32_t* count_out);
int espm_xchg_set_order(espm_xchg* x, int release);
int espm_xchg_order(const espm_xchg* x);
int espm_xchg_destroy(espm_xchg* x);

int espm_mu_shard_exchange_finish(const espm_mu_state* st, espm_xchg* x, uint32_t seq, int src, int slot, espm_stream_t stream);

int espm_mu_iterate_timed(espm_mu_state* st, int n_iter, float* first_ms, float* rest_ms, espm_stream_t stream);

int espm_mu_iterate_sharded(espm_mu_state* st, espm_xchg* x, uint32_t* seq, int n_iter, int final_loss, espm_stream_t stream);

int espm_dichotomy_simplex(const double* num, const double* den, int k, int p, int den_cols,
                           double log_shift, double tol, int maxit, double* nu_out,
                           int32_t* status_out, espm_stream_t stream);

int espm_simplex_root_f32(const float* num, const float* den, int k, int p, float log_shift, float tol, int maxit, int fast_exit,
                          float* delta_out, float* e_out, int32_t* status_out, espm_stream_t stream);

int espm_dichotomy_simplex_acc(double a, const double* b, const double* minus_c, int k, int p, int b_cols, double log_shift,
                               double tol, int maxit, double* nu_out, int32_t* status_out, espm_stream_t stream);
int espm_dichotomy_simplex_pg(const double* a, int k, int p, double log_shift, double tol, int maxit, double* nu_out,
                              espm_stream_t stream);

int espm_mu_l2_step_h(const espm_mu_state* st, int src, float* work, double* scratch, int scratch_doubles, espm_stream_t stream);
int espm_mu_l2_step_w(const espm_mu_state* st, int src, const float* gtg, float* work, double* scratch, int scratch_doubles,
                      espm_stream_t stream);
// ... 99 lines not shown
```

Before: 7641 it/s.

## Store k=5 ELL tables with an implicit last component normalized by row sum

For k=5 in the plain fused path, each LDS table row is divided by its row sum, so only four floats are stored and the fifth component is implied. Dot products and axpys then work on K-1 differences plus a constant, and the fifth accumulator is recovered from the sum. This drops the second LDS read per entry and some FMAs in the inner loops. The KL loss is corrected with per-block channel counts times log2 of the row sums, which needs a new precomputed block-count buffer, an ABI bump and extra build work. The rearrangement changes rounding slightly and handles degenerate rows with a fallback.

```diff
diff --git a/espm_amd/_lib.py b/espm_amd/_lib.py
--- a/espm_amd/_lib.py
+++ b/espm_amd/_lib.py
@@ -64,6 +64,7 @@
     "espm_mu_w_update_tail": (C.c_int, [_SP, C.c_int, C.c_int, _vp]),
     "espm_mu_pack_x": (C.c_int, [_vp, C.c_int, C.c_int, _i64, C.c_int, C.c_int, _vp, _vp, C.c_int, C.c_int, C.c_int, C.c_int, C.c_int, _vp]),
     "espm_mu_ell_count": (C.c_int, [_SP, _vp, _vp, _vp, _vp, _vp]),
+    "espm_mu_ell_block_counts": (C.c_int, [_SP, _vp, _vp, _vp]),
     "espm_mu_ell_count_hist": (C.c_int, [_SP, _vp, _vp, _vp, _vp, _vp, _vp, _vp]),
     "espm_mu_ell_fill_hist": (C.c_int, [_SP, _vp, _vp, _vp, _vp, _vp, _vp, _vp, _vp, _vp, _vp]),
     "espm_mu_ell_plan": (C.c_int, [_SP, _vp, _vp, _vp, _vp, _vp, _vp, _vp, _vp]),
diff --git a/espm_amd/csrc/mu_api.hip b/espm_amd/csrc/mu_api.hip
--- a/espm_amd/csrc/mu_api.hip
+++ b/espm_amd/csrc/mu_api.hip
@@ -33,7 +33,7 @@
   F(ell_h_off) F(ell_klc) F(ell_w) F(ell_w_off) F(chan_perm) F(ell_cbits) F(n_cg) F(pix_perm) F(g_t) F(breg_sr_px) \
   F(breg_sr_ch) F(h_rule) F(pg_gamma_w) F(pg_q) F(ell_fill_px) F(ell_fill_num) F(ell_fill_n) F(tail_mode) F(no_fused) \
   F(ell_pb) F(ell_stream) F(ell_hv_n) F(ell_hv_npx) F(ell_hv_ngrp) F(ell_hv_px) F(ell_hv_px_off) F(ell_hv_pm) F(ell_hv_klc) F(ell_hv_kl) \
-  F(ell_hv_grp) F(ell_hv_grp_off) F(ell_hv_wm) F(hpart_alt)
+  F(ell_hv_grp) F(ell_hv_grp_off) F(ell_hv_wm) F(hpart_alt) F(ell_blk_cnt)
 
 static int check_abi(const espm_mu_state* st) {
   ESPM_REQUIRE(st != nullptr, "state is NULL");
diff --git a/espm_amd/csrc/mu_common.hpp b/espm_amd/csrc/mu_common.hpp
--- a/espm_amd/csrc/mu_common.hpp
+++ b/espm_amd/csrc/mu_common.hpp
@@ -600,6 +600,7 @@
   const int32_t* ell_off;
   const float* ell_klc;
   const int32_t* ell_pix;
+  const float* ell_blk_cnt;
   int ell_bits, n_pad;
   int ell_tp;
   const float* l2_m;
@@ -810,6 +811,7 @@
   a.ell_off = st->ell_h_off;
   a.ell_klc = st->ell_klc;
   a.ell_pix = st->pix_perm;
+  a.ell_blk_cnt = st->ell_blk_cnt;
   a.ell_bits = st->ell_cbits;
   a.ell_tp = st->tile_px;
   a.l2_m = nullptr;
diff --git a/espm_amd/csrc/mu_ell_build.hip b/espm_amd/csrc/mu_ell_build.hip
--- a/espm_amd/csrc/mu_ell_build.hip
+++ b/espm_amd/csrc/mu_ell_build.hip
@@ -426,6 +426,17 @@
   return rc ? rc : rc2;
 }
 
+__global__ __launch_bounds__(256) void ell_block_counts_kernel(const uint8_t* __restrict__ x_pm, int n, int n_pad, int p, int pb, float* __restrict__ out) {
+  const int b = blockIdx.x, c = blockIdx.y * 256 + threadIdx.x;
+  if (c >= n_pad) return;
+  int sum = 0;
+  if (c < n) {
+    const int q0 = b * pb, q1 = min(p, q0 + pb);
+    for (int q = q0; q < q1; ++q) sum += x_pm[(size_t)q * n_pad + c];
+  }
+  out[(size_t)b * n_pad + c] = (float)sum;
+}
+
 int launch_ell_plan(const int32_t* cnt_px, const int32_t* cnt_bc, int n, int n_cg, int nblk, int p_pad, int win,
                     int32_t* chan_perm, int32_t* pix_perm, int32_t* h_off, int32_t* w_off, long long* rows, hipStream_t stream) {
   const size_t lds = (size_t)(n > win ? n : win) * sizeof(int32_t);
@@ -458,3 +469,17 @@
 }
 
 }
+
+extern "C" int espm_mu_ell_block_counts(const espm_mu_state* st, const void* x_pm_u8, float* blk_cnt, espm_stream_t stream) {
+  using namespace espm;
+  ESPM_REQUIRE(st != nullptr, "state is NULL");
+  ESPM_REQUIRE(st->struct_size == (uint32_t)sizeof(espm_mu_state) && st->abi_version == (uint32_t)ESPM_MU_ABI_VERSION,
+               "espm_mu_state of %u bytes, ABI %u handed to a library built for %zu bytes, ABI %d", st->struct_size, st->abi_version,
+               sizeof(espm_mu_state), ESPM_MU_ABI_VERSION);
+  ESPM_REQUIRE(st->x_dtype == ESPM_X_ELL && st->n >= 1 && st->p >= 1 && st->n_pad >= st->n && st->ell_pb >= 128 && st->nblk_w == (st->p + st->ell_pb - 1) / st->ell_pb,
+               "ell_block_counts: set x_dtype = ESPM_X_ELL and call espm_mu_query first");
+  ESPM_REQUIRE(x_pm_u8 && blk_cnt, "ell_block_counts: NULL pointer");
+  hipLaunchKernelGGL(ell_block_counts_kernel, dim3(st->nblk_w, (st->n_pad + 255) / 256), dim3(256), 0, static_cast<hipStream_t>(stream),
+                     static_cast<const uint8_t*>(x_pm_u8), st->n, st->n_pad, st->p, st->ell_pb, blk_cnt);
+  return check_hip(hipGetLastError(), "ell_block_counts launch");
+}
diff --git a/espm_amd/csrc/mu_ell_kernel.hpp b/espm_amd/csrc/mu_ell_kernel.hpp
--- a/espm_amd/csrc/mu_ell_kernel.hpp
+++ b/espm_amd/csrc/mu_ell_kernel.hpp
@@ -109,6 +109,38 @@
     acc[2 * q + 1] = t.y;
   }
   if constexpr (K & 1) acc[K - 1] = fmaf(g[K - 1], r, acc[K - 1]);
+}
+
+template <int K, bool IMPL>
+__device__ __forceinline__ float ell_dot_i(const float (&g)[K], const float (&h)[K]) {
+  if constexpr (!IMPL) {
+    return ell_dot<K>(g, h);
+  } else {
+    float y = h[K - 1];
+#pragma unroll
+    for (int i = 0; i < K - 1; ++i) y = fmaf(g[i], h[i], y);
+    return y;
+  }
+}
+template <int K, bool IMPL>
+__device__ __forceinline__ void ell_axpy_i(float (&acc)[K], const float (&g)[K], float r) {
+  if constexpr (!IMPL) {
+    ell_axpy<K>(acc, g, r);
+  } else {
+#pragma unroll
+    for (int q = 0; q < (K - 1) / 2; ++q) {
+      const f2 t = f2{g[2 * q], g[2 * q + 1]} * r + f2{acc[2 * q], acc[2 * q + 1]};
+      acc[2 * q] = t.x;
+      acc[2 * q + 1] = t.y;
+    }
+    if constexpr ((K - 1) & 1) acc[K - 2] = fmaf(g[K - 2], r, acc[K - 2]);
+    acc[K - 1] += r;
+  }
+}
+template <int K>
+__device__ __forceinline__ void ell_implicit_lane(float (&v)[K]) {
+#pragma unroll
+  for (int i = 0; i < K - 1; ++i) v[i] -= v[K - 1];
 }
 
 struct EllNoFlush {
@@ -273,8 +305,9 @@
   }
 };
 
-template <int K>
+template <int K, bool IMPL = false>
 struct EllGetUnitFix {
+  static_assert(!IMPL || K == 5, "the implicit last component: one float4 per row");
   static constexpr bool FIXED = FixTab<K>::TWO && FixTab<K>::FIXED;
   uint32_t lds_q;
   __device__ __forceinline__ EllGetUnitFix(int rows = 0) : lds_q((uint32_t)(EllTab<K>::WB * rows) * 4u) {}
@@ -282,6 +315,7 @@
     const lds_v4f lo = *(ESPM_LDS(lds_v4f))(uintptr_t)off;
 #pragma unroll
     for (int i = 0; i < (K < 4 ? K : 4); ++i) g[i] = lo[i];
+    if constexpr (IMPL) return;
     if constexpr (K == 5) g[4] = *(ESPM_LDS(float))(uintptr_t)(off + ESPM_TAB2_BASE);
     if constexpr (K == 6) {
       const lds_v2f v = *(ESPM_LDS(lds_v2f))(uintptr_t)(off + ESPM_TAB2_BASE);
@@ -296,12 +330,12 @@
     }
   }
   __device__ __forceinline__ float operator()(uint32_t e, int half, float (&g)[K]) const {
-    if constexpr (FIXED || K <= 4) row(half ? e >> 16 : e & 0xffffu, g);
+    if constexpr (FIXED || K <= 4 || IMPL) row(half ? e >> 16 : e & 0xffffu, g);
     else EllTab<K>::get_unit(lds_q, half ? e >> 16 : e & 0xffffu, g);
     return 1.f;
   }
 };
-template <int K>
+template <int K, bool IMPL = false>
 struct EllGetFix {
   const float* tab;
   int rows, idx_bits;
@@ -309,60 +343,60 @@
   __device__ __forceinline__ EllGetFix(const float* t, int r, int bits) : tab(t), rows(r), idx_bits(bits), mask((1u << bits) - 1u) {}
   __device__ __forceinline__ float operator()(uint32_t e, int half, float (&g)[K]) const {
     const uint32_t v = half ? e >> 16 : e & 0xffffu;
-    if constexpr (EllGetUnitFix<K>::FIXED || K <= 4) EllGetUnitFix<K>::row((v & mask) << 4, g);
+    if constexpr (EllGetUnitFix<K>::FIXED || K <= 4 || IMPL) EllGetUnitFix<K, IMPL>::row((v & mask) << 4, g);
     else EllTab<K>::get(tab, rows, v & mask, g);
     return (float)(v >> idx_bits);
   }
 };
-template <int K, bool FIX>
+template <int K, bool FIX, bool IMPL = false>
 struct EllGetters {
   typedef EllGetUnit<K> Unit;
   typedef EllGet<K> General;
 };
-template <int K>
-struct EllGetters<K, true> {
-  typedef EllGetUnitFix<K> Unit;
-  typedef EllGetFix<K> General;
+template <int K, bool IMPL>
+struct EllGetters<K, true, IMPL> {
+  typedef EllGetUnitFix<K, IMPL> Unit;
+  typedef EllGetFix<K, IMPL> General;
 };
 
 #ifndef ESPM_ELL_KLPROD
 #define ESPM_ELL_KLPROD 1
 #endif
-template <int K, bool LOSS, int UNR, int PF, int PRIO = 0, bool STREAM = false, bool FIX = false, bool PP = false>
+template <int K, bool LOSS, int UNR, int PF, int PRIO = 0, bool STREAM = false, bool FIX = false, bool PP = false, bool IMPL = false>
 __device__ __forceinline__ void ell_h_rows(const uint32_t* lrow, int x0, int x1, int mid, const float* tab, int n_pad, int ell_bits,
                                            const float (&hk)[K], float (&acc)[K], float& kl) {
   if (x0 < mid) {
     if constexpr (LOSS && ESPM_ELL_KLPROD) {
       float prod = 1.f;
-      ell_walk<K, UNR, PF, PRIO, STREAM, PP>(lrow + (size_t)x0 * 64, min(x1, mid) - x0, typename EllGetters<K, FIX>::Unit(n_pad),
+      ell_walk<K, UNR, PF, PRIO, STREAM, PP>(lrow + (size_t)x0 * 64, min(x1, mid) - x0, typename EllGetters<K, FIX, IMPL>::Unit(n_pad),
         [&](float, const float (&g)[K]) {
-          const float r = __builtin_amdgcn_rcpf(ell_dot<K>(g, hk));
-          ell_axpy<K>(acc, g, r);
+          const float r = __builtin_amdgcn_rcpf(ell_dot_i<K, IMPL>(g, hk));
+          ell_axpy_i<K, IMPL>(acc, g, r);
           prod *= r;
         },
         [&](auto redo) {
           const bool ok = __builtin_amdgcn_classf(prod, 0x100);
           if (__builtin_expect(__builtin_amdgcn_ballot_w64(!ok) != 0, 0)) {
-            redo([&](float, const float (&g)[K]) { kl += __builtin_amdgcn_logf(__builtin_amdgcn_rcpf(ell_dot<K>(g, hk))); });
+            redo([&](float, const float (&g)[K]) { kl += __builtin_amdgcn_logf(__builtin_amdgcn_rcpf(ell_dot_i<K, IMPL>(g, hk))); });
           } else {
             kl += __builtin_amdgcn_logf(prod);
           }
           prod = 1.f;
         });
     } else {
-      ell_walk<K, UNR, PF, PRIO, STREAM, PP>(lrow + (size_t)x0 * 64, min(x1, mid) - x0, typename EllGetters<K, FIX>::Unit(n_pad), [&](float, const float (&g)[K]) {
-        const float r = __builtin_amdgcn_rcpf(ell_dot<K>(g, hk));
-        ell_axpy<K>(acc, g, r);
+      ell_walk<K, UNR, PF, PRIO, STREAM, PP>(lrow + (size_t)x0 * 64, min(x1, mid) - x0, typename EllGetters<K, FIX, IMPL>::Unit(n_pad), [&](float, const float (&g)[K]) {
+        const float r = __builtin_amdgcn_rcpf(ell_dot_i<K, IMPL>(g, hk));
+        ell_axpy_i<K, IMPL>(acc, g, r);
         if constexpr (LOSS) kl += __builtin_amdgcn_logf(r);
       });
     }
   }
   if (x1 > mid) {
     const int g0 = max(x0, mid);
-    ell_walk<K, UNR, PF, PRIO, STREAM, PP>(lrow + (size_t)g0 * 64, x1 - g0, typename EllGetters<K, FIX>::General(tab, n_pad, ell_bits), [&](float x, const float (&g)[K]) {
-      const float y = ell_dot<K>(g, hk);
+    ell_walk<K, UNR, PF, PRIO, STREAM, PP>(lrow + (size_t)g0 * 64, x1 - g0, typename EllGetters<K, FIX, IMPL>::General(tab, n_pad, ell_bits), [&](float x, const float (&g)[K]) {
+      const float y = ell_dot_i<K, IMPL>(g, hk);
       const float r = LOSS ? fmaf(x, __builtin_amdgcn_rcpf(y), 1e-37f) : x * __builtin_amdgcn_rcpf(y);
-      ell_axpy<K>(acc, g, r);
+      ell_axpy_i<K, IMPL>(acc, g, r);
       if constexpr (LOSS) kl = fmaf(x, __builtin_amdgcn_logf(r), kl);
     });
   }
diff --git a/espm_amd/csrc/mu_fused.hip b/espm_amd/csrc/mu_fused.hip
--- a/espm_amd/csrc/mu_fused.hip
+++ b/espm_amd/csrc/mu_fused.hip
@@ -147,6 +147,8 @@
                        args.h.simplex_h && args.h.lambda_l != 0.f && args.h.grid_mode && args.h.have_prev && args.h.write_h && args.h.h_rule == 0 &&
                        args.h.tail_on != 1 && !args.static_units && args.slab_lds && !args.w_split && args.red_lds_off >= 0 && staged_ok &&
                        (args.perm_lds != 0) == (pb != ESPM_ELL_PB) && ESPM_FUSED_SMALL_THREADS == ESPM_ELL_WTHREADS;
+    if (plain) ESPM_REQUIRE(!(EllImplicit<K>::ON && args.h.compute_loss) || args.h.ell_blk_cnt,
+                            "fused half-steps at %d components with the loss: espm_mu_state.ell_blk_cnt is missing (espm_mu_ell_block_counts)", K);
     if (plain && args.stream_lists && pb == ESPM_ELL_PB) return launch_fused_plain_stream(args, K, args.h.compute_loss != 0, true, nblk, bytes, stream);
     if (plain) return launch_fused_plain(args, K, args.h.compute_loss != 0, pb == ESPM_ELL_PB, nblk, bytes, stream);
   }
diff --git a/espm_amd/csrc/mu_fused_kernel.hpp b/espm_amd/csrc/mu_fused_kernel.hpp
--- a/espm_amd/csrc/mu_fused_kernel.hpp
+++ b/espm_amd/csrc/mu_fused_kernel.hpp
@@ -112,6 +112,7 @@
   const int TP = PB / 2;
   const int GPT_SHIFT = PBITS - 7;
   constexpr int PROWS = FusedGeom<K>::PROWS;
+  constexpr bool IMPL = EllImplicit<K>::ON && PLAIN;
   constexpr bool S_RT = FULL && FusedGeom<K>::S_MAX > FusedGeom<K>::S;
   const int S = (FULL && !S_RT) ? FusedGeom<K>::S : fa.h_segs;
   constexpr int PF = FULL ? ESPM_FUSED_FULL_PREFETCH : ESPM_FUSED_SMALL_PREFETCH;
@@ -150,18 +151,22 @@
   constexpr bool PREF_W = PLAIN && !FULL && K <= 6 && ESPM_FUSED_FIRST_PREFETCH != 0;
   const int wave_id = __builtin_amdgcn_readfirstlane((int)(threadIdx.x >> 6));
   bool staged = false;
+  float kl_corr = 0.f;
+  const float* blk_cnt = (IMPL && LOSS) ? a.ell_blk_cnt + (size_t)blockIdx.x * a.n_pad : nullptr;
   if constexpr (ESPM_FUSED_PROLOGUE_BATCH) {
     constexpr int TR = 4, PC = 4;
     const int n_perm = perm_lds ? PB + 64 * fa.w.n_cg : 0, n_woff = 2 * fa.w.n_cg + 1;
     staged = PLAIN || (a.n_pad <= TR * NT && n_perm <= PC * NT && n_woff <= NT && a.cs_nbk <= 64 && 2 * K <= NT / 64);
     if (staged) {
       float4 tlo[TR], thi[TR];
+      float tcnt[TR];
 #pragma unroll
       for (int i = 0; i < TR; ++i) {
         const int r = threadIdx.x + i * NT;
         const float* src = a.gw_s + (size_t)min(r, a.n_pad - 1) * KP;
         tlo[i] = *reinterpret_cast<const float4*>(src);
         thi[i] = K > 4 ? *reinterpret_cast<const float4*>(src + 4) : make_float4(0.f, 0.f, 0.f, 0.f);
+        if constexpr (IMPL && LOSS) tcnt[i] = blk_cnt[min(r, a.n_pad - 1)];
       }
       int pv[PC];
 #pragma unroll
@@ -193,7 +198,10 @@
 #pragma unroll
       for (int i = 0; i < TR; ++i) {
         const int r = threadIdx.x + i * NT;
-        if (r < a.n_pad) FixTab<K>::put(tab, a.n_pad, r, tlo[i], thi[i]);
+        if (r < a.n_pad) {
+          const float lg = FixTab<K>::template put<IMPL>(tab, a.n_pad, r, tlo[i], thi[i]);
+          if constexpr (IMPL && LOSS) kl_corr = fmaf(tcnt[i], lg, kl_corr);
+        }
       }
 #pragma unroll
       for (int i = 0; i < PC; ++i) {
@@ -289,8 +297,9 @@
         float hk[K];
 #pragma unroll
         for (int kk = 0; kk < K; ++kk) hk[kk] = a.h_in[(size_t)kk * a.p_pad + px];
+        if constexpr (IMPL) ell_implicit_lane<K>(hk);
         const uint32_t* lrow = a.ell + (size_t)beg * 64 + lane;
-        ell_h_rows<K, LOSS, UNR_H, PF, PRIO, STREAM, true, WALK_PP>(lrow, x0, x1, mid, tab, a.n_pad, a.ell_bits, hk, acc, kl);
+        ell_h_rows<K, LOSS, UNR_H, PF, PRIO, STREAM, true, WALK_PP, IMPL>(lrow, x0, x1, mid, tab, a.n_pad, a.ell_bits, hk, acc, kl);
         if constexpr (PRIO > 0) __builtin_amdgcn_s_setprio(0);
       }
     }
@@ -325,8 +334,8 @@
       }
     }
   };
-  h_epilogue<K, true, 0, ESPM_FUSED_SUM_BATCHED ? (FULL ? FusedGeom<K>::S_MAX : ESPM_FUSED_MAX_SEGS) : 0, PLAIN>(
-      a, part, S, PB, blk0, 0.f, cs_lds, tab, PB, false,
+  h_epilogue<K, true, 0, ESPM_FUSED_SUM_BATCHED ? (FULL ? FusedGeom<K>::S_MAX : ESPM_FUSED_MAX_SEGS) : 0, PLAIN, decltype(request_w), false, IMPL>(
+      a, part, S, PB, blk0, -kl_corr, cs_lds, tab, PB, false,
       (PLAIN || fa.red_lds_off >= 0) ? reinterpret_cast<double*>(reinterpret_cast<unsigned char*>(smem) + fa.red_lds_off) : nullptr, relw, request_w,
       ukl, NGRP * S);
 
@@ -349,6 +358,7 @@
 #pragma unroll
       for (int kk = 0; kk < K; ++kk) gw[kk] = gsrc[kk];
     }
+    if constexpr (IMPL) ell_implicit_lane<K>(gw);
 #pragma unroll
     for (int kk = 0; kk < K; ++kk) acc[kk] = 0.f;
     const int wkind = (PREF_W && first_w) ? fw_kind : 0;
@@ -366,14 +376,20 @@
       }
     }
     const uint32_t* lrow = w.ell + (size_t)beg * 64 + lane;
-    ell_walk_pre<K, UNR_W, PF, PRIO, STREAM, WALK_PP>(lrow + (size_t)(u0 - beg) * 64, u1 - u0, EllGetUnitFix<K>(PB), [&](float, const float (&h)[K]) {
-      ell_axpy<K>(acc, h, __builtin_amdgcn_rcpf(ell_dot<K>(h, gw)));
+    ell_walk_pre<K, UNR_W, PF, PRIO, STREAM, WALK_PP>(lrow + (size_t)(u0 - beg) * 64, u1 - u0, EllGetUnitFix<K, IMPL>(PB), [&](float, const float (&h)[K]) {
+      ell_axpy_i<K, IMPL>(acc, h, __builtin_amdgcn_rcpf(ell_dot_i<K, IMPL>(h, gw)));
     }, EllNoFlush(), wkind == 1, fw_rows);
-    ell_walk_pre<K, UNR_W, PF, PRIO, STREAM, WALK_PP>(lrow + (size_t)(g0 - beg) * 64, g1 - g0, EllGetFix<K>(tab, PB, PBITS), [&](float x, const float (&h)[K]) {
-      const float r = x * __builtin_amdgcn_rcpf(ell_dot<K>(h, gw));
-      ell_axpy<K>(acc, h, r);
+    ell_walk_pre<K, UNR_W, PF, PRIO, STREAM, WALK_PP>(lrow + (size_t)(g0 - beg) * 64, g1 - g0, EllGetFix<K, IMPL>(tab, PB, PBITS), [&](float x, const float (&h)[K]) {
+      const float r = x * __builtin_amdgcn_rcpf(ell_dot_i<K, IMPL>(h, gw));
+      ell_axpy_i<K, IMPL>(acc, h, r);
     }, EllNoFlush(), wkind == 2, fw_rows);
     if constexpr (PRIO > 0) __builtin_amdgcn_s_setprio(0);
+    if constexpr (IMPL) {
+      float low = acc[0];
+#pragma unroll
+      for (int kk = 1; kk < K - 1; ++kk) low += acc[kk];
+      acc[K - 1] = fmaxf(acc[K - 1] - low, 0.f);
+    }
     if (c >= 0) {
       if (slab_lds) {
         float* copy = part + (size_t)whalf * K * w.n_pad;
diff --git a/espm_amd/csrc/mu_h_kernel.hpp b/espm_amd/csrc/mu_h_kernel.hpp
--- a/espm_amd/csrc/mu_h_kernel.hpp
+++ b/espm_amd/csrc/mu_h_kernel.hpp
@@ -40,6 +40,14 @@
 #ifndef ESPM_FIXTAB_MIN_K
 #define ESPM_FIXTAB_MIN_K 6
 #endif
+#ifndef ESPM_ELL_IMPLICIT_K
+#define ESPM_ELL_IMPLICIT_K 5
+#endif
+static_assert(ESPM_ELL_IMPLICIT_K == 0 || ESPM_ELL_IMPLICIT_K == 5, "the implicit last component: built and measured for k = 5");
+template <int K>
+struct EllImplicit {
+  static constexpr bool ON = K == ESPM_ELL_IMPLICIT_K;
+};
 template <int K>
 struct FixTab {
   static constexpr bool TWO = K > 4;
@@ -48,15 +56,25 @@
   __host__ __device__ static constexpr size_t bytes(int rows) {
     return (TWO && FIXED) ? (size_t)ESPM_TAB2_BASE + 16u * (size_t)rows : (size_t)(4 + LdsTabGeom<K>::WB) * 4u * (size_t)rows;
   }
-  static __device__ __forceinline__ void put(float* tab, int rows, int r, const float4 lo, const float4 hi) {
-    if constexpr (!(TWO && FIXED)) {
+  template <bool IMPL = false>
+  static __device__ __forceinline__ float put(float* tab, int rows, int r, const float4 lo, const float4 hi) {
+    if constexpr (IMPL) {
+      static_assert(EllImplicit<K>::ON, "the implicit last component: ESPM_ELL_IMPLICIT_K components");
+      const float s = (((lo.x + lo.y) + lo.z) + lo.w) + hi.x;
+      const bool ok = s > 0.f && s <= 3.0e38f;
+      const float d = ok ? s : 1.f;
+      reinterpret_cast<float4*>(tab)[r] = ok ? make_float4(lo.x / d, lo.y / d, lo.z / d, lo.w / d) : make_float4(0.2f, 0.2f, 0.2f, 0.2f);
+      return ok ? log2f(s) : 0.f;
+    } else if constexpr (!(TWO && FIXED)) {
       lds_table_put<K>(tab, rows, r, lo, hi);
+      return 0.f;
     } else {
       reinterpret_cast<float4*>(tab)[r] = lo;
       float* p2 = tab + ESPM_TAB2_BASE / 4 + 4 * (size_t)r;
       if constexpr (K == 5) p2[0] = hi.x;
       else if constexpr (K == 6) *reinterpret_cast<float2*>(p2) = make_float2(hi.x, hi.y);
       else *reinterpret_cast<float4*>(p2) = hi;
+      return 0.f;
     }
   }
   static __device__ __forceinline__ void put_row(float* tab, int rows, int r, const float* src) {
@@ -115,7 +133,7 @@
 struct HEpiNoHook {
   __device__ __forceinline__ void operator()() const {}
 };
-template <int K, bool EARLY = true, int RULE = 0, int MAXP = 0, bool PLAIN = false, typename Hook = HEpiNoHook, bool CHAIN = false>
+template <int K, bool EARLY = true, int RULE = 0, int MAXP = 0, bool PLAIN = false, typename Hook = HEpiNoHook, bool CHAIN = false, bool IMPL = false>
 __device__ __forceinline__ void h_epilogue(const HStepArgs& a, float* smem, int nparts, int TP, int tile0, float kl_lane,
                                            const double* colsum = nullptr,
                                            float* lds_tab = nullptr, int lds_rows = 0, bool kl_rows = false,
@@ -187,7 +205,7 @@
     if (lds_tab) {
       float4 hi = make_float4(0.f, 0.f, 0.f, 0.f);
       if constexpr (KP > 4 && K > 4) hi = make_float4(ht[4], ht[5], ht[6], ht[7]);
-      FixTab<K>::put(lds_tab, lds_rows, jj, make_float4(ht[0], ht[1], ht[2], ht[3]), hi);
+      FixTab<K>::template put<IMPL>(lds_tab, lds_rows, jj, make_float4(ht[0], ht[1], ht[2], ht[3]), hi);
     } else {
       store_row_kp(a.h_t + (size_t)q * KP, ht);
     }
@@ -196,7 +214,7 @@
   for (int jj = threadIdx.x; jj < TP; jj += (int)blockDim.x) {
     const int q = tile0 + jj;
     if (q >= a.p) {
-      if (lds_tab) FixTab<K>::put(lds_tab, lds_rows, jj, make_float4(1.f, 1.f, 1.f, 1.f), make_float4(1.f, 1.f, 1.f, 1.f));
+      if (lds_tab) FixTab<K>::template put<IMPL>(lds_tab, lds_rows, jj, make_float4(1.f, 1.f, 1.f, 1.f), make_float4(1.f, 1.f, 1.f, 1.f));
       continue;
     }
     if (!loaded) h_epilogue_load<K, PLAIN>(a, q, stencil, in);
@@ -248,6 +266,12 @@
         nv[kk] = s * a.xscale;
         dv[kk] = (float)(colsum ? colsum[kk] : a.colsum_gw[kk]);
       }
+    }
+    if constexpr (IMPL) {
+      float low = nv[0];
+#pragma unroll
+      for (int kk = 1; kk < K - 1; ++kk) low += nv[kk];
+      nv[K - 1] = fmaxf(nv[K - 1] - low, 0.f);
     }
     ESPM_PHASE_STAMP(40);
     if (f_fill) {
diff --git a/espm_amd/ell.py b/espm_amd/ell.py
--- a/espm_amd/ell.py
+++ b/espm_amd/ell.py
@@ -205,6 +205,17 @@
     return out
 
 
+def block_counts(Xpm, n_pad, tile_px=512):
+    p, n = Xpm.shape
+    PB = 2 * tile_px
+    light, _ = split_heavy(Xpm, PB)
+    nblk_w = (p + PB - 1) // PB
+    out = torch.zeros((nblk_w, n_pad), dtype=torch.float32, device=Xpm.device)
+    for b in range(nblk_w):
+        out[b, :n] = light[b * PB:(b + 1) * PB].to(torch.float64).sum(dim=0).to(torch.float32)
+    return out
+
+
 def lds_bytes_h(n_pad, k):
     wb = 0 if k <= 4 else (1 if k == 5 else (2 if k == 6 else (4 if k <= 8 else (8 if k <= 12 else 12))))
     sets = 2 if k <= _lib.ELL_PAIR_MAX_K else 1
diff --git a/espm_amd/engine.py b/espm_amd/engine.py
--- a/espm_amd/engine.py
+++ b/espm_amd/engine.py
@@ -279,6 +279,7 @@
             self.x_cm = self.x_pm = None
             if torch_builder:
                 self.ell = _ell.build(Xd if layout == "pm" else Xd.t(), st.p_pad, st.ell_cbits, st.tile_px)
+                self.ell["blk_cnt"] = _ell.block_counts(Xd if layout == "pm" else Xd.t(), st.n_pad, st.tile_px)
             else:
                 self.ell = self._build_ell(src, n_heavy, nnz)
                 self._tick("sparse store build")
@@ -402,6 +403,7 @@
                 st.ell_hv_klc, st.ell_hv_kl = self.hv_klc.data_ptr(), self.hv_kl.data_ptr()
             st.ell_w, st.ell_w_off, st.chan_perm = (self.ell[key].data_ptr() for key in ("ell_w", "ell_w_off", "chan_perm"))
             st.pix_perm = self.ell["pix_perm"].data_ptr()
+            st.ell_blk_cnt = self.ell["blk_cnt"].data_ptr()
         st.g = self.g.data_ptr() if self.g is not None else None
         st.g_t = self.g_t.data_ptr() if self.g_t is not None else None
         st.colsum_g = self.colsum_g.data_ptr() if self.colsum_g is not None else None
@@ -468,6 +470,8 @@
         bkt_bc = torch.empty((st.nblk_w, st.n_cg * 64, _lib.ELL_BUCKETS), dtype=torch.uint8, device=dev) if hist else None
         self._check(self.lib.espm_mu_ell_count_hist(C.byref(st), _ptr(x8), _ptr(cnt_px), _ptr(cnt_bc), _ptr(klc),
                                                     _ptr(bkt_px) if hist else None, _ptr(bkt_bc) if hist else None, _stream()))
+        blk_cnt = torch.empty((st.nblk_w, st.n_pad), dtype=torch.float32, device=dev)
+        self._check(self.lib.espm_mu_ell_block_counts(C.byref(st), _ptr(x8), _ptr(blk_cnt), _stream()))
         chan_perm = torch.empty((st.nblk_w, st.n_cg * 64), **i32)
         pix_perm = torch.empty(st.p_pad, **i32)
         h_off = torch.empty(2 * (st.p_pad // 64) + 1, **i32)
@@ -487,7 +491,7 @@
         finally:
             st.x_cm = None
         torch.cuda.current_stream().synchronize()
-        out = dict(ell_h=ell_h, ell_h_off=h_off, klc=klc, pix_perm=pix_perm, ell_w=ell_w, ell_w_off=w_off, chan_perm=chan_perm, n_cg=st.n_cg,
+        out = dict(ell_h=ell_h, ell_h_off=h_off, klc=klc, pix_perm=pix_perm, ell_w=ell_w, ell_w_off=w_off, chan_perm=chan_perm, blk_cnt=blk_cnt, n_cg=st.n_cg,
                    nblk_w=st.nblk_w, nnz=nnz, entries_h=int(cnt_px[0].sum()), entries_w=int(cnt_bc[0].sum()), rows_h=rows_h,
                    rows_w=rows_w, unit_rows_h=int((h_off[1::2] - h_off[0:-1:2]).sum()),
                    unit_rows_w=int((w_off[1::2] - w_off[0:-1:2]).sum()))
diff --git a/include/espm_mu.h b/include/espm_mu.h
--- a/include/espm_mu.h
+++ b/include/espm_mu.h
@@ -80,7 +80,7 @@
 #define ESPM_HI_REL_H 6
 #define ESPM_HI_STRIDE 8
 
-#define ESPM_MU_ABI_VERSION 6
+#define ESPM_MU_ABI_VERSION 7
 
 typedef struct espm_mu_state {
   uint32_t struct_size;
@@ -165,6 +165,7 @@
   const int32_t* ell_hv_grp_off;
   const int32_t* ell_hv_wm;
   double* hpart_alt;
+  const float* ell_blk_cnt;
 } espm_mu_state;
 
 const char* espm_mu_version(void);
@@ -181,6 +182,7 @@
 
 int espm_mu_ell_count(const espm_mu_state* st, const void* x_pm_u8, int32_t* cnt_px, int32_t* cnt_bc, float* ell_klc,
                       espm_stream_t stream);
+int espm_mu_ell_block_counts(const espm_mu_state* st, const void* x_pm_u8, float* blk_cnt, espm_stream_t stream);
 int espm_mu_ell_count_hist(const espm_mu_state* st, const void* x_pm_u8, int32_t* cnt_px, int32_t* cnt_bc, float* ell_klc, uint8_t* bkt_px,
                            uint8_t* bkt_bc, espm_stream_t stream);
 int espm_mu_ell_fill_hist(const espm_mu_state* st, const void* x_pm_u8, const int32_t* chan_perm, const int32_t* pix_perm,
```

Result: faster. 8416 it/s (median of 6 runs) (+10.1%).
